# apache/datafusion-comet

Hardware: AMD Instinct MI355X
Metric: rows/sec, TPC-H SF100 Q1 scan->filter->agg (HBM-resident Arrow columns) (higher is better)
Workload: dtype i128 (Decimal128; 256-bit products) / i32 (Date32) / u8 (Utf8 keys); 1 GPU; TPC-H SF100 Q1 stage 1 (Filter -> Project, 3 decimal ops incl. one 256-bit multiply -> partial HashAggregate, 2 Utf8 keys, 8 aggregates) per GPU; rows_per_gpu=600037902, bytes_per_row_algorithmic=78, parallelism=row-range shards x1, jit_toolchain=hiprtc 9.0; comgr 3.0 /opt/rocm/lib/libamd_comgr.so.3

## Files before the change

### datafusion-comet_amd/csrc/exec.cpp

```cpp
#include "exec.hpp"
#include "shuffle_format.hpp"

#include <cerrno>
#include <fcntl.h>
#include <unistd.h>
#include <chrono>
#include <condition_variable>
#include <cstdio>
#include <cstdlib>
#include <cmath>
#include <cstring>
#include <functional>
#include <map>
#include <mutex>

#include "exec_internal.hpp"

namespace comet {

static bool list_of_flat(const DType& t) { return t.id == TypeId::List && t.kids.size() == 1 && !t.kids[0].is_nested(); }
DevTable extend_struct_fields(const DevTable& in) {
  bool any = false;
  for (auto& t : in.types) any |= t.id == TypeId::Struct || list_of_flat(t);
  if (!any) return in;
// ... 847 lines not shown
    const bool fused = is_build ? fbit != ctx.fused_build_.end() : fit != ctx.fused_probe_.end();
    if (fused || op.children[s].get() == leaf[s]) {
      types[s] = leaf[s]->scan_fields;
      valid[s] = hv;
    } else {
      const PipelineDesc cd = generate_pipeline(*op.children[s], hv);
      for (auto& oc : cd.out_cols) {
        types[s].push_back(oc.type);
        valid[s].push_back(oc.nullable);
      }
    }
  }
  JoinFusion fu, fub;
  if (fit != ctx.fused_probe_.end()) { fu = fit->second.fu; fu.src_valid = valid[build_left ? 1 : 0]; }
  if (fbit != ctx.fused_build_.end()) { fub = fbit->second.fu; fub.src_valid = valid[build_left ? 0 : 1]; }
  return generate_join(op, types[0], types[1], valid[0], valid[1], fit != ctx.fused_probe_.end() ? &fu : nullptr, fbit != ctx.fused_build_.end() ? &fub : nullptr);
}

std::string ExecutionContext::compile_only(OperatorP plan, uint64_t plan_hash) {
  size_t nscan = 0;
  std::function<void(const Operator&)> cnt = [&](const Operator& op) {
    if (op.kind == OpKind::Scan) nscan++;
    for (auto& c : op.children) cnt(*c);
  };
  cnt(*plan);
  std::vector<InputSource> ins(nscan);
  ExecutionContext ctx(plan, plan_hash, {}, ins, 8192, 0);
  std::vector<bool> none(ctx.in_types_.size(), false);
  if (ctx.has_join_) {
    ctx.compile_in_infer_ = true;
    ctx.explain_.clear();
    ctx.infer_schema(*ctx.root_source_);
    if (ctx.plan_.get() != ctx.root_source_) {
      auto pv = planned_variant(*ctx.plan_, ctx.plan_hash_, none, true, &ctx.in_types_);
      ctx.explain_ += pv->desc.explain;
    }
  } else {
    planned_variant(*ctx.plan_, ctx.plan_hash_, none, true);
  }
  return ctx.explain_;
}

Variant ExecutionContext::node_variant(const Operator& node, const char* tag, const std::string& validity, const std::function<PipelineDesc()>& generate) {
  const std::string key = std::to_string(plan_hash_ ^ (0x9E3779B97F4A7C15ull * (uint64_t)(node_id_[&node] + 1))) + tag + validity;
  std::shared_ptr<PlannedVariant> pv;
  {
    std::lock_guard<std::mutex> lk(g_plan_mu);
    auto it = g_plan_cache.find(key);
    if (it != g_plan_cache.end()) pv = it->second;
  }
  if (!pv) {
    pv = std::make_shared<PlannedVariant>();
    pv->desc = generate();
    pv->code = jit_compile(pv->desc.source);
    std::lock_guard<std::mutex> lk(g_plan_mu);
    g_plan_cache[key] = pv;
  }
  Variant v;
  v.desc = pv->desc;
  note_sites(v.desc);
  v.mod = jit_load(pv->code);
  return v;
}

Variant& ExecutionContext::variant_for(const std::vector<bool>& has_valid, const std::vector<int>& str_fixed_len) {
  std::string key = validity_key(has_valid) + ":";
  bool any_fixed = false;
  for (int l : str_fixed_len) { key += std::to_string(l) + ","; any_fixed |= l >= 0; }
  auto it = variants_.find(key);
  if (it != variants_.end()) return it->second;
  auto pv = planned_variant(*plan_, plan_hash_, has_valid, true, has_join_ ? &in_types_ : nullptr, any_fixed ? &str_fixed_len : nullptr,
                            dict_id_col_.empty() ? nullptr : &dict_id_col_);
  Variant v;
  v.desc = pv->desc;
  note_sites(v.desc);
  v.mod = jit_load(pv->code);
  auto res = variants_.emplace(key, std::move(v));
  return res.first->second;
}

void ExecutionContext::launch(Variant& v, const char* kernel, int grid, CometKParams& prm, int block) {
  hipFunction_t fn = v.mod->fn(kernel);
  if (!v.desc.blooms.empty()) bind_blooms(v.desc, prm);
  void* args[] = {&prm};
  if (!g_kernel_times.load(std::memory_order_relaxed)) {
    HIP_CHECK(hipModuleLaunchKernel(fn, (unsigned)grid, 1, 1, (unsigned)block, 1, 1, 0, stream_, args, nullptr));
    return;
  }
  hipEvent_t a = pool_get_event(device_id_), b = pool_get_event(device_id_);
  HIP_CHECK(hipEventRecord(a, stream_));
  HIP_CHECK(hipModuleLaunchKernel(fn, (unsigned)grid, 1, 1, (unsigned)block, 1, 1, 0, stream_, args, nullptr));
  HIP_CHECK(hipEventRecord(b, stream_));
  kt_pending_.push_back({kernel, a, b});
}

std::atomic<int> g_kernel_times{getenv("COMET_KERNEL_TIMES") != nullptr && atoi(getenv("COMET_KERNEL_TIMES")) != 0 ? 1 : 0};

std::string ExecutionContext::kernel_times_json() {
  if (!kt_pending_.empty()) {
    HIP_CHECK(hipStreamSynchronize(stream_));
    for (auto& p : kt_pending_) {
      float ms = 0;
      if (hipEventElapsedTime(&ms, p.a, p.b) == hipSuccess) { kernel_times_[p.name].first += ms; kernel_times_[p.name].second++; }
      pool_put_event(device_id_, p.a);
      pool_put_event(device_id_, p.b);
    }
    kt_pending_.clear();
  }
  std::string s = "{";
  for (auto& kv : kernel_times_) {
    char buf[160];
    snprintf(buf, sizeof buf, "%s\"%s\": {\"ms\": %.6f, \"calls\": %lld}", s.size() > 1 ? ", " : "", kv.first.c_str(), kv.second.first, (long long)kv.second.second);
    s += buf;
  }
  return s + "}";
}

void ExecutionContext::prepare_dict_keys(DevTable& src) {
  if (src.rows == 0) return;
  std::vector<bool> none(in_types_.size(), false);
  auto pv = planned_variant(*plan_, plan_hash_, none, false, &in_types_);
  std::vector<int> key_cols = pv->desc.str_key_cols;
  std::sort(key_cols.begin(), key_cols.end());
  key_cols.erase(std::unique(key_cols.begin(), key_cols.end()), key_cols.end());
  if (key_cols.empty()) return;
  const int64_t n = src.rows;
  std::vector<int> id_col(src.cols.size(), -1);
  bool any = false;
  bool need = device_result_;
  for (int c : key_cols) {
    const DeviceColumnView& sc = src.cols[(size_t)c];
    if (sc.offset != 0) return;
    if (need) break;
    if (sc.fixed_len >= 0 && sc.fixed_len <= 15) continue;
    uint32_t* mx = (uint32_t*)err_flags_.p + (kErrBytes / 4 - 1);
    HIP_CHECK(hipMemsetAsync(mx, 0, 4, stream_));
    if (comet_launch_str_max_len((const int32_t*)sc.data, n, mx, stream_) != 0) throw CometError("string keys: launch failed");
    uint32_t longest = 0;
    read_small(&longest, mx, 4);
    HIP_CHECK(hipMemsetAsync(mx, 0, 4, stream_));
    need = longest > 15;
  }
  if (!need || src.cols.size() + key_cols.size() > COMET_MAX_IN) return;
  for (int c : key_cols) {
    const DeviceColumnView& sc = src.cols[(size_t)c];
    if (n >= ((int64_t)1 << 32) - 1) throw CometError("Utf8 group keys longer than 15 bytes over more than 2^32 rows are not supported");
    int64_t slots = 1024;
    while (slots < 2 * n) slots <<= 1;
    DevBuf table;
    table.ensure((size_t)slots * 4);
    HIP_CHECK(hipMemsetAsync(table.p, 0, (size_t)slots * 4, stream_));
    auto rep = std::make_shared<DevBuf>();
    rep->ensure((size_t)n * 8 + 16);
    if (comet_launch_str_dict_build((const int32_t*)sc.data, (const uint8_t*)sc.aux, src.has_valid[(size_t)c] ? sc.valid : nullptr, n, (uint32_t*)table.p, slots,
                                    (int64_t*)rep->p, stream_) != 0)
      throw CometError("string keys: launch failed");
    HIP_CHECK(hipStreamSynchronize(stream_));
    DeviceColumnView idv;
    idv.data = rep->p;
    idv.valid = sc.valid;
    id_col[(size_t)c] = (int)src.cols.size();
    src.types.push_back(DType::of(TypeId::Int64));
    src.cols.push_back(idv);
    src.has_valid.push_back(src.has_valid[(size_t)c]);
    src.owners.push_back(rep);
    any = true;
// ... 641 lines not shown
  c.type = t;
  c.length = rows;
  auto fetch = [&](std::vector<uint8_t>& dst, const void* src, size_t bytes) {
    dst.resize(bytes);
    if (bytes) HIP_CHECK(hipMemcpyAsync(dst.data(), src, bytes, hipMemcpyDeviceToHost, st));
  };
  if (has_valid && v.valid && rows) fetch(c.validity, v.valid, (size_t)((rows + 7) / 8));
  if (t.id == TypeId::Struct) {
    for (size_t i = 0; i < t.kids.size(); i++)
      c.children.push_back(download_column(v.kids.at(i), t.kids[i], i < v.kid_has_valid.size() && v.kid_has_valid[i], rows, st));
  } else if (t.is_listlike()) {
    fetch(c.values, v.data, (size_t)(rows + 1) * 4);
    HIP_CHECK(hipStreamSynchronize(st));
    const int64_t nel = rows ? ((const int32_t*)c.values.data())[rows] : 0;
    if (nel < 0 || nel > v.kid_rows) throw CometError("internal: list offsets run past the element column");
    c.children.push_back(download_column(v.kids.at(0), t.kids.at(0), !v.kid_has_valid.empty() && v.kid_has_valid[0], nel, st));
  } else if (t.id == TypeId::String || t.id == TypeId::Bytes) {
    fetch(c.values, (const int32_t*)v.data + v.offset, (size_t)(rows + 1) * 4);
    HIP_CHECK(hipStreamSynchronize(st));
    const int32_t* o = (const int32_t*)c.values.data();
    const int64_t lo = rows ? o[0] : 0, hi = rows ? o[rows] : 0;
    if (hi > lo) fetch(c.data, (const uint8_t*)v.aux + lo, (size_t)(hi - lo));
    if (lo) { int32_t* w = (int32_t*)c.values.data(); for (int64_t i = 0; i <= rows; i++) w[i] -= (int32_t)lo; }
  } else if (t.id == TypeId::Bool) {
    fetch(c.values, v.data, (size_t)((rows + 7) / 8));
  } else {
    fetch(c.values, v.data, (size_t)rows * (size_t)fixed_width(t));
  }
  HIP_CHECK(hipStreamSynchronize(st));
  if (!c.validity.empty()) {
    int64_t nulls = 0;
    for (int64_t i = 0; i < rows; i++) nulls += !((c.validity[(size_t)(i >> 3)] >> (i & 7)) & 1);
    c.null_count = nulls;
    if (!nulls) c.validity.clear();
  }
  return c;
}
namespace {
std::vector<uint8_t> slice_bits(const std::vector<uint8_t>& b, int64_t off, int64_t len) {
  std::vector<uint8_t> o((size_t)((len + 7) / 8), 0);
  for (int64_t i = 0; i < len; i++)
    if ((b[(size_t)((off + i) >> 3)] >> ((off + i) & 7)) & 1) o[(size_t)(i >> 3)] |= (uint8_t)(1u << (i & 7));
  return o;
}
HostColumn slice_column(const HostColumn& c, int64_t off, int64_t len) {
  if (off == 0 && len == c.length) return c;
  HostColumn o;
  o.type = c.type;
  o.length = len;
  if (!c.validity.empty()) {
    o.validity = slice_bits(c.validity, off, len);
    for (int64_t i = 0; i < len; i++) o.null_count += !((o.validity[(size_t)(i >> 3)] >> (i & 7)) & 1);
    if (!o.null_count) o.validity.clear();
  }
  const TypeId id = c.type.id;
  if (id == TypeId::Struct) {
    for (auto& k : c.children) o.children.push_back(slice_column(k, off, len));
  } else if (id == TypeId::List || id == TypeId::Map || id == TypeId::String || id == TypeId::Bytes) {
    const int32_t* src = (const int32_t*)c.values.data();
    o.values.resize((size_t)(len + 1) * 4);
    int32_t* w = (int32_t*)o.values.data();
    for (int64_t i = 0; i <= len; i++) w[i] = src[off + i] - src[off];
    if (id == TypeId::List || id == TypeId::Map) o.children.push_back(slice_column(c.children.at(0), src[off], src[off + len] - src[off]));
    else o.data.assign(c.data.begin() + src[off], c.data.begin() + src[off + len]);
  } else if (id == TypeId::Bool) {
    o.values = slice_bits(c.values, off, len);
  } else {
    const size_t w = (size_t)fixed_width(c.type);
    o.values.assign(c.values.begin() + (size_t)off * w, c.values.begin() + (size_t)(off + len) * w);
  }
  return o;
}
}

void ExecutionContext::table_to_host_batches(const DevTable& t) {
  if (t.rows == 0) return;
  const size_t ncol = t.cols.size();
  std::vector<HostColumn> nested(ncol);
  for (size_t j = 0; j < ncol; j++)
    if (t.types[j].is_nested()) nested[j] = download_column(t.cols[j], t.types[j], t.has_valid[j], t.rows, stream_);
  std::vector<std::vector<uint8_t>> hv(ncol), hb(ncol);
  std::vector<std::vector<uint8_t>> hd(ncol);
  struct Piece { const void* src; std::vector<uint8_t>* dst; size_t bytes; };
  auto fetch = [&](std::vector<Piece>& pieces) {
    size_t total = 0, longest = 0;
    for (auto& pc : pieces) { pc.dst->resize(pc.bytes); total += (pc.bytes + 15) & ~(size_t)15; longest = std::max(longest, pc.bytes); }
    if (pieces.empty()) return;
    static const bool batched = getenv("COMET_EXPORT_BATCHED") == nullptr || atoi(getenv("COMET_EXPORT_BATCHED")) != 0;
    if (batched && total > 0 && total <= ((size_t)1 << 20) && pieces.size() <= 256) {
      struct Desc { const uint8_t* src; uint8_t* dst; uint64_t len; };
      const size_t head = (pieces.size() * sizeof(Desc) + 63) & ~(size_t)63;
      export_host_.ensure(head + total + 64);
      Desc* d = (Desc*)export_host_.p;
      size_t at = head;
      for (size_t k = 0; k < pieces.size(); k++) {
        d[k].src = (const uint8_t*)pieces[k].src;
        d[k].dst = (uint8_t*)export_host_.p + at;
        d[k].len = pieces[k].bytes;
        at += (pieces[k].bytes + 15) & ~(size_t)15;
      }
      if (comet_launch_copy_small(export_host_.p, (int)pieces.size(), (uint64_t)longest, stream_) != 0) throw CometError("result export: launch failed");
      HIP_CHECK(hipStreamSynchronize(stream_));
      for (size_t k = 0; k < pieces.size(); k++)
        if (pieces[k].bytes) memcpy(pieces[k].dst->data(), d[k].dst, pieces[k].bytes);
      return;
    }
    for (auto& pc : pieces)
      if (pc.bytes) HIP_CHECK(hipMemcpyAsync(pc.dst->data(), pc.src, pc.bytes, hipMemcpyDeviceToHost, stream_));
    HIP_CHECK(hipStreamSynchronize(stream_));
  };
  std::vector<Piece> pieces;
  for (size_t j = 0; j < ncol; j++) {
    const DType& ty = t.types[j];
    if (ty.is_nested()) continue;
    const bool is_str = ty.id == TypeId::String || ty.id == TypeId::Bytes;
    size_t bytes = is_str ? (size_t)(t.rows + 1) * 4 : ty.id == TypeId::Bool ? (size_t)((t.rows + 7) / 8) : (size_t)t.rows * fixed_width(ty);
    pieces.push_back({t.cols[j].data, &hv[j], bytes});
    if (t.has_valid[j]) pieces.push_back({t.cols[j].valid, &hb[j], (size_t)((t.rows + 7) / 8)});
  }
  fetch(pieces);
  pieces.clear();
  for (size_t j = 0; j < ncol; j++) {
    if (t.types[j].id == TypeId::String || t.types[j].id == TypeId::Bytes) {
      const int32_t* offs = (const int32_t*)hv[j].data();
      if (offs[t.rows] > 0) pieces.push_back({t.cols[j].aux, &hd[j], (size_t)offs[t.rows]});
    }
  }
  fetch(pieces);
  check_device_errors();
  const int64_t bs = batch_size_ > 0 ? batch_size_ : t.rows;
  auto getbit = [](const std::vector<uint8_t>& b, int64_t i) { return (b[(size_t)(i >> 3)] >> (i & 7)) & 1; };
  for (int64_t off = 0; off < t.rows; off += bs) {
    const int64_t len = std::min(bs, t.rows - off);
    HostBatch b;
    b.rows = len;
    for (size_t j = 0; j < ncol; j++) {
      if (t.types[j].is_nested()) { b.cols.push_back(slice_column(nested[j], off, len)); continue; }
      HostColumn c;
      c.type = t.types[j];
      c.length = len;
      if (c.type.id == TypeId::String || c.type.id == TypeId::Bytes) {
        const int32_t* offs = (const int32_t*)hv[j].data();
        c.values.resize((size_t)(len + 1) * 4);
        int32_t* o = (int32_t*)c.values.data();
        for (int64_t i = 0; i <= len; i++) o[i] = offs[off + i] - offs[off];
        c.data.assign(hd[j].begin() + offs[off], hd[j].begin() + offs[off + len]);
      } else if (c.type.id == TypeId::Bool) {
        c.values.assign((size_t)((len + 7) / 8), 0);
        for (int64_t i = 0; i < len; i++)
          if (getbit(hv[j], off + i)) c.values[(size_t)(i >> 3)] |= (uint8_t)(1u << (i & 7));
      } else {
        int w = fixed_width(c.type);
        c.values.assign(hv[j].begin() + (size_t)off * w, hv[j].begin() + (size_t)(off + len) * w);
      }
      if (t.has_valid[j]) {
        int64_t nulls = 0;
        std::vector<uint8_t> bm((size_t)((len + 7) / 8), 0);
        for (int64_t i = 0; i < len; i++) {
          if (getbit(hb[j], off + i)) bm[(size_t)(i >> 3)] |= (uint8_t)(1u << (i & 7));
          else nulls++;
        }
        c.null_count = nulls;
        if (nulls) c.validity = std::move(bm);
      }
      b.cols.push_back(std::move(c));
    }
    ready_.push_back(std::move(b));
  }
}

void ExecutionContext::run_to_completion() {
  if (has_join_) {
    DevTable src = extend_struct_fields(materialize(*root_source_));
    if (plan_.get() == root_source_) throw CometError("internal: bare join root");
    if (sink_ == SinkKind::AggGrouped) prepare_dict_keys(src);
    single_chunk_hint_ = true;
    process_chunk(src.cols, src.has_valid, src.rows);
    HIP_CHECK(hipStreamSynchronize(stream_));
    return;
  }
  while (true) {
    bool more = inputs_[0].kind == 0 ? pull_host_chunk() : pull_device_batch();
    if (!more) break;
  }
}

void ExecutionContext::start() {
  if (!started_) {
    HIP_CHECK(hipSetDevice(device_id_));
    stream_ = pool_get_stream(device_id_);
    err_flags_.ensure(kErrBytes);
    HIP_CHECK(hipMemsetAsync(err_flags_.p, 0, kErrBytes, stream_));
    started_ = true;
  } else {
    HIP_CHECK(hipSetDevice(device_id_));
  }
}

namespace {
struct ExportedDeviceColumn {
  std::vector<std::shared_ptr<void>> owners;
  const void* buffers[3];
};
void release_device_array(ArrowArray* a) {
  delete (ExportedDeviceColumn*)a->private_data;
  a->release = nullptr;
}
void release_fmt_schema(ArrowSchema* s) {
  delete (std::string*)s->private_data;
  s->release = nullptr;
}
}

void ExecutionContext::set_memory_manager(int64_t (*acquire)(void*, int64_t), void (*release)(void*, int64_t), void* ctx, long long task_id) {
  mem_->acquire = acquire;
  mem_->release = release;
  mem_->ctx = ctx;
  mem_->task_id = task_id;
}
void ExecutionContext::memory_stats(int64_t out[4]) {
  out[0] = mem_->host_used.load();
  out[1] = mem_->host_peak.load();
  out[2] = mem_->dev_used.load();
  out[3] = mem_->dev_peak.load();
}

int64_t ExecutionContext::execute_device(ArrowDeviceArray** out_arrays, ArrowSchema** out_schemas, int n_out) {
  mem_->owner = std::this_thread::get_id();
  AccountScope account(mem_);
  mem_->flush();
  Timer t;
  start();
  if (sink_ == SinkKind::AggNoGroup)
    throw CometError("comet_execute_plan_device: an ungrouped aggregate result is one row and is exported through comet_execute_plan");
  if (finished_) return -1;
  DevTable tab;
  if (sink_ == SinkKind::AggGrouped) {
    device_result_ = true;
    run_to_completion();
    tab = grouped_to_device();
  } else {
    tab = materialize(*plan_);
  }
  HIP_CHECK(hipStreamSynchronize(stream_));
  check_device_errors();
  collect_timings();
  finished_ = true;
  if ((size_t)n_out != tab.cols.size())
    throw CometError("Output column count mismatch: expected " + std::to_string(n_out) + ", got " + std::to_string(tab.cols.size()));
  for (size_t c = 0; c < tab.types.size(); c++)
    if (tab.types[c].is_nested()) throw CometError("executePlan (device arrays): nested column of type " + tab.types[c].str() + " — nested results are exported through host batches");
  for (int j = 0; j < n_out; j++) {
    const DType& ty = tab.types[(size_t)j];
    const bool is_str = ty.id == TypeId::String || ty.id == TypeId::Bytes;
    if (tab.cols[(size_t)j].offset != 0) throw CometError("comet_execute_plan_device: input column with a non-zero Arrow offset passed through");
    auto* ec = new ExportedDeviceColumn();
    ec->owners = tab.owners;
    ec->buffers[0] = tab.has_valid[(size_t)j] ? tab.cols[(size_t)j].valid : nullptr;
    ec->buffers[1] = tab.cols[(size_t)j].data;
    ec->buffers[2] = is_str ? tab.cols[(size_t)j].aux : nullptr;
    ArrowDeviceArray* d = out_arrays[j];
    memset(d, 0, sizeof *d);
    d->array.length = tab.rows;
    d->array.null_count = tab.has_valid[(size_t)j] ? -1 : 0;
    d->array.n_buffers = is_str ? 3 : 2;
    d->array.buffers = ec->buffers;
    d->array.private_data = ec;
    d->array.release = release_device_array;
    d->device_id = device_id_;
    d->device_type = ARROW_DEVICE_ROCM;
    d->sync_event = nullptr;
    ArrowSchema* s = out_schemas[j];
    memset(s, 0, sizeof *s);
    auto* fmt = new std::string(expected_format(ty));
    s->format = fmt->c_str();
    s->name = "";
    s->flags = ARROW_FLAG_NULLABLE;
    s->private_data = fmt;
    s->release = release_fmt_schema;
  }
  output_rows_ += tab.rows;
  elapsed_compute_ns_ += t.ns();
  return tab.rows;
}

void ExecutionContext::resolve_subqueries() {
  if (subqueries_resolved_) return;
  subqueries_resolved_ = true;
  uint64_t sig = 0xcbf29ce484222325ull;
  auto mix = [&](const void* p, size_t n) { for (size_t k = 0; k < n; k++) sig = (sig ^ ((const uint8_t*)p)[k]) * 0x100000001b3ull; };
  for (auto& e : plan_->subqueries) {
    if (e->kind != ExprKind::Subquery) continue;
    const int64_t id = e->lit_i64;
    bool is_null = true;
    std::string v;
    bool found = false;
    auto it = subquery_values_.find(id);
    if (it != subquery_values_.end()) { is_null = it->second.first; v = it->second.second; found = true; }
    else if (subquery_provider_) found = subquery_provider_(id, e->dtype, is_null, v);
    if (!found) throw CometError("Subquery " + std::to_string(id) + " is not registered with this plan (CometScalarSubquery.setSubquery / comet_plan_set_subquery)");
    auto need = [&](size_t n) { if (!is_null && v.size() < n) throw CometError("Subquery " + std::to_string(id) + ": the value has " + std::to_string(v.size()) + " bytes, its type needs " + std::to_string(n)); };
    e->kind = ExprKind::Literal;
    e->proto_tag = 2;
    e->lit_null = is_null;
    e->lit_i64 = 0;
    int64_t i = 0;
    double d = 0;
    switch (e->dtype.id) {
      case TypeId::Bool: need(1); e->lit_bool = !is_null && v[0] != 0; e->lit_case = 1; break;
      case TypeId::Int8: case TypeId::Int16: case TypeId::Int32: case TypeId::Date: case TypeId::Int64: case TypeId::Timestamp: case TypeId::TimestampNtz:
        need(8);
        if (!is_null) memcpy(&i, v.data(), 8);
        e->lit_i64 = i;
        e->lit_case = e->dtype.id == TypeId::Int8 ? 2 : e->dtype.id == TypeId::Int16 ? 3 : (e->dtype.id == TypeId::Int32 || e->dtype.id == TypeId::Date) ? 4 : 5;
        break;
      case TypeId::Float: case TypeId::Double:
        need(8);
        if (!is_null) memcpy(&d, v.data(), 8);
        e->lit_f64 = e->dtype.id == TypeId::Float ? (double)(float)d : d;
        e->lit_case = e->dtype.id == TypeId::Float ? 6 : 7;
        break;
      case TypeId::Decimal: e->lit_dec = is_null ? 0 : decode_decimal_be(v); e->lit_case = 10; break;
      case TypeId::String: case TypeId::Bytes: e->lit_bytes = is_null ? std::string() : v; e->lit_case = e->dtype.id == TypeId::String ? 8 : 9; break;
      default: throw CometError("Unsupported scalar subquery data type " + e->dtype.str());
    }
    mix(&id, 8);
    mix(&is_null, 1);
    if (e->bloom_arg) {
// ... 89 lines not shown
```

### datafusion-comet_amd/csrc/exec.hpp

```cpp
#pragma once
#include <mutex>
#include <thread>
#include <atomic>
#include <hip/hip_runtime_api.h>

#include <deque>
#include <functional>
#include <map>
#include <set>
#include <memory>
#include <string>
#include <vector>

#include "arrow_abi.hpp"
#include "codegen.hpp"
#include "jit.hpp"
#include "kparams.h"
#include "plan.hpp"

namespace comet {
double process_clock_ms();

struct MemAccount {
  int64_t (*acquire)(void* ctx, int64_t bytes) = nullptr;
// ... 76 lines not shown

struct DevTable {
  int64_t rows = 0;
  std::vector<DType> types;
  std::vector<DeviceColumnView> cols;
  std::vector<bool> has_valid;
  std::vector<std::shared_ptr<void>> owners;
};

struct Staging {
  std::vector<std::unique_ptr<PinnedBuf>> stage_vals, stage_valid, stage_aux;
  std::vector<std::unique_ptr<DevBuf>> dev_vals, dev_valid, dev_aux;
  std::vector<int> dict_index_width;
  std::vector<std::shared_ptr<void>> nested_keep;
  hipEvent_t busy = nullptr;
};

struct Variant {
  PipelineDesc desc;
  std::shared_ptr<LoadedModule> mod;
};

struct BloomAggSpec { int version = 1, k = 1; int64_t num_words = 0; };
BloomAggSpec bloom_agg_spec(const Operator& hash_agg);
bool is_bloom_agg(const Operator& op);
struct BloomRegistry {
  std::map<int64_t, ExprP> subquery_nodes;
  std::map<const Expr*, std::shared_ptr<struct DevBuf>> buffers;
  std::vector<ExprP> keep;
};

void scan_pool_parallel(size_t n, const std::function<void(size_t)>& fn);
std::string parquet_prune_report(const Operator& native_scan, bool page_index, bool bloom_filters = true);
std::vector<uint8_t> parquet_host_plain_values(const Operator& native_scan, size_t column);
void scan_pool_submit(std::function<void()> fn);

extern std::atomic<int> g_kernel_times;

class ExecutionContext {
 public:
  ExecutionContext(OperatorP plan, uint64_t plan_hash, std::vector<std::pair<std::string, std::string>> config,
                   std::vector<InputSource> inputs, int batch_size, int device_id);
  ~ExecutionContext();

  int64_t execute(ArrowArray** out_arrays, ArrowSchema** out_schemas, int n_out);
  int64_t execute_device(ArrowDeviceArray** out_arrays, ArrowSchema** out_schemas, int n_out);
  std::string metrics_proto();
  void set_memory_manager(int64_t (*acquire)(void*, int64_t), void (*release)(void*, int64_t), void* ctx, long long task_id);
  typedef std::function<bool(int64_t id, const DType& type, bool& is_null, std::string& value)> SubqueryProvider;
  void set_subquery_provider(SubqueryProvider p) { subquery_provider_ = std::move(p); }
  void set_subquery_value(int64_t id, bool is_null, std::string value) { subquery_values_[id] = {is_null, std::move(value)}; }
  void resolve_subqueries();
  void memory_stats(int64_t out[4]);
  std::shared_ptr<MemAccount> memory_account() const { return mem_; }
  const std::string& explain();
  static std::string compile_only(OperatorP plan, uint64_t plan_hash);
  static std::string check_only(OperatorP plan, uint64_t plan_hash);
  static PipelineDesc join_codegen(OperatorP plan, uint64_t plan_hash, const std::vector<bool>& has_valid);

  std::string last_error;
  int last_error_kind = 0;

  double last_kernel_ms = 0;
  int64_t last_kernel_launches = 0;
  std::string kernel_times_json();
  double last_aux_ms = 0;
  int64_t last_aux_launches = 0;
  int64_t input_rows = 0;

 private:
  void run_to_completion();
  void start();
  std::vector<std::vector<int>> fixed_len_hint_;
  Variant& variant_for(const std::vector<bool>& has_valid, const std::vector<int>& str_fixed_len);
  void process_chunk(const std::vector<DeviceColumnView>& cols, const std::vector<bool>& has_valid, int64_t n);
  void finish_aggregate();
  void finish_grouped();
  DevTable grouped_to_device();
  std::vector<DType> infer_schema(const Operator& op);
  DevTable materialize(const Operator& op);
  DevTable scan_parquet(const Operator& native_scan);
  friend struct ParquetScan;
  friend struct HashJoinRun;
  int64_t launch_fused_filter(Variant& v, CometKParams& prm, int64_t n);
  DevTable run_chain_to_device(const Operator& top, const DevTable& in);
  void extend_derived(DevTable& in, const std::vector<DerivedCol>& derived);
  void extend_derived_strfn(DevTable& in, const DerivedCol& dc);
  DevTable hash_join(const Operator& j, const DevTable& l, const DevTable& r);
  DevTable hash_join_impl(const Operator& node, const Operator& j, const DevTable& l, const DevTable& r, const std::string& key_suffix,
                          const JoinFusion* fused_probe = nullptr, const JoinFusion* fused_build = nullptr);
  struct FusedProbe { const Operator* source = nullptr; JoinFusion fu; };
  bool plan_fused_probe(const Operator& join, const std::vector<DType>& build_types, PipelineDesc& desc);
  bool plan_fused_build(const Operator& join, FusedProbe& fb);
  DevTable sort_table(const Operator& s, const DevTable& in);
  Variant node_variant(const Operator& node, const char* tag, const std::string& validity, const std::function<PipelineDesc()>& generate);
  std::shared_ptr<DevBuf> sort_key_planes(const Operator& s, const DevTable& in, int& W, std::vector<int64_t>* str_len = nullptr, bool measure_only = false);
  DevTable literal_table(const std::vector<std::vector<ExprP>>& rows, const std::vector<DType>& types);
  DevTable take_rows(const DevTable& in, const uint32_t* dev_perm, int64_t first, int64_t rows, std::shared_ptr<DevBuf> perm_owner);
  DevTable nested_aggregate(const Operator& agg);
  DevTable write_shuffle(const Operator& sw);
  DevTable expand(const Operator& ex, const DevTable& in);
  DevTable explode(const Operator& ex, const DevTable& in);
  DevTable window(const Operator& w, const DevTable& in);
  DevTable bloom_aggregate(const Operator& agg, const DevTable& in);
  const void* bloom_buffer(const PipelineDesc::BloomRef& ref);
  void bind_blooms(const PipelineDesc& d, CometKParams& prm);
  void prepare_dict_keys(DevTable& src);
  static bool is_source(const Operator& op, const Operator* chain_top);
  typedef std::function<std::pair<const DevTable*, int>(int)> GatherSource;
  DevTable outputs_to_table(Variant& v, const std::vector<std::shared_ptr<DevBuf>>& vals, const std::vector<std::shared_ptr<DevBuf>>& valid_bytes,
                            int64_t rows, const GatherSource& gather_source = nullptr);
  DeviceColumnView take_column(const DeviceColumnView& src, const DType& t, bool has_valid, const uint32_t* idx, const uint8_t* ok_bytes, int64_t rows, bool& out_has_valid,
                               std::vector<std::shared_ptr<void>>& owners);
  void take_utf8(const DeviceColumnView& src, const uint32_t* idx, const uint8_t* ok_bytes, const uint8_t* src_valid_bits, int64_t rows,
                 DeviceColumnView& out, std::vector<std::shared_ptr<void>>& owners);
  void table_to_host_batches(const DevTable& t);
  DevTable host_batch_to_table(const HostBatch& b);
  bool pull_host_chunk();
  bool pull_device_batch();
  bool pull_host_table(size_t input, const std::vector<DType>& types, int64_t max_rows, std::vector<DeviceColumnView>& views,
                       std::vector<bool>& has_valid, int64_t& rows);
  bool pull_device_table(size_t input, const std::vector<DType>& types, std::vector<DeviceColumnView>& views, std::vector<bool>& has_valid,
                         int64_t& rows, std::shared_ptr<void>& keepalive);
  void validate_input_schema(size_t input, const std::vector<DType>& types);
  void export_batch(HostBatch& b, ArrowArray** out_arrays, ArrowSchema** out_schemas, int n_out);
  void check_device_errors();
  void raise_device_errors(uint32_t flags);
  void note_sites(const PipelineDesc& d) {
    site_ctx_last_.clear();
    for (auto& kv : d.site_contexts) {
      site_ctx_last_[kv.first] = kv.second;
      auto it = site_ctx_.find(kv.first);
      if (it == site_ctx_.end()) site_ctx_[kv.first] = kv.second;
      else if (it->second != kv.second && !(it->second && kv.second && it->second->sql_text == kv.second->sql_text && it->second->start_index == kv.second->start_index &&
                                            it->second->stop_index == kv.second->stop_index))
        site_ctx_ambiguous_.insert(kv.first);
    }
    for (int k = 0; k < 2; k++) if (d.agg_ctx[k]) agg_ctx_[k] = d.agg_ctx[k];
  }
  const QueryContext* site_context(uint32_t id) const {
    auto a = site_ctx_last_.find(id);
    if (a != site_ctx_last_.end()) return a->second.get();
    if (site_ctx_ambiguous_.count(id)) return nullptr;
    auto b = site_ctx_.find(id);
    return b == site_ctx_.end() ? nullptr : b->second.get();
  }
  std::map<uint32_t, std::shared_ptr<QueryContext>> site_ctx_last_;
  std::set<uint32_t> site_ctx_ambiguous_;
  std::shared_ptr<QueryContext> agg_ctx_[2];
  std::map<uint32_t, std::shared_ptr<QueryContext>> site_ctx_;
  void read_small(void* dst, const void* dev_src, size_t n);
  void write_small(void* dev_dst, const void* src, size_t n);
  void timed_begin();
  void timed_end();
  void collect_timings();
  void launch(Variant& v, const char* kernel, int grid, CometKParams& prm, int block = 256);

  OperatorP plan_;
  uint64_t plan_hash_ = 0;
  std::vector<std::pair<std::string, std::string>> config_;
  std::vector<InputSource> inputs_;
  int batch_size_;
  int device_id_;
  int64_t chunk_rows_;
  hipStream_t stream_ = nullptr;
  std::vector<std::pair<hipEvent_t, hipEvent_t>> timed_;
  size_t timed_done_ = 0;
  struct KtPending { std::string name; hipEvent_t a, b; };
  std::vector<KtPending> kt_pending_;
  std::map<std::string, std::pair<double, int64_t>> kernel_times_;
  hipEvent_t aux_ev_[2] = {nullptr, nullptr};
  int aux_n_ = 0;
  bool started_ = false, finished_ = false;
  std::vector<DType> in_types_;
  std::map<std::string, Variant> variants_;
  Variant* agg_variant_ = nullptr;
  std::string explain_;
  SinkKind sink_ = SinkKind::Output;
  bool has_join_ = false;
  SubqueryProvider subquery_provider_;
  std::map<int64_t, std::pair<bool, std::string>> subquery_values_;
  bool subqueries_resolved_ = false;
  int64_t strfn_rows_ = 0;
  int64_t split_rows_ = 0;
  bool materialize_root_ = false;
  bool compile_in_infer_ = false;
  std::vector<const Operator*> nested_aggs_;
  struct ExpandPart {
    OperatorP proj;
    std::vector<int> out_col;
    std::vector<int> null_cols;
  };
  struct ExpandInfo {
    std::vector<ExpandPart> parts;
    std::vector<OutCol> out_cols;
  };
  std::map<const Operator*, ExpandInfo> expand_info_;
  std::map<const Operator*, OperatorP> bloom_proj_;
  std::shared_ptr<BloomRegistry> blooms_;
  std::map<const Operator*, OperatorP> explode_proj_;
  std::map<const Operator*, OperatorP> window_psort_, window_osort_;
  std::map<const Operator*, OperatorP> range_sort_, range_bsort_;
  std::shared_ptr<void> planes_owner_;
  std::map<const Operator*, OperatorP> shuffle_projs_;
  int64_t shuffle_bytes_written_ = 0, shuffle_data_size_ = 0, shuffle_staged_peak_ = 0;
  double shuffle_repart_ns_ = 0, shuffle_write_ns_ = 0;
  std::vector<int> dict_id_col_;
  bool device_result_ = false;
  DevTable dict_src_;
  std::map<const Operator*, FusedProbe> fused_probe_;
  std::map<const Operator*, FusedProbe> fused_build_;
  int64_t ramp_rows_ = 0;
  bool fuse_probe_ = true;
  int fuse_build_ = 1;
  std::set<const Operator*> smj_needs_sort_;
  std::map<const Operator*, OperatorP> smj_sorts_;
  const Operator* root_source_ = nullptr;
  std::map<const Operator*, int> node_id_;
  std::map<const Operator*, size_t> scan_input_;
  int64_t join_build_rows_ = 0, join_probe_rows_ = 0, join_keymap_bytes_ = 0, join_direct_maps_ = 0, join_bucket_tables_ = 0, join_bitmap_only_ = 0, join_mono_tables_ = 0, join_fused_builds_ = 0;
  int small_write_slot_ = 0;
  bool single_chunk_hint_ = false, part_result_ready_ = false;
  DevTable part_result_;
  int64_t part_merges_ = 0;
  bool try_partitioned_merge(Variant& v, CometKParams& prm, int64_t n);
  struct DevPending {
    std::vector<DeviceColumnView> views;
    std::vector<bool> has_valid;
    int64_t rows = 0;
    std::shared_ptr<void> keep;
    bool valid = false;
  };
  DevPending dev_pending_;
  bool dev_stream_done_ = false;
// ... 40 lines not shown
```

### datafusion-comet_amd/csrc/exec_bloom.cpp

```cpp
#include "exec_internal.hpp"
#include "device/bloom.hpp"

#include "../../include/comet_amd.h"

extern "C" int comet_launch_bloom_put(const void* vals, int width, const uint8_t* valid_bits, int64_t first, int64_t n, uint64_t* f, int64_t nwords, void* stream);
extern "C" int comet_launch_bloom_merge(const uint8_t* src_words, int64_t nwords, uint64_t* f, void* stream);
extern "C" int comet_launch_bloom_finish(const uint64_t* f, int64_t nwords, uint8_t* out, uint64_t* popcnt, void* stream);

namespace comet {

namespace {

uint32_t be32(const uint8_t* p) { return ((uint32_t)p[0] << 24) | ((uint32_t)p[1] << 16) | ((uint32_t)p[2] << 8) | p[3]; }

struct BloomHeader {
  int32_t version = 0, k = 0, seed = 0, num_words = 0;
  size_t header_bytes = 0;
};

bool read_header(const uint8_t* p, size_t len, BloomHeader& h) {
  if (len < 4) return false;
  h.version = (int32_t)be32(p);
  h.header_bytes = h.version == 2 ? 16 : 12;
  if (h.version != 1 && h.version != 2) return true;
// ... 99 lines not shown
  auto hit = blooms_->buffers.find(node);
  if (hit != blooms_->buffers.end()) return hit->second->p;
  if (node->kind != ExprKind::Literal || node->lit_null) throw CometError("internal: might_contain bound to a filter without bytes");
  BloomHeader h;
  const uint8_t* p = (const uint8_t*)node->lit_bytes.data();
  const std::string why = bloom_bytes_problem(p, node->lit_bytes.size(), h);
  if (!why.empty()) throw CometError("might_contain: " + why);
  const std::vector<uint64_t> f = to_device_layout(p, h);
  auto buf = std::make_shared<DevBuf>();
  buf->ensure(f.size() * 8);
  HIP_CHECK(hipMemcpy(buf->p, f.data(), f.size() * 8, hipMemcpyHostToDevice));
  blooms_->buffers[node] = buf;
  blooms_->keep.push_back(ref.node);
  return buf->p;
}

void ExecutionContext::bind_blooms(const PipelineDesc& d, CometKParams& prm) {
  for (size_t j = 0; j < d.blooms.size(); j++) prm.in[COMET_MAX_IN - 1 - j].data = bloom_buffer(d.blooms[j]);
}


DevTable ExecutionContext::bloom_aggregate(const Operator& op, const DevTable& in) {
  const BloomAggSpec spec = bloom_agg_spec(op);
  const size_t fbytes = ((size_t)kBloomHeaderWords + (size_t)spec.num_words + 1) * 8;
  DevBuf acc;
  acc.ensure(fbytes);
  HIP_CHECK(hipMemsetAsync(acc.p, 0, fbytes, stream_));
  const uint64_t header[kBloomHeaderWords] = {(uint64_t)spec.version, (uint64_t)spec.k, 0, (uint64_t)spec.num_words};
  write_small(acc.p, header, sizeof header);
  uint64_t* const f = (uint64_t*)acc.p;
  uint64_t* const popcnt = f + kBloomHeaderWords + spec.num_words;
  if (op.agg_mode == AggMode::Partial) {
    DevTable col = run_chain_to_device(*bloom_proj_.at(&op), in);
    const DType& t = col.types.at(0);
    if (!t.is_integer()) throw CometError("bloom_filter_agg over " + t.str() + " is not supported by the MI355X native engine");
    timed_begin();
    if (comet_launch_bloom_put(col.cols[0].data, fixed_width(t), col.has_valid[0] ? col.cols[0].valid : nullptr, col.cols[0].offset, col.rows, f, spec.num_words, stream_) != 0)
      throw CometError("bloom_filter_agg: launch failed");
    HIP_CHECK(hipStreamSynchronize(stream_));
  } else {
    const size_t sc = (size_t)std::max(0, op.initial_input_buffer_offset);
    if (sc >= in.cols.size() || (in.types[sc].id != TypeId::Bytes && in.types[sc].id != TypeId::String))
      throw CometError("bloom_filter_agg: the merging aggregate expects its Binary state in column " + std::to_string(sc) + " of its child");
    const DeviceColumnView& s = in.cols[sc];
    std::vector<int32_t> offs((size_t)in.rows + 1, 0);
    std::vector<uint8_t> vbits;
    if (in.rows) {
      HIP_CHECK(hipMemcpyAsync(offs.data(), (const int32_t*)s.data + s.offset, offs.size() * 4, hipMemcpyDeviceToHost, stream_));
      if (in.has_valid[sc] && s.valid) {
        vbits.resize((size_t)((s.offset + in.rows + 7) / 8));
        HIP_CHECK(hipMemcpyAsync(vbits.data(), s.valid, vbits.size(), hipMemcpyDeviceToHost, stream_));
      }
      HIP_CHECK(hipStreamSynchronize(stream_));
    }
    timed_begin();
    for (int64_t r = 0; r < in.rows; r++) {
      if (!vbits.empty() && !((vbits[(size_t)((s.offset + r) >> 3)] >> ((s.offset + r) & 7)) & 1)) continue;
      const int64_t lo = offs[(size_t)r], len = (int64_t)offs[(size_t)r + 1] - lo;
      if (lo < 0 || len < 0) throw CometError("bloom_filter_agg: the state column's offsets are not ascending");
      uint8_t hb[16] = {0};
      const size_t have = (size_t)std::min<int64_t>(len, 16);
      if (have) read_small(hb, (const uint8_t*)s.aux + lo, have);
      BloomHeader h;
      if (have < 4) throw CometError("BloomFilter merge: truncated bit array (got 0 bytes, expected " + std::to_string(spec.num_words * 8) + ")");
      h.version = (int32_t)be32(hb);
      if (h.version != spec.version) throw CometError("BloomFilter merge: version mismatch (got " + std::to_string(h.version) + ", expected " + std::to_string(spec.version) + ")");
      if (!read_header(hb, have, h)) throw CometError("BloomFilter merge: truncated bit array (got 0 bytes, expected " + std::to_string(spec.num_words * 8) + ")");
      if (h.k != spec.k) throw CometError("BloomFilter merge: num_hash_functions mismatch (got " + std::to_string((uint32_t)h.k) + ", expected " + std::to_string(spec.k) + ")");
      if (h.seed != 0) throw CometError("BloomFilter merge: seed mismatch (got " + std::to_string(h.seed) + ", expected 0)");
      if ((int64_t)h.num_words != spec.num_words)
        throw CometError("BloomFilter merge: num_words mismatch (got " + std::to_string((uint32_t)h.num_words) + ", expected " + std::to_string(spec.num_words) + ")");
      if (len - (int64_t)h.header_bytes < spec.num_words * 8)
        throw CometError("BloomFilter merge: truncated bit array (got " + std::to_string(len - (int64_t)h.header_bytes) + " bytes, expected " + std::to_string(spec.num_words * 8) + ")");
      if (comet_launch_bloom_merge((const uint8_t*)s.aux + lo + h.header_bytes, spec.num_words, f, stream_) != 0) throw CometError("bloom_filter_agg: launch failed");
    }
  }
  const size_t hdr = spec.version == 2 ? 16 : 12, out_len = hdr + (size_t)spec.num_words * 8;
  auto bytes = std::make_shared<DevBuf>(), out_offs = std::make_shared<DevBuf>();
  bytes->ensure(out_len + 16);
  out_offs->ensure(16);
  if (comet_launch_bloom_finish(f, spec.num_words, (uint8_t*)bytes->p, popcnt, stream_) != 0) throw CometError("bloom_filter_agg: launch failed");
  timed_end();
  uint64_t set_bits = 0;
  read_small(&set_bits, popcnt, 8);
  check_device_errors();
  const bool is_null = op.agg_mode == AggMode::Final && set_bits == 0;
  const int32_t o[2] = {0, is_null ? 0 : (int32_t)out_len};
  write_small(out_offs->p, o, sizeof o);
  DevTable out;
  out.rows = 1;
  out.types.push_back(DType::of(TypeId::Bytes));
  DeviceColumnView v;
  v.data = out_offs->p;
  v.aux = bytes->p;
  out.owners.push_back(out_offs);
  out.owners.push_back(bytes);
  if (is_null) {
    auto vb = std::make_shared<DevBuf>();
    vb->ensure(16);
    const uint8_t zero[8] = {0};
    write_small(vb->p, zero, sizeof zero);
    v.valid = (const uint8_t*)vb->p;
    out.owners.push_back(vb);
  }
  out.cols.push_back(v);
  out.has_valid.push_back(is_null);
  HIP_CHECK(hipStreamSynchronize(stream_));
  return out;
}

}


extern "C" int32_t comet_spark_bloom_might_contain(const uint8_t* bytes, size_t len, int64_t value) {
  comet::BloomHeader h;
  if (!bytes || !comet::bloom_bytes_problem(bytes, len, h).empty()) return -1;
  const std::vector<uint64_t> f = comet::to_device_layout(bytes, h);
  return comet::bloom_might_contain((const comet::u64*)f.data(), (comet::i64)value) ? 1 : 0;
}

extern "C" int64_t comet_spark_bloom_build(const int64_t* values, const uint8_t* valid, int64_t n, int64_t num_items, int64_t num_bits, int32_t version, uint8_t* out, int64_t cap) {
  comet::Operator op;
  op.kind = comet::OpKind::HashAgg;
  comet::AggExpr a;
  a.kind = comet::AggKind::BloomFilter;
  auto lit = [](int64_t v) {
    auto e = std::make_shared<comet::Expr>();
    e->kind = comet::ExprKind::Literal;
    e->dtype = comet::DType::of(comet::TypeId::Int64);
    e->has_dtype = true;
    e->lit_i64 = v;
    return e;
  };
  a.children.push_back(lit(0));
  a.bloom_num_items = lit(num_items);
  a.bloom_num_bits = lit(num_bits);
  a.bloom_version = version == 2 ? 2 : 1;
  op.agg_exprs.push_back(a);
  comet::BloomAggSpec s;
  try {
    s = comet::bloom_agg_spec(op);
  } catch (const comet::CometError&) {
    return -1;
  }
  std::vector<uint64_t> f((size_t)comet::kBloomHeaderWords + (size_t)s.num_words, 0);
  f[0] = (uint64_t)s.version;
  f[1] = (uint64_t)s.k;
  f[3] = (uint64_t)s.num_words;
  for (int64_t i = 0; i < n; i++)
    if (!valid || ((valid[i >> 3] >> (i & 7)) & 1)) comet::bloom_put((comet::u64*)f.data(), (comet::i64)values[i]);
  const std::string bytes = comet::serialize(f);
  if (out && cap >= (int64_t)bytes.size()) memcpy(out, bytes.data(), bytes.size());
  return (int64_t)bytes.size();
}
```

### datafusion-comet_amd/csrc/exec_input.cpp

```cpp
#include "exec_internal.hpp"
#include <emmintrin.h>
#include <mutex>
#include <set>
#include <tuple>

namespace comet {

static void stream_copy(void* dst, const void* src, size_t n) {
  char* d = (char*)dst;
  const char* s = (const char*)src;
  if (n < 4096) { memcpy(d, s, n); return; }
  const size_t head = (size_t)(-(intptr_t)d) & 15;
  if (head) { memcpy(d, s, head); d += head; s += head; n -= head; }
  size_t blocks = n / 64;
  for (; blocks; blocks--, d += 64, s += 64) {
    const __m128i a = _mm_loadu_si128((const __m128i*)s), b = _mm_loadu_si128((const __m128i*)(s + 16)), c = _mm_loadu_si128((const __m128i*)(s + 32)),
                  e = _mm_loadu_si128((const __m128i*)(s + 48));
    _mm_stream_si128((__m128i*)d, a);
    _mm_stream_si128((__m128i*)(d + 16), b);
    _mm_stream_si128((__m128i*)(d + 32), c);
    _mm_stream_si128((__m128i*)(d + 48), e);
  }
  _mm_sfence();
  if (n & 63) memcpy(d, s, n & 63);
// ... 487 lines not shown
}


namespace {
struct UniformKey {
  const void* off; int64_t rows; int32_t len; int32_t first;
  bool operator<(const UniformKey& o) const { return std::tie(off, rows, len, first) < std::tie(o.off, o.rows, o.len, o.first); }
};
std::mutex g_uniform_mu;
std::set<UniformKey> g_uniform_ok;
bool uniform_verdict_known(const void* off, int64_t rows, int32_t len, int32_t first) {
  std::lock_guard<std::mutex> g(g_uniform_mu);
  return g_uniform_ok.count(UniformKey{off, rows, len, first}) != 0;
}
void remember_uniform_verdict(const void* off, int64_t rows, int32_t len, int32_t first) {
  std::lock_guard<std::mutex> g(g_uniform_mu);
  if (g_uniform_ok.size() >= 4096) g_uniform_ok.clear();
  g_uniform_ok.insert(UniformKey{off, rows, len, first});
}
}

bool ExecutionContext::pull_device_table(size_t input, const std::vector<DType>& types, std::vector<DeviceColumnView>& views,
                                         std::vector<bool>& has_valid, int64_t& rows, std::shared_ptr<void>& keepalive) {
  InputSource& in = inputs_[input];
  rows = 0;
  if (in.exhausted) return false;
  static const bool trace = getenv("COMET_TRACE_STAGES") != nullptr;
  Timer tm;
  validate_input_schema(input, types);
  const double t_schema = tm.ns();
  auto da = std::make_shared<ArrowDeviceArray>();
  memset(da.get(), 0, sizeof(ArrowDeviceArray));
  int rc = in.dev->get_next(in.dev, da.get());
  if (trace) fprintf(stderr, "[comet] device input %zu: get_schema %.3f ms, get_next %.3f ms\n", input, t_schema / 1e6, (tm.ns() - t_schema) / 1e6);
  if (rc != 0) {
    const char* m = in.dev->get_last_error ? in.dev->get_last_error(in.dev) : nullptr;
    throw CometError(std::string("input ArrowDeviceArrayStream.get_next failed: ") + (m ? m : "unknown error"));
  }
  if (!da->array.release) {
    in.exhausted = true;
    return false;
  }
  keepalive = std::shared_ptr<void>(da.get(), [da](void*) mutable {
    if (da->array.release) da->array.release(&da->array);
  });
  if (da->device_type != ARROW_DEVICE_ROCM && da->device_type != ARROW_DEVICE_ROCM_HOST)
    throw CometError("device input stream must carry ARROW_DEVICE_ROCM memory");
  if (da->sync_event) HIP_CHECK(hipStreamWaitEvent(stream_, *(hipEvent_t*)da->sync_event, 0));
  const size_t nc = types.size();
  if ((size_t)da->array.n_children != nc) throw CometError("device batch column count does not match Scan fields");
  views.assign(nc, DeviceColumnView());
  has_valid.assign(nc, false);
  for (size_t c = 0; c < nc; c++) {
    const ArrowArray* col = da->array.children[c];
    if (col->dictionary) throw CometError("dictionary-encoded device columns are not supported yet");
    views[c].data = col->buffers[1];
    views[c].offset = col->offset;
    if (types[c].id == TypeId::String || types[c].id == TypeId::Bytes) views[c].aux = col->buffers[2];
    if (types[c].id == TypeId::Decimal && (((uintptr_t)col->buffers[1]) & 15))
      throw CometError("device Decimal128 buffers must be 16-byte aligned");
    if (col->null_count != 0 && col->buffers[0]) {
      has_valid[c] = true;
      views[c].valid = (const uint8_t*)col->buffers[0];
    }
  }
  rows = da->array.length;
  std::vector<size_t> scols;
  for (size_t c = 0; c < nc && rows > 0; c++)
    if (types[c].id == TypeId::String) scols.push_back(c);
  if (!scols.empty() && scols.size() <= 16) {
    small_host_.ensure(4096);
    int32_t* ends = (int32_t*)small_host_.p;
    for (size_t k = 0; k < scols.size(); k++) {
      const ArrowArray* col = da->array.children[scols[k]];
      const int32_t* off = (const int32_t*)col->buffers[1] + col->offset;
      HIP_CHECK(hipMemcpyAsync(ends + 2 * k, off, 4, hipMemcpyDeviceToHost, stream_));
      HIP_CHECK(hipMemcpyAsync(ends + 2 * k + 1, off + rows, 4, hipMemcpyDeviceToHost, stream_));
    }
    HIP_CHECK(hipStreamSynchronize(stream_));
    std::vector<int32_t> first(scols.size()), len(scols.size(), -1);
    std::vector<bool> declared(scols.size(), false);
    uint32_t* flags = (uint32_t*)err_flags_.p + (kErrBytes / 4 - 16);
    HIP_CHECK(hipMemsetAsync(flags, 0, 64, stream_));
    bool any = false;
    if (!aux_ev_[0]) { aux_ev_[0] = pool_get_event(device_id_); aux_ev_[1] = pool_get_event(device_id_); }
    HIP_CHECK(hipEventRecord(aux_ev_[0], stream_));
    int aux_launched = 0;
    for (size_t k = 0; k < scols.size(); k++) {
      first[k] = ends[2 * k];
      const int64_t total = (int64_t)ends[2 * k + 1] - ends[2 * k];
      const int hint = input < fixed_len_hint_.size() && scols[k] < fixed_len_hint_[input].size() ? fixed_len_hint_[input][scols[k]] : -1;
      const ArrowArray* col = da->array.children[scols[k]];
      const int32_t* off = (const int32_t*)col->buffers[1] + col->offset;
      if (hint >= 0) {
        if (total != (int64_t)hint * rows)
          throw CometError("device input column " + std::to_string(scols[k]) + " is declared comet:utf8_fixed_len=" + std::to_string(hint) + " but holds " +
                           std::to_string(total) + " bytes in " + std::to_string(rows) + " rows");
        if ((int64_t)first[k] != (int64_t)col->offset * hint) continue;
        if (uniform_verdict_known(off, rows, hint, first[k])) {
          views[scols[k]].fixed_len = hint;
          continue;
        }
        if (comet_launch_utf8_uniform(off, rows, hint, flags + k, stream_) != 0) continue;
        aux_launched++;
        len[k] = hint;
        declared[k] = true;
        any = true;
        continue;
      }
      if (total % rows != 0 || total / rows > 15 || total < 0) continue;
      if (comet_launch_utf8_uniform(off, rows, (int32_t)(total / rows), flags + k, stream_) != 0) continue;
      aux_launched++;
      len[k] = (int32_t)(total / rows);
      any = true;
    }
    if (any) {
      HIP_CHECK(hipEventRecord(aux_ev_[1], stream_));
      uint32_t f[16];
      read_small(f, flags, 64);
      float aux = 0;
      if (hipEventElapsedTime(&aux, aux_ev_[0], aux_ev_[1]) == hipSuccess) { last_aux_ms += aux; last_aux_launches += aux_launched; }
      HIP_CHECK(hipMemsetAsync(flags, 0, 64, stream_));
      for (size_t k = 0; k < scols.size(); k++) {
        if (len[k] < 0) continue;
        const size_t c = scols[k];
        const ArrowArray* col = da->array.children[c];
        if (declared[k]) {
          if (f[k] != 0)
            throw CometError("device input column " + std::to_string(c) + " is declared comet:utf8_fixed_len=" + std::to_string(len[k]) +
                             " but its offsets are not " + std::to_string(len[k]) + " bytes apart (the byte total alone matches)");
          remember_uniform_verdict((const int32_t*)col->buffers[1] + col->offset, rows, len[k], first[k]);
          views[c].fixed_len = len[k];
          continue;
        }
        if (f[k] != 0) continue;
        if ((int64_t)first[k] != (int64_t)col->offset * len[k]) continue;
        views[c].fixed_len = len[k];
      }
    }
  }
  return true;
}

bool ExecutionContext::pull_device_batch() {
  DevPending cur;
  if (dev_pending_.valid) {
    cur = std::move(dev_pending_);
    dev_pending_ = DevPending();
  } else {
    if (dev_stream_done_ || !pull_device_table(0, in_types_, cur.views, cur.has_valid, cur.rows, cur.keep)) return false;
  }
  if (sink_ == SinkKind::AggGrouped && dev_chunks_seen_ == 0 && !dev_stream_done_) {
    dev_pending_.valid = pull_device_table(0, in_types_, dev_pending_.views, dev_pending_.has_valid, dev_pending_.rows, dev_pending_.keep);
    if (!dev_pending_.valid) dev_stream_done_ = true;
    single_chunk_hint_ = !dev_pending_.valid;
  } else {
    single_chunk_hint_ = false;
  }
  dev_chunks_seen_++;
  process_chunk(cur.views, cur.has_valid, cur.rows);
  HIP_CHECK(hipStreamSynchronize(stream_));
  return true;
}


}
```

### datafusion-comet_amd/csrc/exec_internal.hpp

```cpp
#pragma once
#include "exec.hpp"
#include "shuffle_format.hpp"
#include "fix_scale.hpp"

#include <cerrno>
#include <fcntl.h>
#include <unistd.h>
#include <chrono>
#include <condition_variable>
#include <cstdio>
#include <cstdlib>
#include <cmath>
#include <cstring>
#include <functional>
#include <map>
#include <mutex>

extern "C" int comet_launch_dict_gather_fixed(const void* idx, int iw, const uint8_t* idx_valid, const uint8_t* dict, const uint8_t* dict_valid,
                                              int width, int64_t n, uint8_t* out, uint8_t* out_valid_bytes, void* stream);
extern "C" int comet_launch_dict_gather_str_len(const void* idx, int iw, const uint8_t* idx_valid, const int32_t* dict_offs, const uint8_t* dict_valid,
                                                int64_t n, uint32_t* lengths, uint8_t* out_valid_bytes, void* stream);
extern "C" int comet_launch_dict_gather_str_copy(const void* idx, int iw, const uint8_t* valid_bytes, const int32_t* dict_offs, const uint8_t* dict_bytes,
                                                 int64_t n, const int32_t* out_offs, uint8_t* out_bytes, void* stream);
extern "C" void pq_launch_u32_scan(const uint32_t* in, int64_t n, uint64_t* tiles, int32_t* out, void* st);
// ... 8 lines not shown
                                          int out_width, void* out, uint8_t* out_ok, void* stream);
extern "C" int comet_launch_window_range_bounds(int width, const void* keys, const uint8_t* valid, const int32_t* sp, const uint32_t* first_part, int64_t n, int desc, int nulls_first,
                                                int has_lo, int64_t dlo, int has_hi, int64_t dhi, int32_t* out_lo, int32_t* out_hi, void* stream);
extern "C" int comet_launch_window_valid_flags(const uint8_t* valid, int64_t n, uint32_t* flags, void* stream);
extern "C" int comet_launch_window_pick(int mode, int64_t nth, int lo_kind, int64_t lo_off, int hi_kind, int64_t hi_off, const int32_t* C, const int32_t* sp, const int32_t* sg,
                                        const uint32_t* first_part, const uint32_t* first_peer, int64_t n, uint32_t* idx, uint8_t* ok, void* stream);
extern "C" int comet_launch_window_agg(int fn, int lo_kind, int64_t lo_off, int hi_kind, int64_t hi_off, const void* S128, const void* SH128, const int32_t* C, const int32_t* sp, const int32_t* sg, const uint32_t* first_part,
                                       const uint32_t* first_peer, int64_t n, const void* bound16, const void* scaler16, const void* avg_bound16, void* out, uint8_t* out_ok,
                                       void* stream);
extern "C" int comet_launch_window_fexp(int width, const void* src, const uint8_t* valid_bits, int64_t n, uint64_t* hi_lo, void* stream);
extern "C" int comet_launch_scan192_f64(int width, const void* src, const uint8_t* valid_bits, int64_t n, int scale, int slice, void* tiles, void* out192, void* stream);
extern "C" int comet_launch_scan128_fclass(int width, const void* src, const uint8_t* valid_bits, int64_t n, void* tiles, void* out128, void* stream);
extern "C" int comet_launch_window_fagg(int fn, int lo_kind, int64_t lo_off, int hi_kind, int64_t hi_off, const void* S192, int windows, const void* K128, int scale, const int32_t* sp, const int32_t* sg,
                                        const uint32_t* first_part, const uint32_t* first_peer, int64_t n, double* out, uint8_t* out_ok, void* stream);
extern "C" int comet_launch_window_flags(const uint8_t* part_planes, int Wp, const uint8_t* order_planes, int Wo, int64_t n, uint32_t* fpart, uint32_t* fpeer, void* stream);
extern "C" int comet_launch_window_first(const uint32_t* fpart, const int32_t* sp, const uint32_t* fpeer, const int32_t* sg, int64_t n, uint32_t* first_part,
                                         uint32_t* first_peer, void* stream);
extern "C" int comet_launch_window_rank(int kind, int64_t arg, const int32_t* sp, const int32_t* sg, const uint32_t* first_part, const uint32_t* first_peer, int64_t n,
                                        void* out, void* stream);
extern "C" int comet_launch_window_offset(int64_t shift, const int32_t* sp, const uint32_t* first_part, int64_t n, uint32_t* idx, uint8_t* ok, void* stream);
extern "C" int comet_launch_window_offset_valid(const uint32_t* idx, const uint8_t* ok, const uint8_t* src_valid_bits, int64_t n, uint8_t* out_ok, void* stream);
struct CometConcatArgs {
  int32_t n;
  int32_t lit_len[8];
  const int32_t* offs[8];
  const uint8_t* bytes[8];
  int64_t first[8];
};
extern "C" int comet_launch_concat_lengths(const CometConcatArgs* a, const uint32_t* rows, const uint8_t* ok_bytes, int64_t n, uint32_t* lengths, void* stream);
extern "C" int comet_launch_concat_copy(const CometConcatArgs* a, const uint32_t* rows, const uint8_t* ok_bytes, int64_t n, const int32_t* out_offs, uint8_t* out_bytes, void* stream);
extern "C" int comet_launch_strcase_lengths(const void* views, const uint8_t* ok_bytes, const int32_t* src_offs, const uint8_t* src_bytes, int64_t n, int mode, uint32_t* lengths, void* stream);
extern "C" int comet_launch_strcase_write(const void* views, const uint8_t* ok_bytes, const int32_t* src_offs, const uint8_t* src_bytes, int64_t n, int mode, const int32_t* out_offs,
                                          uint8_t* out_bytes, void* stream);
extern "C" int comet_launch_join_part_scan(uint32_t* cnt, int g, int np, uint32_t* tot, uint32_t limit, uint64_t* over, void* stream);
extern "C" int comet_launch_popcount128(const void* blocks, int64_t n, uint32_t* counts, void* stream);
extern "C" int comet_launch_strfmt_lengths(int kind, long long arg, const void* vals128, const uint8_t* ok_bytes, int64_t n, uint32_t* lengths, void* stream);
extern "C" int comet_launch_strfmt_write(int kind, long long arg, const void* vals128, const uint8_t* ok_bytes, int64_t n, const int32_t* out_offs, uint8_t* out_bytes, void* stream);
extern "C" int comet_launch_strfn_len(int op, const int32_t* offs, const uint8_t* bytes, const uint8_t* valid_bits, int64_t valid_first, int64_t n, const uint8_t* a, int32_t na, const uint8_t* b,
                                      int32_t nb, int64_t k, uint32_t* lengths, uint32_t* too_long, void* stream);
extern "C" int comet_launch_strfn_write(int op, const int32_t* offs, const uint8_t* bytes, const uint8_t* valid_bits, int64_t valid_first, int64_t n, const uint8_t* a, int32_t na, const uint8_t* b,
                                        int32_t nb, int64_t k, const int32_t* out_offs, uint8_t* out, void* stream);
extern "C" int comet_launch_split_count(const int32_t* offs, const uint8_t* bytes, const uint8_t* valid_bits, int64_t valid_first, int64_t n, const uint32_t* prog, const uint32_t* prog2, int32_t limit,
                                        uint32_t* counts, void* stream);
extern "C" int comet_launch_split_write(const int32_t* offs, const uint8_t* bytes, const uint8_t* valid_bits, int64_t valid_first, int64_t n, const uint32_t* prog, const uint32_t* prog2, int32_t limit,
                                        const int32_t* list_offs, void* views, void* stream);
extern "C" int comet_launch_strview_lengths(const void* views, const uint8_t* ok_bytes, int64_t n, const uint8_t* pattern, int32_t pattern_bytes, uint32_t* lengths, void* stream);
extern "C" int comet_launch_strview_copy(const void* views, const uint8_t* ok_bytes, const int32_t* src_offs, const uint8_t* src_bytes, int64_t n, const uint8_t* pattern,
                                         int32_t pattern_bytes, int pad_left, const int32_t* out_offs, uint8_t* out_bytes, void* stream);
extern "C" int comet_launch_str16_lengths(const void* packed, const uint8_t* ok_bytes, int64_t n, uint32_t* lengths, void* stream);
extern "C" int comet_launch_str16_copy(const void* packed, const int32_t* offsets, int64_t n, uint8_t* bytes, void* stream);
extern "C" int comet_launch_str_max_len(const int32_t* offs, int64_t n, uint32_t* out_max, void* stream);
extern "C" int comet_launch_str_dict_build(const int32_t* offs, const uint8_t* bytes, const uint8_t* valid_bits, int64_t n, uint32_t* table, int64_t slots,
                                           int64_t* rep, void* stream);
extern "C" int comet_launch_str_dict_lookup(const int32_t* build_offs, const uint8_t* build_bytes, const uint32_t* table, int64_t slots, const int32_t* offs,
                                            const uint8_t* bytes, const uint8_t* valid_bits, int64_t n, int64_t* rep, uint8_t* ok, void* stream);
extern "C" int64_t comet_partition_tiles(int64_t n);
extern "C" int64_t comet_partition_scratch_bytes(int64_t n, int32_t P);
extern "C" int comet_launch_fill(int width, void* dst, int64_t n, const void* value, void* stream);
extern "C" int comet_launch_copy_small(const void* descs, int n, uint64_t longest, void* stream);
extern "C" int comet_launch_murmur3(int type_id, int precision, const void* values, const uint8_t* validity, const void* aux, int64_t n, uint32_t* hashes, void* stream);
extern "C" int comet_launch_pmod(const uint32_t* hashes, int64_t n, int32_t np, int32_t* out, void* stream);
extern "C" int comet_launch_partition_indices(const int32_t* pids, int64_t n, int32_t P, uint64_t* hist, uint32_t* bad, int64_t* starts,
                                              uint32_t* row_indices, void* stream);
extern "C" int comet_launch_take(int width, const void* src, const uint32_t* idx, int64_t n, void* dst, void* stream);
extern "C" int comet_launch_take_utf8_lengths(const int32_t* offs, const uint32_t* idx, const uint8_t* ok_bytes, const uint8_t* src_valid_bits, int64_t n,
                                              uint32_t* lengths, void* stream);
extern "C" int comet_launch_explode_counts(const int32_t* offs, const uint8_t* valid_bits, int64_t n, int outer, uint32_t* counts, void* stream);
extern "C" int comet_launch_explode_indices(const int32_t* offs, const uint8_t* valid_bits, const uint8_t* elem_valid_bits, int64_t n, const int32_t* out_offs, uint32_t* row_idx,
                                            uint32_t* elem_idx, uint8_t* has_elem, int32_t* pos, uint8_t* elem_ok, void* stream);
extern "C" int comet_launch_take_list_indices(const int32_t* offs, const uint32_t* idx, int64_t n, const int32_t* out_offs, uint32_t* elem_idx, void* stream);
extern "C" int comet_launch_take_utf8_copy(const int32_t* offs, const uint8_t* bytes, const uint32_t* idx, const uint8_t* ok_bytes, const uint8_t* src_valid_bits,
                                           int64_t n, const int32_t* out_offs, uint8_t* out_bytes, void* stream);
extern "C" void pq_launch_u32_scan(const uint32_t* in, int64_t n, uint64_t* tiles, int32_t* out, void* st);
extern "C" int comet_launch_sort_small(const uint8_t* planes, int64_t n, const uint32_t* cand, int m, const int* plane_idx, int nv, uint32_t* out, void* stream);
extern "C" int comet_launch_sort_iota(uint32_t* perm, int64_t n, uint32_t first, void* stream);
extern "C" int comet_launch_sort_gather_digit(const uint8_t* plane, const uint32_t* perm, int64_t n, int32_t* digit, void* stream);
extern "C" int comet_launch_range_partition_ids(const uint8_t* planes, int64_t n, int W, const uint8_t* bkeys, int B, int32_t* pids, void* stream);
extern "C" int comet_launch_sort_plane_varies(const uint8_t* planes, int64_t n, int W, uint32_t* flags, void* stream);
extern "C" int comet_launch_sort_hist256(const uint8_t* plane, const uint32_t* cand, int64_t m, uint64_t* hist, void* stream);
extern "C" int comet_launch_sort_select(const uint8_t* plane, const uint32_t* cand, int64_t m, int dstar, uint32_t* sure, uint32_t* next_cand, uint32_t* counters,
                                        void* stream);
extern "C" int comet_launch_fix_rescale(uint64_t* base, int64_t count, int64_t stride_words, int32_t word_off, int32_t shift, void* stream);
extern "C" int comet_launch_utf8_uniform(const int32_t* offsets, int64_t n, int32_t L, uint32_t* flag, void* stream);

namespace comet {
HostColumn download_column(const DeviceColumnView& v, const DType& t, bool has_valid, int64_t rows, hipStream_t st);

namespace detail {
void plan_execution_begins();
void plan_execution_ends();
int plans_executing();

hipStream_t pool_get_stream(int dev);
void pool_put_stream(int dev, hipStream_t s);
hipEvent_t pool_get_event(int dev);
void pool_put_event(int dev, hipEvent_t e);

int fixed_width(const DType& t);
inline int out_width(const OutCol& oc) { return (oc.view_src >= 0 || oc.fmt_kind) ? 16 : (oc.gather_src >= 0 || !oc.concat_cols.empty()) ? 4 : oc.packed_string ? 16 : (oc.type.id == TypeId::Bool ? 1 : fixed_width(oc.type)); }
void bit_append(uint8_t* dst, int64_t dst_off, const uint8_t* src, int64_t src_off, int64_t n);
bool nested_schema_matches(const ArrowSchema* f, const DType& t);
void append_nested_rows(HostColumn& dst, const ArrowArray* a, const DType& t, int64_t off, int64_t len);
void bit_fill_ones(uint8_t* dst, int64_t dst_off, int64_t n);
bool format_matches(const char* fmt, const DType& t);
struct SrcFmt {
  enum Cls { Unknown, Int, UInt, F32, F64, Date32, Date64, Ts, Dec, Utf8, LargeUtf8, Bool } cls = Unknown;
  int width = 0;
  int64_t per_second = 0;
  int p = 0, s = 0;
};
SrcFmt parse_src_format(const char* fmt);
bool scan_cast_supported(const SrcFmt& f, const DType& t);
bool scan_cast_value(const SrcFmt& f, const char* src, int64_t i, const DType& t, char* dst);
const Operator* find_scan(const Operator* op);
std::string validity_key(const std::vector<bool>& v);
void bind_inputs(CometKParams& prm, const std::vector<DeviceColumnView>& cols, const std::vector<bool>& has_valid, size_t first_slot = 0);
u128 pow10_u128_host(int p);
struct Timer {
  std::chrono::steady_clock::time_point t0 = std::chrono::steady_clock::now();
  double ns() const { return (double)std::chrono::duration_cast<std::chrono::nanoseconds>(std::chrono::steady_clock::now() - t0).count(); }
};

struct PlannedVariant {
  PipelineDesc desc;
  std::shared_ptr<CodeObject> code;
};
extern std::mutex g_plan_mu;
extern std::map<std::string, std::shared_ptr<PlannedVariant>> g_plan_cache;
std::shared_ptr<PlannedVariant> planned_variant(const Operator& plan, uint64_t plan_hash, const std::vector<bool>& has_valid, bool compile,
                                                const std::vector<DType>* source_types = nullptr, const std::vector<int>* str_fixed_len = nullptr,
                                                const std::vector<int>* dict_id_col = nullptr);

}
using namespace detail;
}
```

### datafusion-comet_amd/csrc/exec_join.cpp

```cpp
#include "exec_internal.hpp"

namespace comet {
DevTable ExecutionContext::hash_join(const Operator& j, const DevTable& L, const DevTable& R) {
  auto is_str = [](const DType& t) { return t.id == TypeId::String || t.id == TypeId::Bytes; };
  std::vector<size_t> sk;
  for (size_t k = 0; k < j.left_keys.size() && k < j.right_keys.size(); k++) {
    const ExprP &a = j.left_keys[k], &b = j.right_keys[k];
    if (a->kind == ExprKind::Bound && b->kind == ExprKind::Bound && a->bound_index >= 0 && b->bound_index >= 0 && (size_t)a->bound_index < L.types.size() &&
        (size_t)b->bound_index < R.types.size() && is_str(L.types[(size_t)a->bound_index]) && is_str(R.types[(size_t)b->bound_index]) &&
        L.cols[(size_t)a->bound_index].offset == 0 && R.cols[(size_t)b->bound_index].offset == 0)
      sk.push_back(k);
  }
  if (sk.empty() || L.rows == 0 || R.rows == 0 || L.cols.size() + R.cols.size() + 2 * sk.size() > COMET_MAX_IN) return hash_join_impl(j, j, L, R, "");
  auto longest = [&](const DevTable& t, int c) {
    uint32_t* mx = (uint32_t*)err_flags_.p + (kErrBytes / 4 - 1);
    HIP_CHECK(hipMemsetAsync(mx, 0, 4, stream_));
    if (comet_launch_str_max_len((const int32_t*)t.cols[(size_t)c].data, t.rows, mx, stream_) != 0) throw CometError("string keys: launch failed");
    uint32_t v = 0;
    read_small(&v, mx, 4);
    HIP_CHECK(hipMemsetAsync(mx, 0, 4, stream_));
    return v;
  };
  bool need = false;
  for (size_t k : sk) need = need || longest(L, j.left_keys[k]->bound_index) > 15 || longest(R, j.right_keys[k]->bound_index) > 15;
// ... 257 lines not shown
      HIP_CHECK(hipMemsetAsync(counter(kCntOverflow), 0, 8, stream()));
    }
    cx.launch(v, "k_jpscat", (int)g, prm, 1024);
    cx.launch(v, "k_jtbuild", (int)np, prm);
    cx.join_bucket_tables_++;
    if (mono) cx.join_mono_tables_++;
    return true;
  }

  void build_chained() {
    const bool chained = table == JoinTable::Lds || table == JoinTable::Chained;
    int64_t cap = 1024;
    if (chained) {
      while (cap < 2 * st.entries) cap <<= 1;
      head.ensure((size_t)cap * 4);
      next.ensure((size_t)std::max<int64_t>(B.rows, 1) * 4 + 16);
      HIP_CHECK(hipMemsetAsync(head.p, 0xff, (size_t)cap * 4, stream()));
    }
    nbtiles = (B.rows + 1023) / 1024;
    if (v.desc.join_outer_build) {
      matched.ensure((size_t)std::max<int64_t>(B.rows, 1));
      btiles.ensure((size_t)(nbtiles + 1) * 8);
      HIP_CHECK(hipMemsetAsync(matched.p, 0, (size_t)std::max<int64_t>(B.rows, 1), stream()));
      prm.out[kJoinOutMatched] = matched.p;
      prm.out[kJoinOutBuildTiles] = btiles.p;
      prm.iarg[kJoinArgBuildTiles] = nbtiles;
    }
    if (table != JoinTable::Bucket) {
      int ib = 1;
      while (ib < 31 && ((int64_t)1 << ib) - 1 < std::max<int64_t>(B.rows, 1)) ib++;
      if (((int64_t)1 << ib) - 1 < B.rows) throw CometError("HashJoin: build sides of 2^31 rows or more are not supported");
      chained_table_args(prm, cap, ib);
    }
    if (chained) {
      prm.out[kJoinOutTable] = head.p;
      prm.out[kJoinOutRows] = next.p;
    }
    prm.out[kOutErr] = cx.err_flags_.p;
    cx.timed_begin();
    if (table == JoinTable::Chained && B.rows) cx.launch(v, "k_jbuild", build_grid(), prm);
    prm.out[kJoinOutCounters] = counters.p;
  }

  void maybe_sample_keymap() {
    if (table == JoinTable::BitmapOnly || table == JoinTable::Direct || keymap_built) return;
    if (!(st.keymap_range && set.keymap != 0 && n >= (1 << 20) && (set.keymap == 1 || n >= 4 * B.rows))) return;
    bool wanted = set.keymap == 1;
    if (!wanted) {
      HIP_CHECK(hipMemsetAsync(counters.p, 0, 16, stream()));
      const int64_t ns = 8192;
      sample_args(prm, ns);
      cx.launch(v, table == JoinTable::Bucket ? "k_jsample_b" : "k_jsample", (int)((ns + 255) / 256), prm);
      uint64_t cnt[2] = {0, 0};
      cx.read_small(cnt, counters.p, sizeof cnt);
      wanted = cnt[0] >= 64 && cnt[1] * 2 < cnt[0];
    }
    if (wanted) build_keymap(false);
  }

  void bind_outputs(int64_t rows_cap) {
    const PipelineDesc& d = v.desc;
    for (size_t c = 0; c < d.out_cols.size(); c++) {
      if (!vals[c]) vals[c] = std::make_shared<DevBuf>();
      vals[c]->ensure((size_t)std::max<int64_t>(rows_cap, 1) * out_width(d.out_cols[c]) + 16);
      prm.out[kOutFirstCol + 2 * c] = vals[c]->p;
      if (!vbytes[c]) vbytes[c] = std::make_shared<DevBuf>();
      if (d.out_cols[c].nullable) {
        vbytes[c]->ensure((size_t)std::max<int64_t>(rows_cap, 1) + 16);
        prm.out[kOutFirstCol + 2 * c + 1] = vbytes[c]->p;
      }
    }
  }

  bool probe() {
    const PipelineDesc& d = v.desc;
    int64_t out_cap = d.join_build_only ? 1 : n + 1024;
    for (int attempt = 0; n > 0; attempt++) {
      bind_outputs(out_cap);
      probe_args(prm, out_cap);
      HIP_CHECK(hipMemsetAsync(counter(kCntEmitted), 0, 8, stream()));
      const int64_t ptiles = (n + 4095) / 4096;
      cx.launch(v, probe_kernel(table, keymap_built), (int)std::min<int64_t>(ptiles, table == JoinTable::Lds ? 256 * 3 : 256 * 8), prm);
      uint64_t words[8] = {0, 0, 0, 0, 0, 0, 0, 0};
      cx.read_small(words, counters.p, sizeof words);
      if (table == JoinTable::Bucket && words[kCntOverflow]) {
        cx.timed_end();
        HIP_CHECK(hipStreamSynchronize(stream()));
        cx.join_bucket_tables_--;
        return false;
      }
      out_rows = d.join_build_only ? 0 : (int64_t)words[kCntEmitted];
      if (out_rows <= out_cap) break;
      if (attempt == 1) throw CometError("internal: hash join output exceeded its exact size");
      out_cap = out_rows;
    }
    probe_capacity = n > 0 ? out_cap : 0;
    return true;
  }

  void outer_tail() {
    const PipelineDesc& d = v.desc;
    const size_t ncol = d.out_cols.size();
    if (d.join_outer_build && B.rows > 0) {
      cx.launch(v, "k_jbcount", (int)std::min<int64_t>(nbtiles, 256 * 8), prm);
      cx.launch(v, "k_jbscan", 1, prm);
      uint64_t total = 0;
      cx.read_small(&total, (char*)btiles.p + (size_t)nbtiles * 8, 8);
      tail_rows = (int64_t)total;
      prm.iarg[kJoinArgTailBase] = out_rows;
    }
    const int64_t all_rows = out_rows + tail_rows;
    if (all_rows > probe_capacity || (ncol > 0 && !vals[0])) {
      std::vector<std::shared_ptr<DevBuf>> ov = vals, ob = vbytes;
      for (size_t c = 0; c < ncol; c++) { vals[c].reset(); vbytes[c].reset(); }
      bind_outputs(all_rows);
      for (size_t c = 0; c < ncol && out_rows > 0; c++) {
        HIP_CHECK(hipMemcpyAsync(vals[c]->p, ov[c]->p, (size_t)out_rows * out_width(d.out_cols[c]), hipMemcpyDeviceToDevice, stream()));
        if (d.out_cols[c].nullable) HIP_CHECK(hipMemcpyAsync(vbytes[c]->p, ob[c]->p, (size_t)out_rows, hipMemcpyDeviceToDevice, stream()));
      }
      HIP_CHECK(hipStreamSynchronize(stream()));
    }
    if (tail_rows > 0) cx.launch(v, "k_jbemit", (int)std::min<int64_t>(nbtiles, 256 * 8), prm);
    cx.timed_end();
    out_rows = all_rows;
  }

  DevTable finish() {
    const int nbuild = (int)B.cols.size();
    DevTable out = cx.outputs_to_table(v, vals, vbytes, out_rows, [&](int c) { return c < nbuild ? std::make_pair(&B, c) : std::make_pair(&P, c - nbuild); });
    if (fused_probe || fused_build) cx.check_device_errors();
    if (tail_rows > 0 || n == 0) HIP_CHECK(hipStreamSynchronize(stream()));
    out.owners.push_back(v.mod);
    cx.join_build_rows_ += B.rows;
    cx.join_probe_rows_ += P.rows;
    return out;
  }

  bool run() {
    plan();
    const bool use_lds = B.rows > 0 && B.rows <= 6144;
    bool bucket = !use_lds && allow_bucket && set.bucket_min_rows >= 0 && B.rows >= set.bucket_min_rows;
    if (!use_lds && B.rows >= (bucket ? 65536 : (1 << 20))) count_build();
    table = use_lds ? JoinTable::Lds : JoinTable::Chained;
    if (st.keymap_range != 0 && v.desc.join_dedup_build && set.bitmap_only != 0 && n > 0) {
      build_keymap(false);
      table = JoinTable::BitmapOnly;
      cx.join_bitmap_only_++;
    } else if (st.keymap_range && set.direct != 0 && st.entries == st.keyed_rows) {
      if (try_direct()) table = JoinTable::Direct;
    }
    if (bucket && table == JoinTable::Chained && B.rows != 0 && build_bucket()) table = JoinTable::Bucket;
    vals.resize(v.desc.out_cols.size());
    vbytes.resize(v.desc.out_cols.size());
    build_chained();
    maybe_sample_keymap();
    if (!probe()) return false;
    outer_tail();
    return true;
  }
};

DevTable ExecutionContext::hash_join_impl(const Operator& node, const Operator& j, const DevTable& L, const DevTable& R, const std::string& key_suffix,
                                          const JoinFusion* fused_probe, const JoinFusion* fused_build) {
  for (bool allow_bucket : {true, false}) {
    HashJoinRun run(*this, node, j, L, R, key_suffix, fused_probe, fused_build, allow_bucket);
    if (run.run()) return run.finish();
  }
  throw CometError("internal: a hash join without a bucket table reported a bucket overflow");
}

}
```

### datafusion-comet_amd/csrc/exec_pipeline.cpp

```cpp
#include "exec_internal.hpp"

namespace comet {
void ExecutionContext::process_chunk(const std::vector<DeviceColumnView>& cols, const std::vector<bool>& has_valid, int64_t n) {
  if (n == 0) return;
  std::vector<int> fixed_lens(cols.size(), -1);
  for (size_t i = 0; i < cols.size(); i++) fixed_lens[i] = cols[i].fixed_len;
  Variant& v = variant_for(has_valid, fixed_lens);
  const PipelineDesc& d = v.desc;
  if (d.max_rows_exact && input_rows + n > d.max_rows_exact)
    throw CometError("decimal or integer sum over more rows than its static no-overflow proof allows (" + std::to_string(d.max_rows_exact) + ")");
  CometKParams prm;
  memset(&prm, 0, sizeof prm);
  prm.n = n;
  bind_inputs(prm, cols, has_valid);
  err_flags_.ensure(kErrBytes);
  prm.out[kOutErr] = err_flags_.p;
  if (!has_join_) input_rows += n;
  if (d.sink == SinkKind::AggNoGroup || d.sink == SinkKind::AggGrouped) {
    prm.iarg[kRowBaseArg] = agg_rows_seen_;
    agg_rows_seen_ += n;
  }

  if (d.sink == SinkKind::AggNoGroup) {
    if (agg_variant_ && agg_variant_->desc.NW != d.NW) throw CometError("internal: accumulator layout differs between variants");
    agg_variant_ = &v;
    const int64_t tile = (int64_t)d.R * 256;
    int grid = (int)std::min<int64_t>((n + tile - 1) / tile, 256 * 8);
    size_t need = (size_t)(n_partials_ + grid) * d.NW * 8;
    if (need > partials_.cap) {
      DevBuf bigger;
      bigger.ensure(std::max(need * 2, (size_t)(4096 * d.NW * 8)));
      if (n_partials_) HIP_CHECK(hipMemcpyAsync(bigger.p, partials_.p, (size_t)n_partials_ * d.NW * 8, hipMemcpyDeviceToDevice, stream_));
      HIP_CHECK(hipStreamSynchronize(stream_));
      std::swap(partials_.p, bigger.p);
      std::swap(partials_.cap, bigger.cap);
    }
    prm.out[kOutPartials] = (char*)partials_.p + (size_t)n_partials_ * d.NW * 8;
    for (int attempt = 0;; attempt++) {
      prm.iarg[kFixScaleArg] = packed_fix_scales(d), prm.iarg[kFixScaleArg2] = packed_fix_scales(d, 4);
      timed_begin();
      launch(v, "k_agg", grid, prm);
      timed_end();
      if (d.fix_sums.empty()) break;
      uint64_t aux[2 + 2 * kFixMaxSums];
      read_small(aux, err_flags_.p, sizeof aux);
      std::vector<int> shift;
      if (attempt >= 3 || !adjust_fix_scales(d, aux + 2, shift)) break;
      for (size_t f = 0; f < shift.size(); f++)
        if (shift[f] > 0 && n_partials_ > 0 &&
            comet_launch_fix_rescale((uint64_t*)partials_.p, n_partials_, d.NW, d.fix_sums[f].word, shift[f], stream_) != 0)
          throw CometError("float sum rescale: launch failed");
    }
    fix_has_state_ = fix_has_state_ || !d.fix_sums.empty();
    n_partials_ += grid;
    return;
  }

  if (d.sink == SinkKind::AggGrouped) {
    if (agg_variant_ && (agg_variant_->desc.NW != d.NW || agg_variant_->desc.NK != d.NK))
      throw CometError("internal: group slot layout differs between variants");
    agg_variant_ = &v;
    if (try_partitioned_merge(v, prm, n)) return;
    const size_t slot_bytes = 8 + 8 * (size_t)(d.NK + d.NW);
    auto alloc_table = [&](DevBuf& buf, int64_t cap) {
      buf.ensure((size_t)cap * slot_bytes);
      HIP_CHECK(hipMemsetAsync(buf.p, 0, (size_t)cap * slot_bytes, stream_));
    };
    if (group_cap_ == 0) {
      int64_t want = 1 << 16;
      if (d.merges_states) {
        while (want < 2 * n && want < ((int64_t)1 << 26)) want <<= 1;
      } else if (n <= ((int64_t)1 << 24)) {
        while (want < 2 * n && want < ((int64_t)1 << 22)) want <<= 1;
      }
      group_cap_ = want;
      alloc_table(group_table_, group_cap_);
      group_table_clear_ = true;
      HIP_CHECK(hipMemsetAsync((char*)err_flags_.p + 8, 0, 8, stream_));
    }
    const int64_t tile = (int64_t)d.R * 256;
    int grid_mult = 4;
    if (const char* e = getenv("COMET_GROUPED_GRID_MULT")) grid_mult = std::max(1, atoi(e));
    int grid = (int)std::min<int64_t>((n + tile - 1) / tile, 256 * grid_mult);
    const int64_t per_block_cap = ((int64_t)1 << 19) - 2 * tile;
    grid = (int)std::max<int64_t>(grid, (n + per_block_cap - 1) / per_block_cap);
    while (true) {
      const bool clear = group_table_clear_;
      if (!clear) {
        group_backup_.ensure((size_t)group_cap_ * slot_bytes);
        HIP_CHECK(hipMemcpyAsync(group_backup_.p, group_table_.p, (size_t)group_cap_ * slot_bytes, hipMemcpyDeviceToDevice, stream_));
      }
      prm.out[0] = group_table_.p;
      prm.iarg[0] = group_cap_;
      prm.iarg[kFixScaleArg] = packed_fix_scales(d), prm.iarg[kFixScaleArg2] = packed_fix_scales(d, 4);
      timed_begin();
      launch(v, "k_gagg", grid, prm);
      timed_end();
      uint64_t head[2 + (kErrBytes - 16) / 8];
      uint32_t flags[4];
      read_small(head, err_flags_.p, d.fix_sums.empty() ? 16 : sizeof head);
      memcpy(flags, head, 16);
      uint64_t groups_now;
      memcpy(&groups_now, &flags[2], 8);
      const bool full = (flags[0] & 32u) != 0;
      if (!full && !d.fix_sums.empty() && fix_attempts_ < 3) {
        std::vector<int> shift;
        if (adjust_fix_scales(d, head + 2, shift)) {
          fix_attempts_++;
          if (clear) HIP_CHECK(hipMemsetAsync(group_table_.p, 0, (size_t)group_cap_ * slot_bytes, stream_));
          else HIP_CHECK(hipMemcpyAsync(group_table_.p, group_backup_.p, (size_t)group_cap_ * slot_bytes, hipMemcpyDeviceToDevice, stream_));
          uint32_t restore[4] = {flags[0], flags[1], 0, 0};
          memcpy(&restore[2], &groups_committed_, 8);
          write_small(err_flags_.p, restore, 16);
          for (size_t f = 0; f < shift.size(); f++)
            if (shift[f] > 0 && comet_launch_fix_rescale((uint64_t*)group_table_.p, group_cap_, (int64_t)(slot_bytes / 8), 1 + d.NK + d.fix_sums[f].word, shift[f], stream_) != 0)
              throw CometError("float sum rescale: launch failed");
          continue;
        }
      }
      if (!full && (int64_t)groups_now * 2 <= group_cap_) { groups_committed_ = groups_now; group_table_clear_ = false; break; }
      int64_t new_cap = group_cap_ * 8;
      if (full) {
        int64_t need = 1 << 16;
        while (need < 2 * n && need < ((int64_t)1 << 28)) need <<= 1;
        new_cap = std::max(new_cap, std::min(group_cap_ * 64, need));
      }
      if (new_cap > ((int64_t)1 << 28)) throw CometError("group table would exceed 2^28 slots");
      DevBuf bigger;
      alloc_table(bigger, new_cap);
      uint32_t zero4[4] = {flags[0] & ~32u, flags[1], 0, 0};
      write_small(err_flags_.p, zero4, 16);
      CometKParams rp;
      memset(&rp, 0, sizeof rp);
      rp.out[0] = bigger.p;
      rp.iarg[0] = new_cap;
      rp.out[2] = err_flags_.p;
      rp.out[3] = full ? group_backup_.p : group_table_.p;
      rp.iarg[1] = group_cap_;
      if (!(full && clear)) launch(v, "k_grehash", (int)std::min<int64_t>((group_cap_ + 255) / 256, 256 * 8), rp);
      HIP_CHECK(hipStreamSynchronize(stream_));
      std::swap(group_table_.p, bigger.p);
      std::swap(group_table_.cap, bigger.cap);
      group_cap_ = new_cap;
      if (!full) { groups_committed_ = groups_now; group_table_clear_ = false; break; }
    }
    fix_attempts_ = 0;
    fix_has_state_ = fix_has_state_ || !d.fix_sums.empty();
    if (std::find(d.kernels.begin(), d.kernels.end(), std::string("k_gpick")) != d.kernels.end()) {
      prm.out[0] = group_table_.p;
      prm.iarg[0] = group_cap_;
      timed_begin();
      launch(v, "k_gpick", (int)std::min<int64_t>((group_cap_ + 255) / 256, 256 * 8), prm);
      timed_end();
    }
    return;
  }

  if (d.sink == SinkKind::Output) {
    for (auto& oc : d.out_cols)
      if (oc.gather_src >= 0 || oc.view_src >= 0 || oc.fmt_kind || !oc.concat_cols.empty()) throw CometError("internal: gathered Utf8 outputs must go through the materialising path");
    const size_t ncol = d.out_cols.size();
    int64_t out_rows = n;
    if (out_vals_.size() < ncol) {
      out_vals_.resize(ncol);
      out_valid_.resize(ncol);
      for (size_t j = 0; j < ncol; j++) {
        if (!out_vals_[j]) out_vals_[j].reset(new DevBuf());
        if (!out_valid_[j]) out_valid_[j].reset(new DevBuf());
      }
    }
    auto bind_outputs = [&](int64_t rows_cap) {
      for (size_t j = 0; j < ncol; j++) {
        int w = d.out_cols[j].type.id == TypeId::Bool ? 1 : fixed_width(d.out_cols[j].type);
        out_vals_[j]->ensure((size_t)rows_cap * w + 16);
        prm.out[kOutFirstCol + 2 * j] = out_vals_[j]->p;
        if (d.out_cols[j].nullable) {
          out_valid_[j]->ensure((size_t)rows_cap + 16);
          prm.out[kOutFirstCol + 2 * j + 1] = out_valid_[j]->p;
        }
      }
    };
    timed_begin();
    if (d.has_filter) {
      bind_outputs(n);
      out_rows = launch_fused_filter(v, prm, n);
    } else {
      bind_outputs(n);
      int grid = (int)std::min<int64_t>((n + 255) / 256, 256 * 8);
      launch(v, "k_emit", grid, prm);
    }
    timed_end();
    check_device_errors();
    if (out_rows == 0) return;
    std::vector<std::vector<uint8_t>> hv(ncol), hk(ncol);
    for (size_t j = 0; j < ncol; j++) {
      int w = d.out_cols[j].type.id == TypeId::Bool ? 1 : fixed_width(d.out_cols[j].type);
      hv[j].resize((size_t)out_rows * w);
      HIP_CHECK(hipMemcpyAsync(hv[j].data(), out_vals_[j]->p, hv[j].size(), hipMemcpyDeviceToHost, stream_));
      if (d.out_cols[j].nullable) {
        hk[j].resize((size_t)out_rows);
        HIP_CHECK(hipMemcpyAsync(hk[j].data(), out_valid_[j]->p, hk[j].size(), hipMemcpyDeviceToHost, stream_));
      }
    }
    HIP_CHECK(hipStreamSynchronize(stream_));
    const int64_t bs = batch_size_ > 0 ? batch_size_ : out_rows;
    for (int64_t off = 0; off < out_rows; off += bs) {
      int64_t len = std::min(bs, out_rows - off);
      HostBatch b;
      b.rows = len;
      for (size_t j = 0; j < ncol; j++) {
        HostColumn c;
        c.type = d.out_cols[j].type;
        c.length = len;
        if (c.type.id == TypeId::Bool) {
          c.values.assign((size_t)((len + 7) / 8), 0);
          for (int64_t i = 0; i < len; i++)
            if (hv[j][(size_t)(off + i)]) c.values[(size_t)(i >> 3)] |= (uint8_t)(1u << (i & 7));
        } else {
          int w = fixed_width(c.type);
          c.values.assign(hv[j].begin() + (size_t)off * w, hv[j].begin() + (size_t)(off + len) * w);
        }
        if (d.out_cols[j].nullable) {
          int64_t nulls = 0;
          std::vector<uint8_t> bm((size_t)((len + 7) / 8), 0);
          for (int64_t i = 0; i < len; i++) {
            if (hk[j][(size_t)(off + i)]) bm[(size_t)(i >> 3)] |= (uint8_t)(1u << (i & 7));
            else nulls++;
          }
          c.null_count = nulls;
          if (nulls) c.validity = std::move(bm);
        }
        b.cols.push_back(std::move(c));
      }
      ready_.push_back(std::move(b));
    }
    return;
  }
  throw CometError("internal: unsupported sink");
}

void ExecutionContext::read_small(void* dst, const void* dev_src, size_t n) {
  if (n > 4096) throw CometError("internal: read_small of " + std::to_string(n) + " bytes (its staging holds 4096)");
  small_host_.ensure(4096);
  HIP_CHECK(hipMemcpyAsync(small_host_.p, dev_src, n, hipMemcpyDeviceToHost, stream_));
  HIP_CHECK(hipStreamSynchronize(stream_));
  memcpy(dst, small_host_.p, n);
}
void ExecutionContext::write_small(void* dev_dst, const void* src, size_t n) {
  if (n > 2048) throw CometError("internal: write_small of " + std::to_string(n) + " bytes (its staging holds 2048)");
  small_host_.ensure(4096);
  if (n <= 128) {
    if (small_write_slot_ == 16) {
      HIP_CHECK(hipStreamSynchronize(stream_));
      small_write_slot_ = 0;
    }
    char* slot = (char*)small_host_.p + 2048 + 128 * (size_t)small_write_slot_++;
    memcpy(slot, src, n);
    HIP_CHECK(hipMemcpyAsync(dev_dst, slot, n, hipMemcpyHostToDevice, stream_));
    return;
  }
  HIP_CHECK(hipStreamSynchronize(stream_));
  small_write_slot_ = 0;
  memcpy((char*)small_host_.p + 2048, src, n);
  HIP_CHECK(hipMemcpyAsync(dev_dst, (char*)small_host_.p + 2048, n, hipMemcpyHostToDevice, stream_));
  small_write_slot_ = 16;
}

void ExecutionContext::timed_begin() {
  hipEvent_t a = pool_get_event(device_id_), b = pool_get_event(device_id_);
  timed_.emplace_back(a, b);
  HIP_CHECK(hipEventRecord(a, stream_));
}
void ExecutionContext::timed_end() { HIP_CHECK(hipEventRecord(timed_.back().second, stream_)); }
void ExecutionContext::collect_timings() {
  for (; timed_done_ < timed_.size(); timed_done_++) {
    float ms = 0;
    if (hipEventElapsedTime(&ms, timed_[timed_done_].first, timed_[timed_done_].second) == hipSuccess) {
      last_kernel_ms += ms;
      last_kernel_launches++;
    }
  }
}

void ExecutionContext::check_device_errors() {
  if (!err_flags_.p) return;
  uint32_t flags[4] = {0, 0, 0, 0};
  read_small(flags, err_flags_.p, 16);
  collect_timings();
  raise_device_errors(flags[0]);
}

void ExecutionContext::raise_device_errors(uint32_t f) {
  if (!f) return;
  {
    uint64_t detail[4 + kErrDetailStrBytes / 8];
    memset(detail, 0, sizeof detail);
    read_small(detail, (const char*)err_flags_.p + 8 * kErrDetailWord, sizeof detail);
    ErrSite site;
    if (detail[0] != 0 && lookup_err_site((uint32_t)(detail[0] - 1), site)) {
      throw CometError(err_site_json(site, detail[1], detail[2], (const uint8_t*)(detail + 4), (size_t)kErrDetailStrBytes, site_context((uint32_t)(detail[0] - 1))), 1);
    }
  }
  if (f & 1u) throw CometError("{\"errorType\":\"ArithmeticOverflow\",\"errorClass\":\"ARITHMETIC_OVERFLOW\",\"params\":{\"fromType\":\"decimal\"}}", 1);
  if (f & 2u) throw CometError("{\"errorType\":\"ArithmeticOverflow\",\"errorClass\":\"ARITHMETIC_OVERFLOW\",\"params\":{\"fromType\":\"integer\"}}", 1);
  if (f & 4u) throw CometError("{\"errorType\":\"CastOverFlow\",\"errorClass\":\"CAST_OVERFLOW\",\"params\":{}}", 1);
  if (f & 8u) throw CometError("{\"errorType\":\"NumericValueOutOfRange\",\"errorClass\":\"NUMERIC_VALUE_OUT_OF_RANGE.WITH_SUGGESTION\",\"params\":{}}", 1);
  if (f & 512u) throw CometError("{\"errorType\":\"CastInvalidValue\",\"errorClass\":\"CAST_INVALID_INPUT\",\"params\":{\"fromType\":\"STRING\"}}", 1);
  if (f & 1024u) throw CometError("{\"errorType\":\"InvalidInputInCastToDatetime\",\"errorClass\":\"CAST_INVALID_INPUT\",\"params\":{\"fromType\":\"STRING\",\"toType\":\"DATE\"}}", 1);
  if (f & 8192u) throw CometError("{\"errorType\":\"InvalidInputInCastToDatetime\",\"errorClass\":\"CAST_INVALID_INPUT\",\"params\":{\"fromType\":\"STRING\",\"toType\":\"TIMESTAMP\"}}", 1);
  if (f & 16384u) throw CometError("{\"errorType\":\"InvalidInputInCastToDatetime\",\"errorClass\":\"CAST_INVALID_INPUT\",\"params\":{\"fromType\":\"STRING\",\"toType\":\"TIMESTAMP_NTZ\"}}", 1);
  if (f & 4096u) throw CometError("a string cast to a timestamp names a time zone inside the value, or holds a time of day without a date (which takes the current date): not supported by the MI355X native engine");
  if (f & 2048u) throw CometError("a timestamp lies behind the end of its time zone's table (the year 2400): not supported by the MI355X native engine");
  if (f & 262144u) throw CometError("Arrow error: Compute error: long overflow");
  if (f & 256u) throw CometError("{\"errorType\":\"DivideByZero\",\"errorClass\":\"DIVIDE_BY_ZERO\",\"params\":{}}", 1);
  if (f & (65536u | 131072u)) {
    const int kind = (f & 65536u) ? 0 : 1;
    throw CometError(decimal_sum_overflow_json(kind, agg_ctx_[kind].get()), 1);
  }
  if (f & 32768u) throw CometError("{\"errorType\":\"RemainderByZero\",\"errorClass\":\"REMAINDER_BY_ZERO\",\"params\":{}}", 1);
  if (f & 64u) throw CometError("Utf8 group keys longer than 15 bytes are not supported by the GPU hash aggregate yet");
  if (f & 16u)
    throw CometError("decimal or ANSI/TRY integer sum overflow cannot be decided order-independently for this input (mixed signs beyond the type's bound); "
                     "exact sequential evaluation is not implemented");
  throw CometError("device error flags " + std::to_string(f));
}

bool ExecutionContext::try_partitioned_merge(Variant& v, CometKParams& prm, int64_t n) {
  const PipelineDesc& d = v.desc;
  static const int64_t min_rows = getenv("COMET_AGG_PARTITIONED_MIN_ROWS") ? atoll(getenv("COMET_AGG_PARTITIONED_MIN_ROWS")) : 32768;
  static const int64_t max_rows_any = getenv("COMET_AGG_PARTITIONED_MAX_ROWS") ? atoll(getenv("COMET_AGG_PARTITIONED_MAX_ROWS")) : ((int64_t)1 << 22);
  if (!single_chunk_hint_ || group_cap_ != 0 || part_result_ready_ || !d.fix_sums.empty() || !dict_id_col_.empty() || min_rows < 0 || n < min_rows) return false;
  if (!d.merges_states && n > max_rows_any) return false;
  if (std::find(d.kernels.begin(), d.kernels.end(), std::string("k_gpmerge")) == d.kernels.end()) return false;
  const int slot_bytes = 8 + 8 * (d.NK + d.NW);
  const int64_t cap = slot_bytes <= 48 ? 1024 : slot_bytes <= 96 ? 512 : slot_bytes <= 192 ? 256 : 128;
  constexpr int64_t kMaxP = 16384;
  const int64_t np = (n + cap / 2 - 1) / (cap / 2);
  if (np > kMaxP) return false;
  const int64_t tile = (int64_t)d.R * 256;
  const int64_t g = std::max<int64_t>(1, std::min<int64_t>(1024, (n + 4 * tile - 1) / (4 * tile)));
  const int64_t chunk = ((n + g - 1) / g + tile - 1) / tile * tile;
  const int64_t rec_words = d.NK + d.NW;
  DevBuf recs, part;
  recs.ensure((size_t)n * (size_t)rec_words * 8 + 16);
  part.ensure((size_t)(2 * kMaxP + 16 + g * np) * 4 + 16);
  const size_t ncol = d.out_cols.size();
  std::vector<std::shared_ptr<DevBuf>> vals(ncol), vbytes(ncol);
  for (size_t j = 0; j < ncol; j++) {
    vals[j] = std::make_shared<DevBuf>();
    vbytes[j] = std::make_shared<DevBuf>();
    vals[j]->ensure((size_t)n * out_width(d.out_cols[j]) + 16);
    vbytes[j]->ensure((size_t)n + 16);
    HIP_CHECK(hipMemsetAsync(vbytes[j]->p, 1, (size_t)n, stream_));
    prm.out[kOutFirstCol + 2 * j] = vals[j]->p;
    prm.out[kOutFirstCol + 2 * j + 1] = vbytes[j]->p;
  }
  HIP_CHECK(hipMemsetAsync((char*)err_flags_.p + 8, 0, 8, stream_));
  prm.out[1] = recs.p;
  prm.out[3] = part.p;
  prm.iarg[2] = np;
  prm.iarg[5] = chunk;
  prm.iarg[kFixScaleArg] = packed_fix_scales(d), prm.iarg[kFixScaleArg2] = packed_fix_scales(d, 4);
  timed_begin();
  launch(v, "k_gphist", (int)g, prm);
  uint64_t* skew_flag = (uint64_t*)((char*)err_flags_.p + kErrBytes - 8);
  HIP_CHECK(hipMemsetAsync(skew_flag, 0, 8, stream_));
  if (comet_launch_join_part_scan((uint32_t*)part.p + (2 * kMaxP + 16), (int)g, (int)np, (uint32_t*)part.p + (kMaxP + 16), d.merges_states ? 0xffffffffu : (uint32_t)(4 * cap), skew_flag,
                                  stream_) != 0)
    throw CometError("partitioned aggregate: launch failed");
  if (!d.merges_states) {
    uint64_t skew = 0;
    read_small(&skew, skew_flag, 8);
    if (skew) {
      timed_end();
      return false;
    }
  }
  launch(v, "k_gpscat", (int)g, prm);
  launch(v, "k_gpmerge", (int)std::min<int64_t>(np, 256 * 16), prm);
  timed_end();
  uint32_t hdr[4] = {0, 0, 0, 0};
  read_small(hdr, err_flags_.p, 16);
  if (hdr[0] & 32u) {
    uint32_t reset[4] = {hdr[0] & ~32u, hdr[1], 0, 0};
    write_small(err_flags_.p, reset, 16);
    HIP_CHECK(hipStreamSynchronize(stream_));
    return false;
  }
  collect_timings();
  raise_device_errors(hdr[0]);
  uint64_t ngroups = 0;
  memcpy(&ngroups, hdr + 2, 8);
  GatherSource gs = nullptr;
  part_result_ = outputs_to_table(v, vals, vbytes, (int64_t)ngroups, gs);
  part_result_.owners.push_back(v.mod);
  part_result_ready_ = true;
  part_merges_++;
  groups_committed_ = ngroups;
  return true;
}

void ExecutionContext::finish_aggregate() {
  std::vector<bool> none(in_types_.size(), false);
  Variant& v = agg_variant_ ? *agg_variant_ : variant_for(none, std::vector<int>(in_types_.size(), -1));
  const PipelineDesc& d = v.desc;
  CometKParams prm;
  memset(&prm, 0, sizeof prm);
  partials_.ensure(64);
  const size_t ncol = d.out_cols.size();
  const size_t block_bytes = kErrBytes + ncol * 32;
  if (err_flags_.cap < block_bytes) {
    DevBuf bigger;
    bigger.ensure(block_bytes);
    HIP_CHECK(hipMemcpyAsync(bigger.p, err_flags_.p, kErrBytes, hipMemcpyDeviceToDevice, stream_));
    HIP_CHECK(hipStreamSynchronize(stream_));
    std::swap(err_flags_.p, bigger.p);
    std::swap(err_flags_.cap, bigger.cap);
  }
  prm.out[kOutPartials] = partials_.p;
  prm.out[kOutErr] = err_flags_.p;
  prm.iarg[0] = n_partials_;
  char* base = (char*)err_flags_.p + kErrBytes;
  HIP_CHECK(hipMemsetAsync(base, 1, ncol * 32, stream_));
  for (size_t j = 0; j < ncol; j++) {
    prm.out[kOutFirstCol + 2 * j] = base + j * 32;
    prm.out[kOutFirstCol + 2 * j + 1] = base + j * 32 + 16;
  }
  prm.iarg[kFixScaleArg] = packed_fix_scales(d), prm.iarg[kFixScaleArg2] = packed_fix_scales(d, 4);
  launch(v, "k_agg_final", 1, prm);
  result_host_.ensure(block_bytes);
  HIP_CHECK(hipMemcpyAsync(result_host_.p, err_flags_.p, block_bytes, hipMemcpyDeviceToHost, stream_));
  HIP_CHECK(hipStreamSynchronize(stream_));
  collect_timings();
  raise_device_errors(((const uint32_t*)result_host_.p)[0]);
  const uint8_t* hb = (const uint8_t*)result_host_.p + kErrBytes;
  HostBatch b;
  b.rows = 1;
  for (size_t j = 0; j < ncol; j++) {
    HostColumn c;
    c.type = d.out_cols[j].type;
    c.length = 1;
    const uint8_t* val = hb + j * 32;
    if (c.type.id == TypeId::Bool) {
      c.values.assign(1, val[0] ? 1 : 0);
    } else {
      int w = fixed_width(c.type);
      c.values.assign(val, val + w);
    }
    if (d.out_cols[j].nullable && val[16] == 0) {
      c.null_count = 1;
      c.validity.assign(1, 0);
    }
    b.cols.push_back(std::move(c));
  }
  ready_.push_back(std::move(b));
}

DevTable ExecutionContext::grouped_to_device() {
  if (part_result_ready_) {
    part_result_ready_ = false;
    return std::move(part_result_);
  }
  DevTable empty;
  if (!agg_variant_) {
    std::vector<bool> none(in_types_.size(), false);
    auto pv = planned_variant(*plan_, plan_hash_, none, false, has_join_ ? &in_types_ : nullptr);
    for (auto& oc : pv->desc.out_cols) {
      empty.types.push_back(oc.type);
      empty.cols.push_back(DeviceColumnView());
      empty.has_valid.push_back(false);
    }
    return empty;
  }
  Variant& v = *agg_variant_;
  const PipelineDesc& d = v.desc;
  uint64_t ngroups = 0;
  {
    uint32_t hdr[4] = {0, 0, 0, 0};
    read_small(hdr, err_flags_.p, 16);
    collect_timings();
    memcpy(&ngroups, hdr + 2, 8);
    raise_device_errors(hdr[0]);
  }
  if (getenv("COMET_TRACE_STAGES")) fprintf(stderr, "[comet] grouped result: %llu groups in a table of %lld slots x %zu bytes\n", (unsigned long long)ngroups, (long long)group_cap_, (size_t)(8 + 8 * (d.NK + d.NW)));
  const size_t ncol = d.out_cols.size();
  CometKParams prm;
  memset(&prm, 0, sizeof prm);
  prm.out[0] = group_table_.p;
  prm.iarg[0] = group_cap_;
  scratch_counts_.ensure(64);
  HIP_CHECK(hipMemsetAsync(scratch_counts_.p, 0, 8, stream_));
  prm.out[1] = scratch_counts_.p;
  prm.out[kOutErr] = err_flags_.p;
  std::vector<std::shared_ptr<DevBuf>> vals(ncol), vbytes(ncol);
  for (size_t j = 0; j < ncol; j++) {
    vals[j] = std::make_shared<DevBuf>();
    vbytes[j] = std::make_shared<DevBuf>();
    vals[j]->ensure((size_t)std::max<uint64_t>(ngroups, 1) * out_width(d.out_cols[j]) + 16);
    vbytes[j]->ensure((size_t)std::max<uint64_t>(ngroups, 1) + 16);
    HIP_CHECK(hipMemsetAsync(vbytes[j]->p, 1, (size_t)std::max<uint64_t>(ngroups, 1), stream_));
    prm.out[kOutFirstCol + 2 * j] = vals[j]->p;
    prm.out[kOutFirstCol + 2 * j + 1] = vbytes[j]->p;
  }
  prm.iarg[kFixScaleArg] = packed_fix_scales(d), prm.iarg[kFixScaleArg2] = packed_fix_scales(d, 4);
  if (ngroups) launch(v, "k_gemit", (int)std::min<int64_t>((group_cap_ + 255) / 256, 256 * 8), prm);
  GatherSource gs = nullptr;
  if (!dict_id_col_.empty()) gs = [this](int c) { return std::make_pair((const DevTable*)&dict_src_, c); };
  DevTable t = outputs_to_table(v, vals, vbytes, (int64_t)ngroups, gs);
  t.owners.push_back(v.mod);
  check_device_errors();
  return t;
}

void ExecutionContext::finish_grouped() {
  if (!agg_variant_) return;
  if (part_result_ready_) {
    DevTable t = grouped_to_device();
    table_to_host_batches(t);
    return;
  }
  Variant& v = *agg_variant_;
  const PipelineDesc& d = v.desc;
  uint64_t ngroups = 0;
  {
    uint32_t head[4] = {0, 0, 0, 0};
    read_small(head, err_flags_.p, 16);
    collect_timings();
    raise_device_errors(head[0]);
    memcpy(&ngroups, head + 2, 8);
  }
  if (ngroups == 0) return;
  if (!dict_id_col_.empty()) {
    DevTable t = grouped_to_device();
    table_to_host_batches(t);
    return;
  }
  const size_t ncol = d.out_cols.size();
  CometKParams prm;
  memset(&prm, 0, sizeof prm);
  prm.out[0] = group_table_.p;
  prm.iarg[0] = group_cap_;
  scratch_counts_.ensure(64);
  HIP_CHECK(hipMemsetAsync(scratch_counts_.p, 0, 8, stream_));
  prm.out[1] = scratch_counts_.p;
  prm.out[kOutErr] = err_flags_.p;
  std::vector<int> widths(ncol);
  std::vector<size_t> val_off(ncol);
  size_t arena = 0;
  for (size_t j = 0; j < ncol; j++) {
    const OutCol& oc = d.out_cols[j];
    widths[j] = oc.packed_string ? 16 : (oc.type.id == TypeId::Bool ? 1 : fixed_width(oc.type));
    val_off[j] = arena;
    arena += ((size_t)ngroups * (size_t)widths[j] + 15) & ~(size_t)15;
  }
  const size_t valid_base = arena, valid_stride = ((size_t)ngroups + 15) & ~(size_t)15;
  arena += valid_stride * ncol;
  emit_arena_.ensure(arena + 16);
  HIP_CHECK(hipMemsetAsync((char*)emit_arena_.p + valid_base, 1, valid_stride * ncol, stream_));
  for (size_t j = 0; j < ncol; j++) {
    prm.out[kOutFirstCol + 2 * j] = (char*)emit_arena_.p + val_off[j];
    prm.out[kOutFirstCol + 2 * j + 1] = (char*)emit_arena_.p + valid_base + j * valid_stride;
  }
  prm.iarg[kFixScaleArg] = packed_fix_scales(d), prm.iarg[kFixScaleArg2] = packed_fix_scales(d, 4);
  launch(v, "k_gemit", (int)std::min<int64_t>((group_cap_ + 255) / 256, 256 * 8), prm);
  struct HostSpan {
    const uint8_t* p = nullptr;
    size_t n = 0;
    const uint8_t* data() const { return p; }
    const uint8_t* begin() const { return p; }
    uint8_t operator[](size_t i) const { return p[i]; }
  };
  PinnedBuf host_arena;
  host_arena.ensure(arena + 16);
  HIP_CHECK(hipMemcpyAsync(host_arena.p, emit_arena_.p, arena, hipMemcpyDeviceToHost, stream_));
  std::vector<HostSpan> hv(ncol), hk(ncol);
  for (size_t j = 0; j < ncol; j++) {
    hv[j].p = (const uint8_t*)host_arena.p + val_off[j];
    hv[j].n = (size_t)ngroups * widths[j];
    hk[j].p = (const uint8_t*)host_arena.p + valid_base + j * valid_stride;
    hk[j].n = (size_t)ngroups;
  }
  HIP_CHECK(hipStreamSynchronize(stream_));
  check_device_errors();
  const int64_t total = (int64_t)ngroups;
  const int64_t bs = batch_size_ > 0 ? batch_size_ : total;
  for (int64_t off = 0; off < total; off += bs) {
    const int64_t len = std::min(bs, total - off);
    HostBatch b;
    b.rows = len;
    for (size_t j = 0; j < ncol; j++) {
      const OutCol& oc = d.out_cols[j];
      HostColumn c;
      c.type = oc.type;
      c.length = len;
      if (oc.packed_string) {
        c.values.resize((size_t)(len + 1) * 4);
        int32_t* offs = (int32_t*)c.values.data();
        offs[0] = 0;
        for (int64_t i = 0; i < len; i++) {
          uint64_t w[2];
          memcpy(w, hv[j].data() + (size_t)(off + i) * 16, 16);
          int slen = hk[j][(size_t)(off + i)] ? (int)(w[1] >> 56) : 0;
          for (int k = 0; k < slen; k++) c.data.push_back((uint8_t)(k < 8 ? (w[0] >> (8 * k)) : (w[1] >> (8 * (k - 8)))));
          offs[i + 1] = (int32_t)c.data.size();
        }
      } else if (c.type.id == TypeId::Bool) {
        c.values.assign((size_t)((len + 7) / 8), 0);
        for (int64_t i = 0; i < len; i++)
          if (hv[j][(size_t)(off + i)]) c.values[(size_t)(i >> 3)] |= (uint8_t)(1u << (i & 7));
      } else {
        int w = widths[j];
        c.values.assign(hv[j].begin() + (size_t)off * w, hv[j].begin() + (size_t)(off + len) * w);
      }
      if (oc.nullable) {
        const uint8_t* vb = hk[j].data() + off;
        int64_t valid = 0;
        for (int64_t i = 0; i < len; i++) valid += vb[i] != 0;
        c.null_count = len - valid;
        if (c.null_count) {
          std::vector<uint8_t> bm((size_t)((len + 7) / 8), 0);
          for (int64_t i = 0; i < len; i++)
            if (vb[i]) bm[(size_t)(i >> 3)] |= (uint8_t)(1u << (i & 7));
          c.validity = std::move(bm);
        }
      }
      b.cols.push_back(std::move(c));
    }
    ready_.push_back(std::move(b));
  }
}

long long ExecutionContext::packed_fix_scales(const PipelineDesc& d, int first) {
  if (fix_scales_.size() != d.fix_sums.size()) fix_scales_.assign(d.fix_sums.size(), kFixDefaultScale);
  uint64_t p = 0;
  for (size_t f = (size_t)first; f < fix_scales_.size() && f < (size_t)first + 4; f++) p |= (uint64_t)(uint16_t)(int16_t)fix_scales_[f] << (16 * (f - (size_t)first));
  return (long long)p;
}

bool ExecutionContext::adjust_fix_scales(const PipelineDesc& d, const uint64_t* aux, std::vector<int>& shift_right) {
  bool rerun = false;
  shift_right.assign(d.fix_sums.size(), 0);
  for (size_t f = 0; f < d.fix_sums.size(); f++) {
    const uint64_t hi = aux[d.fix_sums[f].aux_hi], lo = aux[d.fix_sums[f].aux_lo];
    if (hi == 0) continue;
    const int top = (int)hi - 1200, low = 1200 - (int)lo, s = fix_scales_[f];
    int target = s;
    if (top > s + kFixW) target = top + 10 - kFixW;
    else if (low < s && !fix_has_state_) target = fix_scale_for_range(top, low, kFixW);
    if (target < kFixScaleFloor) target = kFixScaleFloor;
    if (target == s) continue;
    if (target > s && fix_has_state_) shift_right[f] = target - s;
    fix_scales_[f] = target;
    rerun = true;
  }
  return rerun;
}

int64_t ExecutionContext::launch_fused_filter(Variant& v, CometKParams& prm, int64_t n) {
  const int64_t tile_rows = 256 * (int64_t)v.desc.R;
  const int64_t ntiles = (n + tile_rows - 1) / tile_rows;
  scratch_mask_.ensure((size_t)ntiles * 8 + 64);
  scratch_counts_.ensure(64);
  HIP_CHECK(hipMemsetAsync(scratch_mask_.p, 0, (size_t)ntiles * 8, stream_));
  HIP_CHECK(hipMemsetAsync(scratch_counts_.p, 0, 16, stream_));
  prm.out[0] = scratch_mask_.p;
  prm.out[1] = scratch_counts_.p;
  launch(v, "k_filter", (int)std::min<int64_t>(ntiles, 256 * 8), prm);
  uint64_t total = 0;
  read_small(&total, (char*)scratch_counts_.p + 8, 8);
  return (int64_t)total;
}

}
```

### datafusion-comet_amd/csrc/exec_shuffle.cpp

```cpp
#include "exec_internal.hpp"

namespace comet {
DevTable ExecutionContext::write_shuffle(const Operator& sw) {
  static const bool trace = getenv("COMET_TRACE_STAGES") != nullptr;
  Timer tm;
  double t_last = 0;
  auto lap = [&](const char* what) {
    if (!trace) return;
    const double now = tm.ns() / 1e6;
    fprintf(stderr, "[comet] shuffle write: %s %.3f ms\n", what, now - t_last);
    t_last = now;
  };
  auto sp = shuffle_projs_.find(&sw);
  const Operator& child = sp != shuffle_projs_.end() ? *sp->second : *sw.children[0];
  DevTable in = materialize(child);
  const int64_t n = in.rows;
  lap("child");
  const int P = sw.shuffle_partitioning == Operator::Partitioning::Single ? 1 : sw.shuffle_num_partitions;
  size_t n_payload = in.cols.size();
  std::vector<int> key_cols;
  {
    size_t appended = 0;
    for (auto& e : sw.shuffle_hash_exprs) appended += e->kind != ExprKind::Bound;
    for (auto& k : sw.shuffle_sort_orders) appended += k.child->kind != ExprKind::Bound;
// ... 4 lines not shown
    for (auto& e : sw.shuffle_hash_exprs) key_cols.push_back(e->kind == ExprKind::Bound ? e->bound_index : (int)next++);
  } else if (sw.shuffle_partitioning == Operator::Partitioning::RoundRobin) {
    const size_t k = sw.shuffle_max_hash_columns <= 0 ? n_payload : std::min<size_t>((size_t)sw.shuffle_max_hash_columns, n_payload);
    for (size_t i = 0; i < k; i++)
      if (!in.types[i].is_nested()) key_cols.push_back((int)i);
  }
  if (n >= (int64_t)1 << 32) throw CometError("ShuffleWriter: more than 2^32 rows in one task are not supported (u32 row indices, multi_partition.rs)");
  std::vector<int64_t> starts((size_t)P + 1, 0);
  starts[(size_t)P] = n;
  DevTable grouped;
  if (P > 1 && n > 0) {
    DevBuf hashes, pids, dstarts, hist;
    auto ridx = std::make_shared<DevBuf>();
    hashes.ensure((size_t)n * 4);
    pids.ensure((size_t)n * 4);
    ridx->ensure((size_t)n * 4 + 16);
    dstarts.ensure(((size_t)P + 1) * 8);
    const bool by_range = sw.shuffle_partitioning == Operator::Partitioning::Range;
    std::shared_ptr<DevBuf> planes;
    DevBuf bkeys;
    if (by_range) {
      int W = 0, Wb = 0;
      const int B = (int)sw.shuffle_bounds.size();
      std::vector<DType> btypes;
      for (auto& k : range_sort_.at(&sw)->sort_orders) btypes.push_back(k.child->dtype);
      DevTable bt = literal_table(sw.shuffle_bounds, btypes);
      std::vector<int64_t> lr, lb;
      {
        int w0 = 0;
        (void)sort_key_planes(*range_sort_.at(&sw), in, w0, &lr, true);
        if (B > 0) (void)sort_key_planes(*range_bsort_.at(&sw), bt, w0, &lb, true);
        for (size_t s = 0; s < lr.size(); s++) lr[s] = std::max<int64_t>(lr[s], s < lb.size() ? lb[s] : 0);
        lb = lr;
      }
      planes = sort_key_planes(*range_sort_.at(&sw), in, W, &lr);
      std::vector<uint8_t> rowmajor((size_t)std::max(B, 1) * (size_t)std::max(W, 1), 0);
      if (B > 0) {
        auto bplanes = sort_key_planes(*range_bsort_.at(&sw), bt, Wb, &lb);
        if (Wb != W) throw CometError("internal: range boundary keys and row keys differ in width");
        std::vector<uint8_t> pl((size_t)W * (size_t)B);
        HIP_CHECK(hipMemcpyAsync(pl.data(), bplanes->p, pl.size(), hipMemcpyDeviceToHost, stream_));
        HIP_CHECK(hipStreamSynchronize(stream_));
        for (int b = 0; b < B; b++)
          for (int p = 0; p < W; p++) rowmajor[(size_t)b * W + p] = pl[(size_t)p * B + b];
        for (int b = 1; b < B; b++)
          if (memcmp(&rowmajor[(size_t)(b - 1) * W], &rowmajor[(size_t)b * W], (size_t)W) > 0) throw CometError("ShuffleWriter: range boundaries are not in ascending order");
      }
      bkeys.ensure(rowmajor.size() + 16);
      HIP_CHECK(hipMemcpyAsync(bkeys.p, rowmajor.data(), rowmajor.size(), hipMemcpyHostToDevice, stream_));
      if (comet_launch_range_partition_ids((const uint8_t*)planes->p, n, W, (const uint8_t*)bkeys.p, B, (int32_t*)pids.p, stream_) != 0)
        throw CometError("shuffle: launch failed");
      HIP_CHECK(hipStreamSynchronize(stream_));
    }
    const uint32_t seed = 42;
    if (!by_range && comet_launch_fill(4, hashes.p, n, &seed, stream_) != 0) throw CometError("shuffle: launch failed");
    for (int c : key_cols) {
      const DeviceColumnView& v = in.cols[(size_t)c];
      if (v.offset != 0) throw CometError("ShuffleWriter: hash key column with a non-zero Arrow offset is not supported yet");
      if (comet_launch_murmur3((int)in.types[(size_t)c].id, in.types[(size_t)c].precision, v.data, in.has_valid[(size_t)c] ? v.valid : nullptr, v.aux, n,
                               (uint32_t*)hashes.p, stream_) != 0)
        throw CometError("ShuffleWriter: cannot hash a column of type " + in.types[(size_t)c].str());
    }
    const int64_t W = comet_partition_tiles(n);
    const size_t hist_bytes = ((size_t)P * (size_t)W + 1) * 8;
    hist.ensure((size_t)comet_partition_scratch_bytes(n, P));
    uint32_t* bad = (uint32_t*)((char*)hist.p + hist_bytes);
    HIP_CHECK(hipMemsetAsync(bad, 0, 4, stream_));
    if ((!by_range && comet_launch_pmod((const uint32_t*)hashes.p, n, P, (int32_t*)pids.p, stream_) != 0) ||
        comet_launch_partition_indices((const int32_t*)pids.p, n, P, (uint64_t*)hist.p, bad, (int64_t*)dstarts.p, (uint32_t*)ridx->p, stream_) != 0)
      throw CometError("shuffle: launch failed");
    HIP_CHECK(hipMemcpyAsync(starts.data(), dstarts.p, ((size_t)P + 1) * 8, hipMemcpyDeviceToHost, stream_));
    HIP_CHECK(hipStreamSynchronize(stream_));
    DevTable payload = in;
    payload.types.resize(n_payload);
    payload.cols.resize(n_payload);
    payload.has_valid.resize(n_payload);
    grouped = take_rows(payload, (const uint32_t*)ridx->p, 0, n, ridx);
  } else {
    grouped = in;
    grouped.types.resize(n_payload);
    grouped.cols.resize(n_payload);
    grouped.has_valid.resize(n_payload);
  }
  HIP_CHECK(hipStreamSynchronize(stream_));
  check_device_errors();
  shuffle_repart_ns_ += tm.ns();
  lap("partition (murmur3, pmod, indices, takes)");

  const int64_t bs = batch_size_ > 0 ? batch_size_ : std::max<int64_t>(n, 1);
  const ShuffleCodec codec = (ShuffleCodec)sw.shuffle_codec;
  size_t staging_bytes = (size_t)256 << 20;
  for (auto& kv : config_)
    if (kv.first == "spark.comet.gpu.shuffle.stagingBytes") staging_bytes = (size_t)std::max<long long>(1 << 16, atoll(kv.second.c_str()));
  if (const char* e = getenv("COMET_SHUFFLE_STAGING_BYTES")) staging_bytes = (size_t)std::max<long long>(1 << 16, atoll(e));
  size_t row_bytes = 0;
  std::vector<char> is_str(n_payload, 0);
  std::vector<HostColumn> nested_host(n_payload);
  std::vector<ColumnSlice> nested_slice(n_payload);
  std::function<void(const HostColumn&, ColumnSlice&)> slice_of = [&](const HostColumn& h, ColumnSlice& c) {
    c.type = h.type;
    c.validity = h.validity.empty() ? nullptr : h.validity.data();
    c.values = h.values.empty() ? nullptr : h.values.data();
    c.data = h.data.empty() ? nullptr : h.data.data();
    c.first = 0;
    c.kids.resize(h.children.size());
    for (size_t k = 0; k < h.children.size(); k++) slice_of(h.children[k], c.kids[k]);
  };
  for (size_t j = 0; j < n_payload; j++) {
    if (!grouped.types[j].is_nested()) continue;
    nested_host[j] = download_column(grouped.cols[j], grouped.types[j], grouped.has_valid[j], n, stream_);
    slice_of(nested_host[j], nested_slice[j]);
    row_bytes += 32;
  }
  for (size_t j = 0; j < n_payload; j++) {
    const DType& ty = grouped.types[j];
    const DeviceColumnView& v = grouped.cols[j];
    if (ty.is_nested()) continue;
    if (n > 0 && v.offset != 0) throw CometError("ShuffleWriter: input column with a non-zero Arrow offset is not supported yet");
    is_str[j] = ty.id == TypeId::String || ty.id == TypeId::Bytes;
    if (is_str[j]) {
      int32_t ends[2] = {0, 0};
      if (n > 0) {
        read_small(&ends[0], v.data, 4);
        read_small(&ends[1], (const char*)v.data + (size_t)n * 4, 4);
        if (ends[0] != 0) throw CometError("ShuffleWriter: Utf8 column whose offsets do not start at 0");
      }
      row_bytes += 4 + (n > 0 ? (size_t)(ends[1] / n) + 1 : 0);
    } else {
      row_bytes += ty.id == TypeId::Bool ? 1 : (size_t)fixed_width(ty);
    }
    if (grouped.has_valid[j]) row_bytes += 1;
  }
  const double write_t0 = tm.ns();
  struct BlockTask { int p; int64_t first, rows; };
  std::vector<BlockTask> tasks;
  for (int p = 0; p < P; p++)
    for (int64_t r = starts[(size_t)p]; r < starts[(size_t)p + 1]; r += bs) tasks.push_back({p, r, std::min(bs, starts[(size_t)p + 1] - r)});
  struct Run {
    size_t first = 0, last = 0;
    std::vector<uint8_t> bytes;
    std::vector<size_t> block_size;
    std::string error;
    bool done = false;
    double encode_ms = 0;
  };
  struct Slab {
    size_t run0 = 0, run1 = 0;
    int64_t base = 0, end = 0;
  };
  std::vector<Run> runs;
  std::vector<Slab> slabs;
  {
    const size_t rb = std::max<size_t>(row_bytes, 1);
    const size_t run_target = std::min<size_t>((size_t)4 << 20, std::max<size_t>(staging_bytes / 64, (size_t)64 << 10));
    size_t slab_acc = 0;
    for (size_t t = 0; t < tasks.size();) {
      size_t e = t, acc = 0;
      while (e < tasks.size() && acc < run_target) acc += (size_t)tasks[e++].rows * rb;
      Run r;
      r.first = t;
      r.last = e;
      if (slabs.empty() || slab_acc + acc > staging_bytes) {
        Slab sl;
        sl.run0 = runs.size();
        sl.base = tasks[t].first & ~(int64_t)7;
        slabs.push_back(sl);
        slab_acc = 0;
      }
// ... 205 lines not shown
```

### datafusion-comet_amd/csrc/exec_window.cpp

```cpp
#include "exec_internal.hpp"

namespace comet {
u128 detail::pow10_u128_host(int p) {
  u128 r = 1;
  for (int i = 0; i < p; i++) r *= 10;
  return r;
}

DevTable ExecutionContext::window(const Operator& w, const DevTable& in) {
  const int64_t n = in.rows;
  if (n >= ((int64_t)1 << 31)) throw CometError("Window: more than 2^31 rows in one partition of the plan");
  DevTable out = in;
  auto add_col = [&](const DType& t, std::shared_ptr<DevBuf> data, std::shared_ptr<DevBuf> valid_bits, std::shared_ptr<DevBuf> aux = nullptr) {
    DeviceColumnView v;
    v.data = data ? data->p : nullptr;
    v.valid = valid_bits ? (const uint8_t*)valid_bits->p : nullptr;
    v.aux = aux ? aux->p : nullptr;
    out.types.push_back(t);
    out.cols.push_back(v);
    out.has_valid.push_back(valid_bits != nullptr);
    if (data) out.owners.push_back(data);
    if (valid_bits) out.owners.push_back(valid_bits);
    if (aux) out.owners.push_back(aux);
  };
// ... 247 lines not shown
          HIP_CHECK(hipMemsetAsync(zero_bits.p, 0, (size_t)((n + 7) / 8), stream_));
          vb = (const uint8_t*)zero_bits.p;
        }
        const bool split = c >= 0 && in.types[(size_t)c].id == TypeId::Decimal && in.types[(size_t)c].precision > 18;
        if (split) {
          wide_hi.ensure((size_t)n * 16 + 16);
          SH = std::make_shared<DevBuf>();
          SH->ensure((size_t)n * 16 + 16);
        }
        if (comet_launch_window_widen(width, src, vb, n, wide.p, split ? wide_hi.p : nullptr, (uint32_t*)okf.p, stream_) != 0 ||
            comet_launch_scan128(wide.p, n, t128.p, S->p, stream_) != 0 || (split && comet_launch_scan128(wide_hi.p, n, t128.p, SH->p, stream_) != 0))
          throw CometError("window: launch failed");
        pq_launch_u32_scan((const uint32_t*)okf.p, n, (uint64_t*)t32.p, (int32_t*)C->p, stream_);
        HIP_CHECK(hipStreamSynchronize(stream_));
        it = prefix.emplace(c, Prefix{S, SH, C}).first;
      }
      const DType at = c >= 0 ? in.types[(size_t)c] : arg->dtype;
      int fnk = a.kind == AggKind::Count ? 2 : a.kind == AggKind::Avg ? 3 : (at.id == TypeId::Decimal ? 0 : 1);
      const DType rt = fnk == 2 || fnk == 1 ? DType::of(TypeId::Int64) : a.dtype;
      const DType sum_t = fnk == 3 ? a.sum_dtype : a.dtype;
      u128 bound = fnk == 0 || fnk == 3 ? pow10_u128_host(sum_t.precision) - 1 : 0, avg_bound = fnk == 3 ? pow10_u128_host(a.dtype.precision) - 1 : 0;
      i128 scaler = fnk == 3 ? (i128)pow10_u128_host(std::max(0, a.dtype.scale - sum_t.scale)) : 1;
      auto data = std::make_shared<DevBuf>(), okb = std::make_shared<DevBuf>(), bits = std::make_shared<DevBuf>();
      data->ensure((size_t)n * (fnk == 0 || fnk == 3 ? 16 : 8) + 16);
      okb->ensure((size_t)n + 16);
      bits->ensure((size_t)((n + 7) / 8) + 16);
      if (comet_launch_window_agg(fnk, lo_kind, lo_off, hi_kind, hi_off, it->second.S->p, it->second.SH ? it->second.SH->p : nullptr, (const int32_t*)it->second.C->p, (const int32_t*)sp->p, (const int32_t*)sg->p,
                                  (const uint32_t*)first_part->p, (const uint32_t*)first_peer->p, n, &bound, &scaler, &avg_bound, data->p, (uint8_t*)okb->p, stream_) != 0)
        throw CometError("window: launch failed");
      pq_launch_pack((const uint8_t*)okb->p, (uint8_t*)bits->p, n, stream_);
      add_col(rt, data, fnk == 2 ? nullptr : bits);
      if (fnk == 2) out.owners.push_back(bits);
      out.owners.push_back(okb);
      continue;
    }
    const std::string& f = fn.func;
    int kind = f == "row_number" ? 0 : f == "rank" ? 1 : f == "dense_rank" ? 2 : f == "percent_rank" ? 3 : f == "cume_dist" ? 4 : f == "ntile" ? 5 : -1;
    if (kind >= 0) {
      const bool dbl = kind == 3 || kind == 4;
      auto data = std::make_shared<DevBuf>();
      data->ensure((size_t)n * (dbl ? 8 : 4) + 16);
      if (comet_launch_window_rank(kind, kind == 5 ? fn.args[0]->lit_i64 : 0, (const int32_t*)sp->p, (const int32_t*)sg->p, (const uint32_t*)first_part->p,
                                   (const uint32_t*)first_peer->p, n, data->p, stream_) != 0)
        throw CometError("window: launch failed");
      add_col(DType::of(dbl ? TypeId::Double : TypeId::Int32), data, nullptr);
      continue;
    }
    if (f == "nth_value") {
      int lo_kind, hi_kind;
      int64_t lo_off, hi_off;
      frame_of(fn, lo_kind, hi_kind, lo_off, hi_off);
      pick_and_gather(fn.args[0]->bound_index, 2, fn.args[1]->lit_i64, fn.ignore_nulls, lo_kind, lo_off, hi_kind, hi_off);
      continue;
    }
    const int c = fn.args[0]->bound_index;
    const int64_t k = fn.args.size() >= 2 ? fn.args[1]->lit_i64 : 1;
    const int64_t shift = f == "lag" ? -k : k;
    if (in.cols[(size_t)c].offset != 0) throw CometError(f + " over a column with a non-zero Arrow offset is not supported yet");
    DevBuf ok;
    auto idx = std::make_shared<DevBuf>();
    idx->ensure((size_t)n * 4 + 16);
    ok.ensure((size_t)n + 16);
    const Expr* dflt = fn.args.size() == 3 && !fn.args[2]->lit_null ? fn.args[2].get() : nullptr;
    if (fn.ignore_nulls && in.has_valid[(size_t)c] && k != 0) {
      DevBuf flags, t32, counts;
      flags.ensure((size_t)n * 4 + 16);
      counts.ensure((size_t)(n + 2) * 4);
      t32.ensure((size_t)((n + 1023) / 1024 + 2) * 8);
      if (comet_launch_window_valid_flags(in.cols[(size_t)c].valid, n, (uint32_t*)flags.p, stream_) != 0) throw CometError("window: launch failed");
      pq_launch_u32_scan((const uint32_t*)flags.p, n, (uint64_t*)t32.p, (int32_t*)counts.p, stream_);
      const bool backwards = (f == "lag") == (k > 0);
      if (comet_launch_window_pick(backwards ? 3 : 4, k > 0 ? k : -k, 0, 0, 0, 0, (const int32_t*)counts.p, (const int32_t*)sp->p, (const int32_t*)sg->p, (const uint32_t*)first_part->p,
                                   (const uint32_t*)first_peer->p, n, (uint32_t*)idx->p, (uint8_t*)ok.p, stream_) != 0)
        throw CometError("window: launch failed");
      gather_rows(c, idx, ok, dflt);
      HIP_CHECK(hipStreamSynchronize(stream_));
      continue;
    }
    if (comet_launch_window_offset(shift, (const int32_t*)sp->p, (const uint32_t*)first_part->p, n, (uint32_t*)idx->p, (uint8_t*)ok.p, stream_) != 0) throw CometError("window: launch failed");
    gather_rows(c, idx, ok, dflt);
    HIP_CHECK(hipStreamSynchronize(stream_));
  }
  timed_end();
  HIP_CHECK(hipStreamSynchronize(stream_));
  check_device_errors();
  return out;
}

DevTable ExecutionContext::expand(const Operator& ex, const DevTable& in) {
  const ExpandInfo& info = expand_info_.at(&ex);
  const size_t ncol = info.out_cols.size(), P = info.parts.size();
  const int64_t n = in.rows, total = n * (int64_t)P;
  if (total >= ((int64_t)1 << 32)) throw CometError("Expand: more than 2^32 output rows in one partition");
  Variant u;
  u.desc.out_cols = info.out_cols;
  std::vector<std::shared_ptr<DevBuf>> vals(ncol), vbytes(ncol);
  for (size_t c = 0; c < ncol; c++) {
    vals[c] = std::make_shared<DevBuf>();
    vbytes[c] = std::make_shared<DevBuf>();
    vals[c]->ensure((size_t)std::max<int64_t>(total, 1) * (size_t)out_width(info.out_cols[c]) + 16);
    vbytes[c]->ensure((size_t)std::max<int64_t>(total, 1) + 16);
    HIP_CHECK(hipMemsetAsync(vbytes[c]->p, 1, (size_t)std::max<int64_t>(total, 1), stream_));
  }
  timed_begin();
  for (size_t p = 0; p < P; p++) {
    const ExpandPart& part = info.parts[p];
    const int64_t base = (int64_t)p * n;
    if (!part.proj->project_list.empty()) {
      auto pv = planned_variant(*part.proj, plan_hash_ ^ (0x9E3779B97F4A7C15ull * (uint64_t)(node_id_[part.proj.get()] + 1)), in.has_valid, true, &in.types);
      Variant v;
      v.desc = pv->desc;
      note_sites(v.desc);
      v.mod = jit_load(pv->code);
      if (!u.mod) u.mod = v.mod;
      CometKParams prm;
      memset(&prm, 0, sizeof prm);
      prm.n = n;
      bind_inputs(prm, in.cols, in.has_valid);
      prm.out[kOutErr] = err_flags_.p;
      for (size_t k = 0; k < part.out_col.size(); k++) {
        const size_t c = (size_t)part.out_col[k];
        prm.out[kOutFirstCol + 2 * k] = (char*)vals[c]->p + (size_t)base * (size_t)out_width(info.out_cols[c]);
        prm.out[kOutFirstCol + 2 * k + 1] = (char*)vbytes[c]->p + (size_t)base;
      }
      if (n) launch(v, "k_emit", (int)std::min<int64_t>((n + 255) / 256, 256 * 8), prm);
      u.desc.kernels = v.desc.kernels;
      HIP_CHECK(hipStreamSynchronize(stream_));
    }
    for (int c : part.null_cols) {
      if (!n) continue;
      HIP_CHECK(hipMemsetAsync((char*)vbytes[(size_t)c]->p + (size_t)base, 0, (size_t)n, stream_));
      HIP_CHECK(hipMemsetAsync((char*)vals[(size_t)c]->p + (size_t)base * (size_t)out_width(info.out_cols[(size_t)c]), 0,
                               (size_t)n * (size_t)out_width(info.out_cols[(size_t)c]), stream_));
    }
  }
  timed_end();
  if (!u.mod) throw CometError("Expand: every projection consists of NULL literals only");
  DevTable out = outputs_to_table(u, vals, vbytes, total, [&](int c) { return std::make_pair(&in, c); });
  out.owners.push_back(u.mod);
  HIP_CHECK(hipStreamSynchronize(stream_));
  check_device_errors();
  return out;
}

}
```

### datafusion-comet_amd/csrc/kernels_static.hip

```cpp
#include <hip/hip_runtime.h>

#include "device/comet_device.hpp"

using namespace comet;

template <class F>
__global__ __launch_bounds__(256) void mm3_kernel(const void* values, const u8* validity, i64 n, u32* hashes, F f) {
  for (i64 i = (i64)blockIdx.x * 256 + threadIdx.x; i < n; i += (i64)gridDim.x * 256) {
    if (validity && !((validity[i >> 3] >> (i & 7)) & 1)) continue;
    hashes[i] = f(values, i, hashes[i]);
  }
}

struct HashBool { __device__ u32 operator()(const void* v, i64 i, u32 s) const { return mm3_hash_i32((((const u8*)v)[i >> 3] >> (i & 7)) & 1, s); } };
struct HashI8 { __device__ u32 operator()(const void* v, i64 i, u32 s) const { return mm3_hash_i32((i32)((const i8*)v)[i], s); } };
struct HashI16 { __device__ u32 operator()(const void* v, i64 i, u32 s) const { return mm3_hash_i32((i32)((const i16*)v)[i], s); } };
struct HashI32 { __device__ u32 operator()(const void* v, i64 i, u32 s) const { return mm3_hash_i32(((const i32*)v)[i], s); } };
struct HashI64 { __device__ u32 operator()(const void* v, i64 i, u32 s) const { return mm3_hash_i64(((const i64*)v)[i], s); } };
struct HashF32 { __device__ u32 operator()(const void* v, i64 i, u32 s) const { return mm3_hash_f32(((const float*)v)[i], s); } };
struct HashF64 { __device__ u32 operator()(const void* v, i64 i, u32 s) const { return mm3_hash_f64(((const double*)v)[i], s); } };
struct HashDecSmall { __device__ u32 operator()(const void* v, i64 i, u32 s) const { return mm3_hash_i64(((const i64*)v)[2 * i], s); } };
struct HashDecWide { __device__ u32 operator()(const void* v, i64 i, u32 s) const { return mm3_hash_i128(((const i128*)v)[i], s); } };
struct HashUtf8 {
  const u8* bytes;
  __device__ u32 operator()(const void* v, i64 i, u32 s) const {
    const i32* off = (const i32*)v;
    return mm3_hash_bytes(bytes + off[i], off[i + 1] - off[i], s);
  }
};

__global__ __launch_bounds__(256) void pmod_kernel(const u32* hashes, i64 n, i32 np, i32* out) {
  for (i64 i = (i64)blockIdx.x * 256 + threadIdx.x; i < n; i += (i64)gridDim.x * 256) out[i] = pmod(hashes[i], np);
}

__global__ __launch_bounds__(256) void utf8_uniform_kernel(const i32* off, i64 n, i32 L, u32* flag) {
  bool bad = false;
  const i32 o0 = off[0];
  const i64 total = n + 1;
  i64 head = 0;
  while (head < total && ((((uintptr_t)(off + head)) & 15) != 0)) head++;
  const int4* v4 = (const int4*)(off + head);
  const i64 ngroups = (total - head) / 4;
  constexpr int U = 4;
  for (i64 g0 = ((i64)blockIdx.x * 256 + threadIdx.x) * U; g0 < ngroups; g0 += (i64)gridDim.x * 256 * U) {
    int4 v[U];
#pragma unroll
    for (int u = 0; u < U; u++) v[u] = g0 + u < ngroups ? v4[g0 + u] : make_int4(0, 0, 0, 0);
#pragma unroll
    for (int u = 0; u < U; u++) {
      if (g0 + u < ngroups) {
        const i64 i = head + 4 * (g0 + u);
        const i32 e = o0 + (i32)(i * L);
        bad |= (v[u].x != e) | (v[u].y != e + L) | (v[u].z != e + 2 * L) | (v[u].w != e + 3 * L);
      }
    }
  }
  if (blockIdx.x == 0) {
    for (i64 i = threadIdx.x; i < head; i += 256) bad |= off[i] != o0 + (i32)(i * L);
    for (i64 i = head + ngroups * 4 + threadIdx.x; i < total; i += 256) bad |= off[i] != o0 + (i32)(i * L);
  }
  if (__any(bad) && lane_id() == 0) atomicOr(flag, 1u);
}

__device__ __forceinline__ i64 dict_index(const void* idx, int iw, i64 i) {
  switch (iw) {
    case 1: return ((const i8*)idx)[i];
    case 2: return ((const i16*)idx)[i];
    case 4: return ((const i32*)idx)[i];
    default: return ((const i64*)idx)[i];
  }
}
__global__ __launch_bounds__(256) void dict_gather_fixed_kernel(const void* idx, int iw, const u8* idx_valid, const u8* dict, const u8* dict_valid,
                                                                int width, i64 n, u8* out, u8* out_valid_bytes) {
  for (i64 i = (i64)blockIdx.x * 256 + threadIdx.x; i < n; i += (i64)gridDim.x * 256) {
    bool ok = !idx_valid || ((idx_valid[i >> 3] >> (i & 7)) & 1);
    i64 k = ok ? dict_index(idx, iw, i) : 0;
    if (ok && dict_valid) ok = (dict_valid[k >> 3] >> (k & 7)) & 1;
    for (int b = 0; b < width; b++) out[i * width + b] = ok ? dict[k * width + b] : 0;
    out_valid_bytes[i] = ok ? 1 : 0;
  }
}
__global__ __launch_bounds__(256) void dict_gather_str_len_kernel(const void* idx, int iw, const u8* idx_valid, const i32* dict_offs, const u8* dict_valid,
                                                                  i64 n, u32* lengths, u8* out_valid_bytes) {
  for (i64 i = (i64)blockIdx.x * 256 + threadIdx.x; i < n; i += (i64)gridDim.x * 256) {
    bool ok = !idx_valid || ((idx_valid[i >> 3] >> (i & 7)) & 1);
    i64 k = ok ? dict_index(idx, iw, i) : 0;
    if (ok && dict_valid) ok = (dict_valid[k >> 3] >> (k & 7)) & 1;
    lengths[i] = ok ? (u32)(dict_offs[k + 1] - dict_offs[k]) : 0;
    out_valid_bytes[i] = ok ? 1 : 0;
  }
}
__global__ __launch_bounds__(256) void dict_gather_str_copy_kernel(const void* idx, int iw, const u8* valid_bytes, const i32* dict_offs, const u8* dict_bytes,
                                                                   i64 n, const i32* out_offs, u8* out_bytes) {
  for (i64 i = (i64)blockIdx.x * 256 + threadIdx.x; i < n; i += (i64)gridDim.x * 256) {
    if (!valid_bytes[i]) continue;
    i64 k = dict_index(idx, iw, i);
    const u8* src = dict_bytes + dict_offs[k];
    i32 len = dict_offs[k + 1] - dict_offs[k];
    u8* dst = out_bytes + out_offs[i];
    for (i32 b = 0; b < len; b++) dst[b] = src[b];
  }
}

static int grid_for(i64 n) {
  i64 g = (n + 255) / 256;
  return (int)(g < 1 ? 1 : (g > 256 * 8 ? 256 * 8 : g));
}

extern "C" int comet_launch_murmur3(int type_id, int precision, const void* values, const uint8_t* validity, const void* aux,
                                    int64_t n, uint32_t* hashes, void* stream) {
  hipStream_t st = (hipStream_t)stream;
  if (n <= 0) return 0;
  int g = grid_for(n);
  switch (type_id) {
    case 0: hipLaunchKernelGGL(mm3_kernel<HashBool>, g, 256, 0, st, values, validity, (i64)n, hashes, HashBool()); break;
    case 1: hipLaunchKernelGGL(mm3_kernel<HashI8>, g, 256, 0, st, values, validity, (i64)n, hashes, HashI8()); break;
    case 2: hipLaunchKernelGGL(mm3_kernel<HashI16>, g, 256, 0, st, values, validity, (i64)n, hashes, HashI16()); break;
    case 3: case 12: hipLaunchKernelGGL(mm3_kernel<HashI32>, g, 256, 0, st, values, validity, (i64)n, hashes, HashI32()); break;
    case 4: case 9: case 11: hipLaunchKernelGGL(mm3_kernel<HashI64>, g, 256, 0, st, values, validity, (i64)n, hashes, HashI64()); break;
    case 5: hipLaunchKernelGGL(mm3_kernel<HashF32>, g, 256, 0, st, values, validity, (i64)n, hashes, HashF32()); break;
    case 6: hipLaunchKernelGGL(mm3_kernel<HashF64>, g, 256, 0, st, values, validity, (i64)n, hashes, HashF64()); break;
    case 7: case 8: {
      HashUtf8 h;
      h.bytes = (const u8*)aux;
      hipLaunchKernelGGL(mm3_kernel<HashUtf8>, g, 256, 0, st, values, validity, (i64)n, hashes, h);
      break;
    }
    case 10:
      if (precision <= 18) hipLaunchKernelGGL(mm3_kernel<HashDecSmall>, g, 256, 0, st, values, validity, (i64)n, hashes, HashDecSmall());
      else hipLaunchKernelGGL(mm3_kernel<HashDecWide>, g, 256, 0, st, values, validity, (i64)n, hashes, HashDecWide());
      break;
    default: return -1;
  }
  return hipGetLastError() == hipSuccess ? 0 : -1;
}

__global__ __launch_bounds__(256) void fix_rescale_kernel(u64* base, i64 count, i64 stride, i32 word_off, i32 shift) {
  for (i64 i = (i64)blockIdx.x * 256 + threadIdx.x; i < count; i += (i64)gridDim.x * 256) {
    u64* t = base + i * stride + word_off;
    const u64 w[3] = {t[0], t[1], t[2]};
    const u64 sign = (w[2] >> 63) ? ~0ull : 0ull;
    u64 r[3];
    const int ws = shift >> 6, bs = shift & 63;
#pragma unroll
    for (int k = 0; k < 3; k++) {
      const u64 lo = k + ws < 3 ? w[k + ws] : sign;
      const u64 hi = k + ws + 1 < 3 ? w[k + ws + 1] : sign;
      r[k] = bs ? (lo >> bs) | (hi << (64 - bs)) : lo;
    }
    t[0] = r[0]; t[1] = r[1]; t[2] = r[2];
  }
}
extern "C" int comet_launch_fix_rescale(uint64_t* base, int64_t count, int64_t stride_words, int32_t word_off, int32_t shift, void* stream) {
  if (count <= 0 || shift <= 0) return 0;
  hipLaunchKernelGGL(fix_rescale_kernel, grid_for(count), 256, 0, (hipStream_t)stream, (u64*)base, (i64)count, (i64)stride_words, word_off, shift > 191 ? 191 : shift);
  return hipGetLastError() == hipSuccess ? 0 : 1;
}

template <class T>
__global__ __launch_bounds__(256) void calib_read_kernel(const T* p, i64 n, u64* sink) {
  u64 acc = 0;
  for (i64 i = (i64)blockIdx.x * 256 + threadIdx.x; i < n; i += (i64)gridDim.x * 256) {
    const T v = p[i];
    const u32* w = (const u32*)&v;
#pragma unroll
    for (int k = 0; k < (int)(sizeof(T) / 4); k++) acc += w[k];
  }
  if (acc == 0x123456789abcdefull) *sink = acc;
}
struct CalibB16 { u32 w[4]; };
__global__ __launch_bounds__(256) void calib_read_lo8_kernel(const u64* p, i64 n, u64* sink) {
  u64 acc = 0;
  for (i64 i = (i64)blockIdx.x * 256 + threadIdx.x; i < n; i += (i64)gridDim.x * 256) acc += p[2 * i];
  if (acc == 0x123456789abcdefull) *sink = acc;
}
extern "C" int comet_calib_read(const void* p, int64_t n_bytes, int32_t lane_bytes, uint64_t* sink, void* stream) {
  hipStream_t st = (hipStream_t)stream;
  const int grid = 256 * 8;
  if (lane_bytes == 4) hipLaunchKernelGGL(calib_read_kernel<u32>, grid, 256, 0, st, (const u32*)p, (i64)(n_bytes / 4), (u64*)sink);
  else if (lane_bytes == 8) hipLaunchKernelGGL(calib_read_kernel<u64>, grid, 256, 0, st, (const u64*)p, (i64)(n_bytes / 8), (u64*)sink);
  else if (lane_bytes == 16) hipLaunchKernelGGL(calib_read_kernel<CalibB16>, grid, 256, 0, st, (const CalibB16*)p, (i64)(n_bytes / 16), (u64*)sink);
  else if (lane_bytes == 816) hipLaunchKernelGGL(calib_read_lo8_kernel, grid, 256, 0, st, (const u64*)p, (i64)(n_bytes / 16), (u64*)sink);
  else return -1;
  return hipGetLastError() == hipSuccess ? 0 : -1;
}

extern "C" int comet_launch_utf8_uniform(const int32_t* offsets, int64_t n, int32_t L, uint32_t* flag, void* stream) {
  if (n <= 0) return 0;
  hipLaunchKernelGGL(utf8_uniform_kernel, grid_for(n), 256, 0, (hipStream_t)stream, offsets, (i64)n, L, flag);
  return hipGetLastError() == hipSuccess ? 0 : -1;
}

extern "C" int comet_launch_dict_gather_fixed(const void* idx, int iw, const uint8_t* idx_valid, const uint8_t* dict, const uint8_t* dict_valid,
                                              int width, int64_t n, uint8_t* out, uint8_t* out_valid_bytes, void* stream) {
  if (n <= 0) return 0;
  hipLaunchKernelGGL(dict_gather_fixed_kernel, grid_for(n), 256, 0, (hipStream_t)stream, idx, iw, idx_valid, dict, dict_valid, width, (i64)n, out, out_valid_bytes);
  return hipGetLastError() == hipSuccess ? 0 : -1;
}
extern "C" int comet_launch_dict_gather_str_len(const void* idx, int iw, const uint8_t* idx_valid, const int32_t* dict_offs, const uint8_t* dict_valid,
                                                int64_t n, uint32_t* lengths, uint8_t* out_valid_bytes, void* stream) {
  if (n <= 0) return 0;
  hipLaunchKernelGGL(dict_gather_str_len_kernel, grid_for(n), 256, 0, (hipStream_t)stream, idx, iw, idx_valid, dict_offs, dict_valid, (i64)n, lengths, out_valid_bytes);
  return hipGetLastError() == hipSuccess ? 0 : -1;
}
extern "C" int comet_launch_dict_gather_str_copy(const void* idx, int iw, const uint8_t* valid_bytes, const int32_t* dict_offs, const uint8_t* dict_bytes,
                                                 int64_t n, const int32_t* out_offs, uint8_t* out_bytes, void* stream) {
  if (n <= 0) return 0;
  hipLaunchKernelGGL(dict_gather_str_copy_kernel, grid_for(n), 256, 0, (hipStream_t)stream, idx, iw, valid_bytes, dict_offs, dict_bytes, (i64)n, out_offs, out_bytes);
  return hipGetLastError() == hipSuccess ? 0 : -1;
}

struct CometCopyDesc { const uint8_t* src; uint8_t* dst; uint64_t len; };
__global__ __launch_bounds__(256) void copy_small_kernel(const CometCopyDesc* __restrict__ descs) {
  const CometCopyDesc d = descs[blockIdx.y];
  const u64 lo = (u64)blockIdx.x << 14, hi = lo + 16384 < d.len ? lo + 16384 : d.len;
  if (lo >= d.len) return;
  if ((((u64)d.src | (u64)d.dst) & 3u) == 0) {
    const u64 words = (hi - lo) >> 2;
    const u32* s4 = (const u32*)(d.src + lo);
    u32* d4 = (u32*)(d.dst + lo);
    for (u64 i = threadIdx.x; i < words; i += 256) d4[i] = s4[i];
    for (u64 i = lo + (words << 2) + threadIdx.x; i < hi; i += 256) d.dst[i] = d.src[i];
  } else {
    for (u64 i = lo + threadIdx.x; i < hi; i += 256) d.dst[i] = d.src[i];
  }
}
extern "C" int comet_launch_copy_small(const void* descs, int n, uint64_t longest, void* stream) {
  if (n <= 0 || !longest) return 0;
  hipLaunchKernelGGL(copy_small_kernel, dim3((unsigned)((longest + 16383) >> 14), (unsigned)n), 256, 0, (hipStream_t)stream, (const CometCopyDesc*)descs);
  return hipGetLastError() == hipSuccess ? 0 : -1;
}

extern "C" int comet_launch_pmod(const uint32_t* hashes, int64_t n, int32_t np, int32_t* out, void* stream) {
  if (n <= 0) return 0;
  hipLaunchKernelGGL(pmod_kernel, grid_for(n), 256, 0, (hipStream_t)stream, hashes, (i64)n, np, out);
  return hipGetLastError() == hipSuccess ? 0 : -1;
}

struct Q6Static {
  static constexpr int R = 4;
  static constexpr int NW = 3;
  static constexpr bool PIPELINED = false;
  static __device__ __forceinline__ void init(u64* a) { a[0] = a[1] = a[2] = 0; }
  static __device__ __forceinline__ void combine(u64* a, const u64* b) {
    acc_add64(a, b);
    acc_add128(a + 1, b + 1);
  }
  static __device__ __forceinline__ void tile(const CometKParams& prm, i64 base, i64 n, u64* acc) {
    bool k[R];
    i64 idx[R];
    i32 sd[R];
    i64 disc[R], qty[R], price[R];
#pragma unroll
    for (int r = 0; r < R; r++) { idx[r] = base + (i64)r * kBlock + threadIdx.x; k[r] = idx[r] < n; }
#pragma unroll
    for (int r = 0; r < R; r++) if (k[r]) sd[r] = ld<i32>(prm.in[3], idx[r]);
#pragma unroll
    for (int r = 0; r < R; r++) if (k[r]) k[r] = sd[r] >= (i32)prm.iarg[1] && sd[r] < (i32)prm.iarg[2];
#pragma unroll
    for (int r = 0; r < R; r++) if (k[r]) disc[r] = ld_dec_lo(prm.in[2], idx[r]);
#pragma unroll
    for (int r = 0; r < R; r++) if (k[r]) k[r] = disc[r] >= prm.iarg[3] && disc[r] <= prm.iarg[4];
#pragma unroll
    for (int r = 0; r < R; r++) if (k[r]) qty[r] = ld_dec_lo(prm.in[0], idx[r]);
#pragma unroll
    for (int r = 0; r < R; r++) if (k[r]) k[r] = qty[r] < prm.iarg[5];
#pragma unroll
    for (int r = 0; r < R; r++) if (k[r]) price[r] = ld_dec_lo(prm.in[1], idx[r]);
#pragma unroll
    for (int r = 0; r < R; r++) if (k[r]) {
      acc[0] += 1;
      acc_feed_i128(acc + 1, (i128)price[r] * (i128)disc[r]);
    }
// ... 55 lines not shown
```

### include/comet_amd.h

```cpp
#ifndef COMET_AMD_H
#define COMET_AMD_H

#include <stddef.h>
#include <stdint.h>

#ifdef __cplusplus
extern "C" {
#endif
#if defined(__GNUC__)
#pragma GCC visibility push(default)
#endif

struct ArrowArray;
struct ArrowSchema;
struct ArrowDeviceArray;

#define COMET_INPUT_HOST_STREAM 0
#define COMET_INPUT_DEVICE_STREAM 1
#define COMET_INPUT_SHUFFLE_BLOCKS 2

struct CometShuffleBlockStream {
  int64_t (*next_block)(struct CometShuffleBlockStream* self, const uint8_t** data);
  const char* (*get_last_error)(struct CometShuffleBlockStream* self);
  void (*release)(struct CometShuffleBlockStream* self);
  void* private_data;
};

#define COMET_ERR_NATIVE 0
#define COMET_ERR_QUERY_EXECUTION 1

int64_t comet_create_plan(const uint8_t* plan, size_t plan_len, const uint8_t* config, size_t config_len,
                          void** inputs, const int32_t* input_kinds, int32_t n_inputs, int32_t partition_count,
                          int32_t batch_size, int32_t device_id);

int64_t comet_execute_plan(int64_t handle, struct ArrowArray** out_arrays, struct ArrowSchema** out_schemas,
                           int32_t n_out);

int64_t comet_execute_plan_device(int64_t handle, struct ArrowDeviceArray** out_arrays, struct ArrowSchema** out_schemas,
                                  int32_t n_out);

void comet_release_plan(int64_t handle);

const char* comet_last_error(int64_t handle);
int32_t comet_last_error_kind(int64_t handle);

int64_t comet_plan_metrics(int64_t handle, uint8_t* buf, size_t cap);

const char* comet_explain(int64_t handle);

void comet_plan_kernel_stats(int64_t handle, double* kernel_ms, int64_t* launches, int64_t* input_rows);

int64_t comet_plan_kernel_times(int64_t handle, char* buf, size_t cap);
void comet_set_kernel_times(int32_t on);

void comet_plan_aux_kernel_stats(int64_t handle, double* aux_ms, int64_t* aux_launches);

int32_t comet_compile_plan(const uint8_t* plan, size_t plan_len, char* out, size_t cap);

int32_t comet_check_plan(const uint8_t* plan, size_t plan_len, char* out, size_t cap);

int32_t comet_murmur3_column(int32_t type_id, int32_t precision, const void* values, const uint8_t* validity,
                             const void* aux_bytes, int64_t n, uint32_t* hashes, void* hip_stream);
int32_t comet_pmod_partition(const uint32_t* hashes, int64_t n, int32_t num_partitions, int32_t* partition_ids,
                             void* hip_stream);

int32_t comet_partition_indices(const int32_t* partition_ids, int64_t n, int32_t num_partitions, int64_t* partition_starts,
                                uint32_t* partition_row_indices, void* hip_stream);

int32_t comet_take_column(int32_t width_bytes, const void* src, const uint32_t* row_indices, int64_t n, void* dst,
                          void* hip_stream);

int64_t comet_take_utf8_offsets(const int32_t* offsets, const uint8_t* validity_bits, const uint32_t* row_indices, int64_t n,
                                int32_t* out_offsets, void* hip_stream);
int32_t comet_take_utf8_bytes(const int32_t* offsets, const uint8_t* bytes, const uint8_t* validity_bits, const uint32_t* row_indices,
                              int64_t n, const int32_t* out_offsets, uint8_t* out_bytes, void* hip_stream);

int64_t comet_parquet_reader_init(const char* file_path, int64_t file_size, const int64_t* starts, const int64_t* lengths, int32_t n_ranges,
                                  const uint8_t* filter, size_t filter_len, const uint8_t* required_schema_ipc, size_t required_len,
                                  const uint8_t* data_schema_ipc, size_t data_len, const char* session_timezone, int32_t batch_size,
                                  int32_t case_sensitive, int32_t device_id);
int32_t comet_parquet_reader_next(int64_t handle);
int32_t comet_parquet_reader_column(int64_t handle, int32_t column, struct ArrowArray* out_array, struct ArrowSchema* out_schema);
void comet_parquet_reader_close(int64_t handle);

int32_t comet_plan_set_memory_manager(int64_t plan, int64_t (*acquire)(void* ctx, int64_t bytes), void (*release)(void* ctx, int64_t bytes), void* ctx,
                                      int64_t task_id);
void comet_plan_memory_stats(int64_t plan, int64_t* out4);

int64_t comet_parquet_prune_report(const uint8_t* plan, size_t plan_len, int32_t page_index, char* out, size_t cap);
uint64_t comet_xxh64(const uint8_t* data, size_t len, uint64_t seed);
int32_t comet_sbbf_might_contain(const uint8_t* bitset, size_t nbytes, uint64_t hash);
int64_t comet_parquet_host_plain_values(const uint8_t* plan, size_t plan_len, int32_t column, uint8_t* out, size_t cap);

int32_t comet_rlike_match(const char* pattern, const uint8_t* value, size_t value_len);

int32_t comet_regexp_extract_host(const char* pattern, int32_t group, const uint8_t* value, size_t value_len, int32_t* start, int32_t* len);

#ifdef COMET_TEST_ABI
int64_t comet_plan_codegen(const uint8_t* plan, size_t plan_len, const uint8_t* has_valid, int32_t n_valid, char* out, int64_t cap);
int64_t comet_embedded_header(const char* name, char* out, int64_t cap);
int64_t comet_error_site_json(uint32_t site_id, uint64_t lo, uint64_t hi, const uint8_t* str, int64_t str_avail, char* out, int64_t cap);
int comet_calib_read(const void* buf, int64_t bytes, int32_t width, uint64_t* sink, void* stream);
int comet_launch_utf8_uniform(const int32_t* offsets, int64_t n, int32_t L, uint32_t* flag, void* stream);
int32_t comet_spark_bloom_might_contain(const uint8_t* bytes, size_t len, int64_t value);
int64_t comet_spark_bloom_build(const int64_t* values, const uint8_t* valid, int64_t n, int64_t num_items, int64_t num_bits, int32_t version, uint8_t* out, int64_t cap);
#endif

typedef int32_t (*comet_subquery_provider)(void* ctx, int64_t id, int32_t type_id, int32_t* is_null, uint8_t* out, int64_t cap, int64_t* len);
int32_t comet_plan_set_subquery(int64_t handle, int64_t id, int32_t is_null, const uint8_t* value, size_t value_len);
int32_t comet_plan_set_subquery_provider(int64_t handle, comet_subquery_provider provider, void* provider_ctx);

int64_t comet_strfn_host(int32_t op, const uint8_t* value, int32_t n, const uint8_t* a, int32_t na, const uint8_t* b, int32_t nb, int64_t k, uint8_t* out, int64_t cap);

int32_t comet_extract_all_host(const char* pattern, int32_t group, const uint8_t* value, size_t value_len, int32_t* starts, int32_t* lens, int32_t cap);

int32_t comet_split_host(const char* pattern, int32_t limit, const uint8_t* value, size_t value_len, int32_t* starts, int32_t* lens, int32_t cap);

int32_t comet_date_fn_host(int32_t fn, int64_t a, int64_t b, int64_t c, int64_t* out);

int64_t comet_zone_table(const char* zone, int64_t* out, int64_t cap);

int64_t comet_error_json(const char* error_type, const char* error_class, const char* from_type, const char* to_type, int32_t precision, int32_t scale,
                         int32_t value_kind, const char* suffix, uint64_t lo, uint64_t hi, const uint8_t* str, int64_t str_avail, char* out, int64_t cap);

int64_t comet_plan_error_json(const uint8_t* plan, size_t plan_len, int32_t site_index, uint64_t lo, uint64_t hi, const uint8_t* str, int64_t str_avail,
                              char* out, int64_t cap);

int64_t comet_plan_site_error_json(const uint8_t* plan, size_t plan_len, uint32_t site_id, uint64_t lo, uint64_t hi, const uint8_t* str, int64_t str_avail,
                                   char* out, int64_t cap);

int32_t comet_page_decompress(int32_t codec, const uint8_t* src, size_t src_len, uint8_t* dst, size_t dst_len);
int64_t comet_snappy_view_read(const uint8_t* src, size_t src_len, int32_t max_elems, const int64_t* offsets, int32_t n, uint8_t* out);

int64_t comet_snappy_inflate_pages(const uint8_t* streams, const int64_t* stream_off, const int32_t* stream_len, const int32_t* page_len,
                                   int32_t npages, uint8_t* out, const int64_t* out_off, int32_t device_id, double* kernel_ms);
int64_t comet_snappy2_inflate_pages(const uint8_t* streams, const int64_t* stream_off, const int32_t* stream_len, const int32_t* page_len,
                                    int32_t npages, uint8_t* out, const int64_t* out_off, int32_t device_id, double* kernel_ms, uint32_t* status_out);
int64_t comet_zstd2_inflate_pages(const uint8_t* streams, const int64_t* stream_off, const int32_t* stream_len, const int32_t* page_len,
                                  int32_t npages, uint8_t* out, const int64_t* out_off, int32_t device_id, double* kernel_ms, uint32_t* status_out);

typedef struct CometExchangeColumn {
  int32_t type_id;
  int32_t precision;
  const void* values;
  const uint8_t* validity;
  const uint8_t* aux;
} CometExchangeColumn;
int32_t comet_comm_unique_id(uint8_t* out128);
int64_t comet_comm_init_rank(const uint8_t* id128, int32_t world, int32_t rank, int32_t device_id);
int64_t comet_comm_init_local(int64_t group_id, int32_t world, int32_t rank, int32_t device_id);
int64_t comet_comm_init_tcp(const char* peers, int32_t world, int32_t rank, int32_t device_id, int32_t timeout_ms);
const char* comet_comm_transport(int64_t comm);
int32_t comet_comm_stats(int64_t comm, int64_t* out4);
void comet_comm_destroy(int64_t comm);
int64_t comet_exchange(int64_t comm, int32_t n_cols, const CometExchangeColumn* cols, int64_t rows, const int32_t* key_cols, int32_t n_keys);
int64_t comet_exchange_result_rows(int64_t result);
int32_t comet_exchange_result_column(int64_t result, int32_t col, void** values, void** validity);
int32_t comet_exchange_result_aux(int64_t result, int32_t col, void** bytes, int64_t* n_bytes);
void comet_exchange_result_release(int64_t result);
const char* comet_exchange_last_error(void);

int64_t comet_decode_shuffle_block(const uint8_t* block, int64_t len, struct ArrowArray** out_arrays, struct ArrowSchema** out_schemas,
                                   int32_t n_out);

#ifdef COMET_TEST_ABI
int64_t comet_concat_nested_column(struct ArrowArray** arrays, struct ArrowSchema* schema, int32_t n, struct ArrowArray* out, struct ArrowSchema* out_schema);
#endif

int32_t comet_encode_shuffle_block(struct ArrowArray** arrays, struct ArrowSchema** schemas, int32_t n_cols, int32_t codec,
                                   int32_t compression_level, uint8_t** out, int64_t* out_len);
void comet_free_buffer(uint8_t* p);

int64_t comet_columnar_to_row_init(int32_t batch_size, int32_t device_id);
int32_t comet_columnar_to_row_convert(int64_t handle, struct ArrowArray** arrays, struct ArrowSchema** schemas, int32_t n_cols, int64_t num_rows,
                                      const uint8_t** out_buffer, const int32_t** out_offsets, const int32_t** out_lengths);
void comet_columnar_to_row_close(int64_t handle);
const char* comet_columnar_to_row_error(int64_t handle);

void comet_sort_row_partitions(int64_t* records, int64_t n);

int32_t comet_write_sorted_rows(const int64_t* row_addresses, const int32_t* row_sizes, int64_t row_num, const uint8_t* const* serialized_datatypes,
                                const int32_t* datatype_lens, int32_t n_cols, const char* file_path, int32_t batch_size, int32_t checksum_enabled,
                                int32_t checksum_algo, int64_t current_checksum, const char* compression_codec, int32_t compression_level,
                                int64_t out_result[3]);

int32_t comet_parquet_describe(const char* path, char* out, size_t cap);
// ... 13 lines not shown
```

Before: 72.63 billion rows/s.

## Piggyback error-flag reads on existing syncs and batch Utf8 uniform checks

Device error-flag checks now queue a 16-byte read of the error header alongside readbacks that already happen, so each check no longer needs its own extra synchronize and copy. The header is cached and reused by later aggregate finalization. Separately, the per-column Utf8 offset-uniformity kernels are merged into one multi-column launch, which uses unit-based tiling and nontemporal vector loads. This cuts launches and host round trips at the cost of more state to track about whether the cached error header is still valid.

```diff
diff --git a/datafusion-comet_amd/csrc/exec.cpp b/datafusion-comet_amd/csrc/exec.cpp
--- a/datafusion-comet_amd/csrc/exec.cpp
+++ b/datafusion-comet_amd/csrc/exec.cpp
@@ -953,6 +953,7 @@
 void ExecutionContext::launch(Variant& v, const char* kernel, int grid, CometKParams& prm, int block) {
   hipFunction_t fn = v.mod->fn(kernel);
   if (!v.desc.blooms.empty()) bind_blooms(v.desc, prm);
+  err_head_known_ = false;
   void* args[] = {&prm};
   if (!g_kernel_times.load(std::memory_order_relaxed)) {
     HIP_CHECK(hipModuleLaunchKernel(fn, (unsigned)grid, 1, 1, (unsigned)block, 1, 1, 0, stream_, args, nullptr));
@@ -1760,6 +1761,13 @@
   std::vector<std::vector<uint8_t>> hv(ncol), hb(ncol);
   std::vector<std::vector<uint8_t>> hd(ncol);
   struct Piece { const void* src; std::vector<uint8_t>* dst; size_t bytes; };
+  bool head_fetched = false;
+  auto wait = [&] {
+    const bool with_head = !head_fetched && err_flags_.p;
+    if (with_head) queue_err_head_read();
+    HIP_CHECK(hipStreamSynchronize(stream_));
+    if (with_head) { (void)queued_err_head(); head_fetched = true; }
+  };
   auto fetch = [&](std::vector<Piece>& pieces) {
     size_t total = 0, longest = 0;
     for (auto& pc : pieces) { pc.dst->resize(pc.bytes); total += (pc.bytes + 15) & ~(size_t)15; longest = std::max(longest, pc.bytes); }
@@ -1778,14 +1786,14 @@
         at += (pieces[k].bytes + 15) & ~(size_t)15;
       }
       if (comet_launch_copy_small(export_host_.p, (int)pieces.size(), (uint64_t)longest, stream_) != 0) throw CometError("result export: launch failed");
-      HIP_CHECK(hipStreamSynchronize(stream_));
+      wait();
       for (size_t k = 0; k < pieces.size(); k++)
         if (pieces[k].bytes) memcpy(pieces[k].dst->data(), d[k].dst, pieces[k].bytes);
       return;
     }
     for (auto& pc : pieces)
       if (pc.bytes) HIP_CHECK(hipMemcpyAsync(pc.dst->data(), pc.src, pc.bytes, hipMemcpyDeviceToHost, stream_));
-    HIP_CHECK(hipStreamSynchronize(stream_));
+    wait();
   };
   std::vector<Piece> pieces;
   for (size_t j = 0; j < ncol; j++) {
@@ -1805,7 +1813,12 @@
     }
   }
   fetch(pieces);
-  check_device_errors();
+  if (head_fetched) {
+    collect_timings();
+    raise_device_errors(err_head_[0]);
+  } else {
+    check_device_errors();
+  }
   const int64_t bs = batch_size_ > 0 ? batch_size_ : t.rows;
   auto getbit = [](const std::vector<uint8_t>& b, int64_t i) { return (b[(size_t)(i >> 3)] >> (i & 7)) & 1; };
   for (int64_t off = 0; off < t.rows; off += bs) {
@@ -1869,6 +1882,7 @@
     stream_ = pool_get_stream(device_id_);
     err_flags_.ensure(kErrBytes);
     HIP_CHECK(hipMemsetAsync(err_flags_.p, 0, kErrBytes, stream_));
+    err_head_known_ = false;
     started_ = true;
   } else {
     HIP_CHECK(hipSetDevice(device_id_));
@@ -1920,8 +1934,7 @@
   } else {
     tab = materialize(*plan_);
   }
-  HIP_CHECK(hipStreamSynchronize(stream_));
-  check_device_errors();
+  sync_and_check_device_errors();
   collect_timings();
   finished_ = true;
   if ((size_t)n_out != tab.cols.size())
diff --git a/datafusion-comet_amd/csrc/exec.hpp b/datafusion-comet_amd/csrc/exec.hpp
--- a/datafusion-comet_amd/csrc/exec.hpp
+++ b/datafusion-comet_amd/csrc/exec.hpp
@@ -182,7 +182,7 @@
   DevTable scan_parquet(const Operator& native_scan);
   friend struct ParquetScan;
   friend struct HashJoinRun;
-  int64_t launch_fused_filter(Variant& v, CometKParams& prm, int64_t n);
+  int64_t launch_fused_filter(Variant& v, CometKParams& prm, int64_t n, uint32_t* head = nullptr);
   DevTable run_chain_to_device(const Operator& top, const DevTable& in);
   void extend_derived(DevTable& in, const std::vector<DerivedCol>& derived);
   void extend_derived_strfn(DevTable& in, const DerivedCol& dc);
@@ -225,6 +225,7 @@
   void validate_input_schema(size_t input, const std::vector<DType>& types);
   void export_batch(HostBatch& b, ArrowArray** out_arrays, ArrowSchema** out_schemas, int n_out);
   void check_device_errors();
+  void sync_and_check_device_errors();
   void raise_device_errors(uint32_t flags);
   void note_sites(const PipelineDesc& d) {
     site_ctx_last_.clear();
@@ -250,6 +251,12 @@
   std::shared_ptr<QueryContext> agg_ctx_[2];
   std::map<uint32_t, std::shared_ptr<QueryContext>> site_ctx_;
   void read_small(void* dst, const void* dev_src, size_t n);
+  void read_small_and_head(void* dst, const void* dev_src, size_t n, uint32_t head[4]);
+  bool err_head_known_ = false;
+  uint32_t err_head_[4] = {0, 0, 0, 0};
+  void remember_err_head(const void* head16);
+  void queue_err_head_read();
+  const uint32_t* queued_err_head();
   void write_small(void* dev_dst, const void* src, size_t n);
   void timed_begin();
   void timed_end();
diff --git a/datafusion-comet_amd/csrc/exec_bloom.cpp b/datafusion-comet_amd/csrc/exec_bloom.cpp
--- a/datafusion-comet_amd/csrc/exec_bloom.cpp
+++ b/datafusion-comet_amd/csrc/exec_bloom.cpp
@@ -205,8 +205,10 @@
   if (comet_launch_bloom_finish(f, spec.num_words, (uint8_t*)bytes->p, popcnt, stream_) != 0) throw CometError("bloom_filter_agg: launch failed");
   timed_end();
   uint64_t set_bits = 0;
-  read_small(&set_bits, popcnt, 8);
-  check_device_errors();
+  uint32_t head[4];
+  read_small_and_head(&set_bits, popcnt, 8, head);
+  collect_timings();
+  raise_device_errors(head[0]);
   const bool is_null = op.agg_mode == AggMode::Final && set_bits == 0;
   const int32_t o[2] = {0, is_null ? 0 : (int32_t)out_len};
   write_small(out_offs->p, o, sizeof o);
diff --git a/datafusion-comet_amd/csrc/exec_input.cpp b/datafusion-comet_amd/csrc/exec_input.cpp
--- a/datafusion-comet_amd/csrc/exec_input.cpp
+++ b/datafusion-comet_amd/csrc/exec_input.cpp
@@ -593,10 +593,9 @@
     std::vector<bool> declared(scols.size(), false);
     uint32_t* flags = (uint32_t*)err_flags_.p + (kErrBytes / 4 - 16);
     HIP_CHECK(hipMemsetAsync(flags, 0, 64, stream_));
-    bool any = false;
     if (!aux_ev_[0]) { aux_ev_[0] = pool_get_event(device_id_); aux_ev_[1] = pool_get_event(device_id_); }
     HIP_CHECK(hipEventRecord(aux_ev_[0], stream_));
-    int aux_launched = 0;
+    std::vector<CometUtf8Check> checks;
     for (size_t k = 0; k < scols.size(); k++) {
       first[k] = ends[2 * k];
       const int64_t total = (int64_t)ends[2 * k + 1] - ends[2 * k];
@@ -612,19 +611,18 @@
           views[scols[k]].fixed_len = hint;
           continue;
         }
-        if (comet_launch_utf8_uniform(off, rows, hint, flags + k, stream_) != 0) continue;
-        aux_launched++;
+        checks.push_back(CometUtf8Check{off, rows, hint, flags + k});
         len[k] = hint;
         declared[k] = true;
-        any = true;
         continue;
       }
       if (total % rows != 0 || total / rows > 15 || total < 0) continue;
-      if (comet_launch_utf8_uniform(off, rows, (int32_t)(total / rows), flags + k, stream_) != 0) continue;
-      aux_launched++;
+      checks.push_back(CometUtf8Check{off, rows, (int32_t)(total / rows), flags + k});
       len[k] = (int32_t)(total / rows);
-      any = true;
-    }
+    }
+    bool any = !checks.empty();
+    if (any && comet_launch_utf8_uniform_multi(checks.data(), (int32_t)checks.size(), stream_) != 0) throw CometError("Utf8 offset check: launch failed");
+    const int aux_launched = any ? 1 : 0;
     if (any) {
       HIP_CHECK(hipEventRecord(aux_ev_[1], stream_));
       uint32_t f[16];
diff --git a/datafusion-comet_amd/csrc/exec_internal.hpp b/datafusion-comet_amd/csrc/exec_internal.hpp
--- a/datafusion-comet_amd/csrc/exec_internal.hpp
+++ b/datafusion-comet_amd/csrc/exec_internal.hpp
@@ -114,6 +114,11 @@
                                         void* stream);
 extern "C" int comet_launch_fix_rescale(uint64_t* base, int64_t count, int64_t stride_words, int32_t word_off, int32_t shift, void* stream);
 extern "C" int comet_launch_utf8_uniform(const int32_t* offsets, int64_t n, int32_t L, uint32_t* flag, void* stream);
+#ifndef COMET_UTF8_CHECK_DEFINED
+#define COMET_UTF8_CHECK_DEFINED
+struct CometUtf8Check { const int32_t* offsets; int64_t n; int32_t L; uint32_t* flag; };
+#endif
+extern "C" int comet_launch_utf8_uniform_multi(const CometUtf8Check* checks, int32_t ncols, void* stream);
 
 namespace comet {
 HostColumn download_column(const DeviceColumnView& v, const DType& t, bool has_valid, int64_t rows, hipStream_t st);
diff --git a/datafusion-comet_amd/csrc/exec_join.cpp b/datafusion-comet_amd/csrc/exec_join.cpp
--- a/datafusion-comet_amd/csrc/exec_join.cpp
+++ b/datafusion-comet_amd/csrc/exec_join.cpp
@@ -363,7 +363,9 @@
       const int64_t ptiles = (n + 4095) / 4096;
       cx.launch(v, probe_kernel(table, keymap_built), (int)std::min<int64_t>(ptiles, table == JoinTable::Lds ? 256 * 3 : 256 * 8), prm);
       uint64_t words[8] = {0, 0, 0, 0, 0, 0, 0, 0};
-      cx.read_small(words, counters.p, sizeof words);
+      uint32_t err_head[4];
+      if (fused_probe || fused_build) cx.read_small_and_head(words, counters.p, sizeof words, err_head);
+      else cx.read_small(words, counters.p, sizeof words);
       if (table == JoinTable::Bucket && words[kCntOverflow]) {
         cx.timed_end();
         HIP_CHECK(hipStreamSynchronize(stream()));
@@ -409,7 +411,10 @@
   DevTable finish() {
     const int nbuild = (int)B.cols.size();
     DevTable out = cx.outputs_to_table(v, vals, vbytes, out_rows, [&](int c) { return c < nbuild ? std::make_pair(&B, c) : std::make_pair(&P, c - nbuild); });
-    if (fused_probe || fused_build) cx.check_device_errors();
+    if (fused_probe || fused_build) {
+      if (cx.err_head_known_) cx.raise_device_errors(cx.err_head_[0]);
+      else cx.check_device_errors();
+    }
     if (tail_rows > 0 || n == 0) HIP_CHECK(hipStreamSynchronize(stream()));
     out.owners.push_back(v.mod);
     cx.join_build_rows_ += B.rows;
diff --git a/datafusion-comet_amd/csrc/exec_pipeline.cpp b/datafusion-comet_amd/csrc/exec_pipeline.cpp
--- a/datafusion-comet_amd/csrc/exec_pipeline.cpp
+++ b/datafusion-comet_amd/csrc/exec_pipeline.cpp
@@ -77,6 +77,7 @@
       alloc_table(group_table_, group_cap_);
       group_table_clear_ = true;
       HIP_CHECK(hipMemsetAsync((char*)err_flags_.p + 8, 0, 8, stream_));
+      err_head_known_ = false;
     }
     const int64_t tile = (int64_t)d.R * 256;
     int grid_mult = 4;
@@ -99,6 +100,7 @@
       uint64_t head[2 + (kErrBytes - 16) / 8];
       uint32_t flags[4];
       read_small(head, err_flags_.p, d.fix_sums.empty() ? 16 : sizeof head);
+      remember_err_head(head);
       memcpy(flags, head, 16);
       uint64_t groups_now;
       memcpy(&groups_now, &flags[2], 8);
@@ -183,14 +185,16 @@
     timed_begin();
     if (d.has_filter) {
       bind_outputs(n);
-      out_rows = launch_fused_filter(v, prm, n);
+      uint32_t head[4];
+      out_rows = launch_fused_filter(v, prm, n, head);
+      collect_timings();
+      raise_device_errors(head[0]);
     } else {
       bind_outputs(n);
       int grid = (int)std::min<int64_t>((n + 255) / 256, 256 * 8);
       launch(v, "k_emit", grid, prm);
-    }
-    timed_end();
-    check_device_errors();
+      timed_end();
+    }
     if (out_rows == 0) return;
     std::vector<std::vector<uint8_t>> hv(ncol), hk(ncol);
     for (size_t j = 0; j < ncol; j++) {
@@ -202,7 +206,12 @@
         HIP_CHECK(hipMemcpyAsync(hk[j].data(), out_valid_[j]->p, hk[j].size(), hipMemcpyDeviceToHost, stream_));
       }
     }
+    if (!d.has_filter) queue_err_head_read();
     HIP_CHECK(hipStreamSynchronize(stream_));
+    if (!d.has_filter) {
+      collect_timings();
+      raise_device_errors(queued_err_head()[0]);
+    }
     const int64_t bs = batch_size_ > 0 ? batch_size_ : out_rows;
     for (int64_t off = 0; off < out_rows; off += bs) {
       int64_t len = std::min(bs, out_rows - off);
@@ -246,7 +255,29 @@
   HIP_CHECK(hipStreamSynchronize(stream_));
   memcpy(dst, small_host_.p, n);
 }
+void ExecutionContext::read_small_and_head(void* dst, const void* dev_src, size_t n, uint32_t head[4]) {
+  if (n > 2048 - 16) throw CometError("internal: read_small_and_head of " + std::to_string(n) + " bytes (its staging holds 2032)");
+  small_host_.ensure(4096);
+  HIP_CHECK(hipMemcpyAsync(small_host_.p, dev_src, n, hipMemcpyDeviceToHost, stream_));
+  queue_err_head_read();
+  HIP_CHECK(hipStreamSynchronize(stream_));
+  memcpy(dst, small_host_.p, n);
+  memcpy(head, queued_err_head(), 16);
+}
+void ExecutionContext::queue_err_head_read() {
+  small_host_.ensure(4096);
+  HIP_CHECK(hipMemcpyAsync((char*)small_host_.p + 2048 - 16, err_flags_.p, 16, hipMemcpyDeviceToHost, stream_));
+}
+void ExecutionContext::remember_err_head(const void* head16) {
+  memcpy(err_head_, head16, 16);
+  err_head_known_ = true;
+}
+const uint32_t* ExecutionContext::queued_err_head() {
+  remember_err_head((const char*)small_host_.p + 2048 - 16);
+  return err_head_;
+}
 void ExecutionContext::write_small(void* dev_dst, const void* src, size_t n) {
+  if (dev_dst == err_flags_.p) err_head_known_ = false;
   if (n > 2048) throw CometError("internal: write_small of " + std::to_string(n) + " bytes (its staging holds 2048)");
   small_host_.ensure(4096);
   if (n <= 128) {
@@ -288,6 +319,17 @@
   read_small(flags, err_flags_.p, 16);
   collect_timings();
   raise_device_errors(flags[0]);
+}
+
+void ExecutionContext::sync_and_check_device_errors() {
+  if (!err_flags_.p) {
+    HIP_CHECK(hipStreamSynchronize(stream_));
+    return;
+  }
+  queue_err_head_read();
+  HIP_CHECK(hipStreamSynchronize(stream_));
+  collect_timings();
+  raise_device_errors(queued_err_head()[0]);
 }
 
 void ExecutionContext::raise_device_errors(uint32_t f) {
@@ -356,6 +398,7 @@
     prm.out[kOutFirstCol + 2 * j + 1] = vbytes[j]->p;
   }
   HIP_CHECK(hipMemsetAsync((char*)err_flags_.p + 8, 0, 8, stream_));
+  err_head_known_ = false;
   prm.out[1] = recs.p;
   prm.out[3] = part.p;
   prm.iarg[2] = np;
@@ -477,7 +520,8 @@
   uint64_t ngroups = 0;
   {
     uint32_t hdr[4] = {0, 0, 0, 0};
-    read_small(hdr, err_flags_.p, 16);
+    if (err_head_known_) memcpy(hdr, err_head_, 16);
+    else read_small(hdr, err_flags_.p, 16);
     collect_timings();
     memcpy(&ngroups, hdr + 2, 8);
     raise_device_errors(hdr[0]);
@@ -524,7 +568,8 @@
   uint64_t ngroups = 0;
   {
     uint32_t head[4] = {0, 0, 0, 0};
-    read_small(head, err_flags_.p, 16);
+    if (err_head_known_) memcpy(head, err_head_, 16);
+    else read_small(head, err_flags_.p, 16);
     collect_timings();
     raise_device_errors(head[0]);
     memcpy(&ngroups, head + 2, 8);
@@ -580,8 +625,10 @@
     hk[j].p = (const uint8_t*)host_arena.p + valid_base + j * valid_stride;
     hk[j].n = (size_t)ngroups;
   }
+  queue_err_head_read();
   HIP_CHECK(hipStreamSynchronize(stream_));
-  check_device_errors();
+  collect_timings();
+  raise_device_errors(queued_err_head()[0]);
   const int64_t total = (int64_t)ngroups;
   const int64_t bs = batch_size_ > 0 ? batch_size_ : total;
   for (int64_t off = 0; off < total; off += bs) {
@@ -656,7 +703,7 @@
   return rerun;
 }
 
-int64_t ExecutionContext::launch_fused_filter(Variant& v, CometKParams& prm, int64_t n) {
+int64_t ExecutionContext::launch_fused_filter(Variant& v, CometKParams& prm, int64_t n, uint32_t* head) {
   const int64_t tile_rows = 256 * (int64_t)v.desc.R;
   const int64_t ntiles = (n + tile_rows - 1) / tile_rows;
   scratch_mask_.ensure((size_t)ntiles * 8 + 64);
@@ -667,7 +714,12 @@
   prm.out[1] = scratch_counts_.p;
   launch(v, "k_filter", (int)std::min<int64_t>(ntiles, 256 * 8), prm);
   uint64_t total = 0;
-  read_small(&total, (char*)scratch_counts_.p + 8, 8);
+  if (head) {
+    timed_end();
+    read_small_and_head(&total, (char*)scratch_counts_.p + 8, 8, head);
+  } else {
+    read_small(&total, (char*)scratch_counts_.p + 8, 8);
+  }
   return (int64_t)total;
 }
 
diff --git a/datafusion-comet_amd/csrc/exec_shuffle.cpp b/datafusion-comet_amd/csrc/exec_shuffle.cpp
--- a/datafusion-comet_amd/csrc/exec_shuffle.cpp
+++ b/datafusion-comet_amd/csrc/exec_shuffle.cpp
@@ -110,8 +110,7 @@
     grouped.cols.resize(n_payload);
     grouped.has_valid.resize(n_payload);
   }
-  HIP_CHECK(hipStreamSynchronize(stream_));
-  check_device_errors();
+  sync_and_check_device_errors();
   shuffle_repart_ns_ += tm.ns();
   lap("partition (murmur3, pmod, indices, takes)");
 
diff --git a/datafusion-comet_amd/csrc/exec_window.cpp b/datafusion-comet_amd/csrc/exec_window.cpp
--- a/datafusion-comet_amd/csrc/exec_window.cpp
+++ b/datafusion-comet_amd/csrc/exec_window.cpp
@@ -353,8 +353,7 @@
     HIP_CHECK(hipStreamSynchronize(stream_));
   }
   timed_end();
-  HIP_CHECK(hipStreamSynchronize(stream_));
-  check_device_errors();
+  sync_and_check_device_errors();
   return out;
 }
 
@@ -409,8 +408,7 @@
   if (!u.mod) throw CometError("Expand: every projection consists of NULL literals only");
   DevTable out = outputs_to_table(u, vals, vbytes, total, [&](int c) { return std::make_pair(&in, c); });
   out.owners.push_back(u.mod);
-  HIP_CHECK(hipStreamSynchronize(stream_));
-  check_device_errors();
+  sync_and_check_device_errors();
   return out;
 }
 
diff --git a/datafusion-comet_amd/csrc/kernels_static.hip b/datafusion-comet_amd/csrc/kernels_static.hip
--- a/datafusion-comet_amd/csrc/kernels_static.hip
+++ b/datafusion-comet_amd/csrc/kernels_static.hip
@@ -1,4 +1,7 @@
 #include <hip/hip_runtime.h>
+
+#include <algorithm>
+#include <cstring>
 
 #include "device/comet_device.hpp"
 
@@ -33,33 +36,65 @@
   for (i64 i = (i64)blockIdx.x * 256 + threadIdx.x; i < n; i += (i64)gridDim.x * 256) out[i] = pmod(hashes[i], np);
 }
 
-__global__ __launch_bounds__(256) void utf8_uniform_kernel(const i32* off, i64 n, i32 L, u32* flag) {
-  bool bad = false;
-  const i32 o0 = off[0];
-  const i64 total = n + 1;
-  i64 head = 0;
-  while (head < total && ((((uintptr_t)(off + head)) & 15) != 0)) head++;
-  const int4* v4 = (const int4*)(off + head);
-  const i64 ngroups = (total - head) / 4;
-  constexpr int U = 4;
-  for (i64 g0 = ((i64)blockIdx.x * 256 + threadIdx.x) * U; g0 < ngroups; g0 += (i64)gridDim.x * 256 * U) {
-    int4 v[U];
-#pragma unroll
-    for (int u = 0; u < U; u++) v[u] = g0 + u < ngroups ? v4[g0 + u] : make_int4(0, 0, 0, 0);
-#pragma unroll
-    for (int u = 0; u < U; u++) {
-      if (g0 + u < ngroups) {
-        const i64 i = head + 4 * (g0 + u);
-        const i32 e = o0 + (i32)(i * L);
+constexpr int kUtf8CheckMaxCols = 16, kUtf8CheckLoads = 8, kUtf8CheckUnit = 256 * kUtf8CheckLoads, kUtf8CheckMaxGrid = 256 * 8;
+struct Utf8CheckCol {
+  const i32* off;
+  u32* flag;
+  i64 total;
+  i64 head;
+  i64 ngroups;
+  i64 unit_end;
+  i32 L;
+};
+struct Utf8CheckArgs {
+  Utf8CheckCol col[kUtf8CheckMaxCols];
+  i32 ncols;
+};
+typedef i32 utf8_v4i __attribute__((ext_vector_type(4)));
+
+__global__ __launch_bounds__(256) void utf8_uniform_kernel(const Utf8CheckArgs a) {
+  const i64 units = a.col[a.ncols - 1].unit_end;
+  int k = 0;
+  i32 o0 = a.col[0].off[0];
+  for (i64 unit = blockIdx.x; unit < units; unit += gridDim.x) {
+    if (unit >= a.col[k].unit_end) {
+      while (unit >= a.col[k].unit_end) k++;
+      o0 = a.col[k].off[0];
+    }
+    const i32* off = a.col[k].off;
+    const i64 total = a.col[k].total, head = a.col[k].head, ngroups = a.col[k].ngroups;
+    const i32 L = a.col[k].L;
+    const i64 g0 = (unit - (k ? a.col[k - 1].unit_end : 0)) * kUtf8CheckUnit + threadIdx.x;
+    const COMET_GLOBAL utf8_v4i* v4 = (const COMET_GLOBAL utf8_v4i*)(off + head) + g0;
+    const i64 left = ngroups - (g0 - threadIdx.x);
+    bool bad = false;
+    utf8_v4i v[kUtf8CheckLoads];
+    if (left >= kUtf8CheckUnit) {
+#pragma unroll
+      for (int u = 0; u < kUtf8CheckLoads; u++) v[u] = __builtin_nontemporal_load(v4 + u * 256);
+#pragma unroll
+      for (int u = 0; u < kUtf8CheckLoads; u++) {
+        const i32 e = o0 + (i32)((head + 4 * (g0 + u * 256)) * L);
         bad |= (v[u].x != e) | (v[u].y != e + L) | (v[u].z != e + 2 * L) | (v[u].w != e + 3 * L);
       }
-    }
-  }
-  if (blockIdx.x == 0) {
-    for (i64 i = threadIdx.x; i < head; i += 256) bad |= off[i] != o0 + (i32)(i * L);
-    for (i64 i = head + ngroups * 4 + threadIdx.x; i < total; i += 256) bad |= off[i] != o0 + (i32)(i * L);
-  }
-  if (__any(bad) && lane_id() == 0) atomicOr(flag, 1u);
+    } else {
+#pragma unroll
+      for (int u = 0; u < kUtf8CheckLoads; u++)
+        if (g0 + u * 256 < ngroups) v[u] = __builtin_nontemporal_load(v4 + u * 256);
+#pragma unroll
+      for (int u = 0; u < kUtf8CheckLoads; u++) {
+        if (g0 + u * 256 < ngroups) {
+          const i32 e = o0 + (i32)((head + 4 * (g0 + u * 256)) * L);
+          bad |= (v[u].x != e) | (v[u].y != e + L) | (v[u].z != e + 2 * L) | (v[u].w != e + 3 * L);
+        }
+      }
+    }
+    if (g0 == threadIdx.x) {
+      for (i64 i = threadIdx.x; i < head; i += 256) bad |= off[i] != o0 + (i32)(i * L);
+      for (i64 i = head + ngroups * 4 + threadIdx.x; i < total; i += 256) bad |= off[i] != o0 + (i32)(i * L);
+    }
+    if (__any(bad) && lane_id() == 0) atomicOr(a.col[k].flag, 1u);
+  }
 }
 
 __device__ __forceinline__ i64 dict_index(const void* idx, int iw, i64 i) {
@@ -185,10 +220,33 @@
   return hipGetLastError() == hipSuccess ? 0 : -1;
 }
 
+struct CometUtf8Check { const int32_t* offsets; int64_t n; int32_t L; uint32_t* flag; };
+extern "C" int comet_launch_utf8_uniform_multi(const CometUtf8Check* checks, int32_t ncols, void* stream) {
+  if (ncols < 0 || ncols > kUtf8CheckMaxCols) return -1;
+  Utf8CheckArgs a;
+  memset(&a, 0, sizeof a);
+  i64 units = 0;
+  for (int32_t k = 0; k < ncols; k++) {
+    if (checks[k].n <= 0) continue;
+    Utf8CheckCol& c = a.col[a.ncols++];
+    c.off = checks[k].offsets;
+    c.flag = checks[k].flag;
+    c.L = checks[k].L;
+    c.total = checks[k].n + 1;
+    const uintptr_t addr = (uintptr_t)c.off;
+    c.head = (addr & 3) ? c.total : std::min<i64>(c.total, (i64)(((16 - (addr & 15)) & 15) / 4));
+    c.ngroups = (c.total - c.head) / 4;
+    units += std::max<i64>(1, (c.ngroups + kUtf8CheckUnit - 1) / kUtf8CheckUnit);
+    c.unit_end = units;
+  }
+  if (!a.ncols) return 0;
+  hipLaunchKernelGGL(utf8_uniform_kernel, (int)std::min<i64>(units, kUtf8CheckMaxGrid), 256, 0, (hipStream_t)stream, a);
+  return hipGetLastError() == hipSuccess ? 0 : -1;
+}
+extern "C" int comet_utf8_uniform_max_grid(void) { return kUtf8CheckMaxGrid; }
 extern "C" int comet_launch_utf8_uniform(const int32_t* offsets, int64_t n, int32_t L, uint32_t* flag, void* stream) {
-  if (n <= 0) return 0;
-  hipLaunchKernelGGL(utf8_uniform_kernel, grid_for(n), 256, 0, (hipStream_t)stream, offsets, (i64)n, L, flag);
-  return hipGetLastError() == hipSuccess ? 0 : -1;
+  const CometUtf8Check one = {offsets, n, L, flag};
+  return comet_launch_utf8_uniform_multi(&one, 1, stream);
 }
 
 extern "C" int comet_launch_dict_gather_fixed(const void* idx, int iw, const uint8_t* idx_valid, const uint8_t* dict, const uint8_t* dict_valid,
diff --git a/include/comet_amd.h b/include/comet_amd.h
--- a/include/comet_amd.h
+++ b/include/comet_amd.h
@@ -102,6 +102,12 @@
 int64_t comet_error_site_json(uint32_t site_id, uint64_t lo, uint64_t hi, const uint8_t* str, int64_t str_avail, char* out, int64_t cap);
 int comet_calib_read(const void* buf, int64_t bytes, int32_t width, uint64_t* sink, void* stream);
 int comet_launch_utf8_uniform(const int32_t* offsets, int64_t n, int32_t L, uint32_t* flag, void* stream);
+#ifndef COMET_UTF8_CHECK_DEFINED
+#define COMET_UTF8_CHECK_DEFINED
+struct CometUtf8Check { const int32_t* offsets; int64_t n; int32_t L; uint32_t* flag; };
+#endif
+int comet_launch_utf8_uniform_multi(const struct CometUtf8Check* checks, int32_t ncols, void* stream);
+int comet_utf8_uniform_max_grid(void);
 int32_t comet_spark_bloom_might_contain(const uint8_t* bytes, size_t len, int64_t value);
 int64_t comet_spark_bloom_build(const int64_t* values, const uint8_t* valid, int64_t n, int64_t num_items, int64_t num_bits, int32_t version, uint8_t* out, int64_t cap);
 #endif
```

New measurement: 74.22 billion rows/s (median of 6 runs). 2.2% higher.
